# autonomousvision/gta

Hardware: AMD Instinct MI355X
Metric: GTA-attn Mtokens/s (V=5,H=W=128,d=768) (higher is better)
Workload: dtype bf16; 1 GPU; ms-enc: GTA attention forward (rep build + K/V rep pre-pass + attention kernel), B=32/GPU, H=8, Tq=1280, Tk=1280, dh=96, f_dims={'triv': 0, 'se3': 48, 'so3': 24, 'so2': 24}, views q/k=5/5; global_batch=32, parallelism=dp1

## Files before the change

gta_amd/csrc/gen_attn64.py:

```python
#!/usr/bin/env python3
import argparse

from isa_model import CheckError, Ins, barrier, branch, check_wait_states, clobber_list, label, nop, wait, write_macro

RB = 2
KS, DB, CHP = 6, 3, 12
IMG = 64 * CHP * 16
TILE = 2 * IMG
NP = IMG // 4096
THR_BITS = 0x42c00000


def _sbase(p, rb, hh):
    return 64 + 16 * rb if hh == 0 else 96 + 16 * (p * 2 + rb)


def S(p, rb, hh, r=None):
    b = _sbase(p, rb, hh)
    return f"v[{b}:{b + 15}]" if r is None else f"v{b + r}"


def Sregs(p, rb, hh):
    b = _sbase(p, rb, hh)
    return [f"v{b + i}" for i in range(16)]
# ... 620 lines not shown
                if fallthrough and step_state is not None and pend and [sorted(x) for x in pend] != [sorted(x) for x in step_state]:
                    raise CheckError(f"outstanding LDS reads at {ins.label} differ between paths")
                if fallthrough and pend:
                    step_state = [set(x) for x in pend]
                elif step_state is not None:
                    pend = [set(x) for x in step_state]
            else:
                if pend and fallthrough:
                    out.append(wait(lgkm=0))
                pend = []
            out.append(ins)
            prev = ins
            continue
        if ins.kind == "branch":
            uncond = ins.text.startswith("s_branch")
            to_step = ins.target.startswith("L_step")
            rare = ins.target.startswith("L_slow") or ins.target.startswith("L_tail")
            if pend and ((uncond and not (to_step and carry)) or (not uncond and not rare)):
                out.append(wait(lgkm=0))
                pend = []
            if uncond and to_step and carry and pend:
                if step_state is None:
                    step_state = [set(x) for x in pend]
                elif [sorted(x) for x in pend] != [sorted(x) for x in step_state]:
                    raise CheckError(f"outstanding LDS reads at the jump to {ins.target} differ from the step label's state")
            out.append(ins)
            prev = ins
            continue
        if ins.kind == "wait" and ins.fx[2] is not None:
            del pend[:max(0, len(pend) - ins.fx[2])]
            out.append(ins)
            prev = ins
            continue
        touched = list(ins.rd) + list(ins.wr)
        i = need(touched)
        if i >= 0:
            left = min(len(pend) - 1 - i, 15)
            out.append(wait(lgkm=left))
            del pend[:len(pend) - left]
        if ins.kind == "ready":
            continue
        out.append(ins)
        if ins.kind == "ds":
            pend.append(set(ins.wr))
        prev = ins
    if pend:
        out.append(wait(lgkm=0))
    if carry and seed_state is None and step_state is not None:
        return insert_waits(prog, carry=True, seed_state=step_state)
    return out


class Sim:
    def __init__(self, gen, prog, n_tiles, rebase_at=(), has_tail=False, items=2, first_rebase=True):
        self.g, self.prog, self.n, self.rebase_at, self.has_tail, self.items = gen, prog, n_tiles, set(rebase_at), has_tail, items
        self.first_rebase = first_rebase or not gen.first_fast
        self.labels = {ins.label: i for i, ins in enumerate(prog) if ins.kind == "label"}
        self.count = 0

    def fail(self, msg, ins=None):
        raise CheckError(f"{msg}" + (f"   at: {ins.text}" if ins is not None else ""))

    def run(self):
        R = self.g.R
        self.kslot = [None] * R
        self.vslot = [None] * R
        self.vmq = []
        self.got = {}
        self.hist = []
        stats = {"instr": 0, "mfma": 0}
        for t in range(R):
            for i in range(NP):
                self.vmq.append(("K", t % R, i, (0, t)))
        for t in range(R - 1):
            for i in range(NP):
                self.vmq.append(("V", t % R, i, (0, t)))
        kptr, vptr = (0, R), (0, R - 1)
        for item in range(self.items):
            kptr, vptr = self.run_item(item, kptr, vptr, stats)
        return stats

    def land(self, ent):
        ring, slot, piece, tile = ent
        key = (ring, slot)
        cur = self.pending_tile.get(key)
        if cur is None or cur[0] != tile:
            self.pending_tile[key] = (tile, set())
        self.pending_tile[key][1].add(piece)

    def run_item(self, item, kptr, vptr, stats):
        g, R, n = self.g, self.g.R, self.n
        regs = {}
        pend_ds = []
        pending_regs = set()
        sc = {}
        self.pending_tile = getattr(self, "pending_tile", {})
        msver = [0, 0]
        o_done = {(rb, d): set() for rb in range(RB) for d in range(DB)}
        l_done = {rb: set() for rb in range(RB)}
        sums = {}
        packed_from = {}
        exps = {}
        flags = {"scc": 0, "vcc": 0}
        ksel_done = vsel_done = False
        pc = 0
        prog = self.prog
        rebased_tiles = set()
        steps = 0

        def setreg(r, tag, need):
            old = regs.get(r)
            if old is not None and old[1] > 0:
                self.fail(f"register {r} overwritten with {old[1]} reads of {old[0]} outstanding", cur)
            regs[r] = [tag, need]

        def usereg(r, expect_prefix, cur_ins):
            v = regs.get(r)
            if v is None:
                self.fail(f"register {r} read but never written (expected {expect_prefix})", cur_ins)
            if r in pending_regs:
                self.fail(f"register {r} read before its LDS read was waited for", cur_ins)
            if tuple(v[0][:len(expect_prefix)]) != tuple(expect_prefix):
                self.fail(f"register {r} holds {v[0]}, expected {expect_prefix}", cur_ins)
            v[1] -= 1
            return v[0]

        while True:
            if pc >= len(prog):
                self.fail("fell off the end of the program")
            cur = prog[pc]
            pc += 1
            if cur.kind == "label":
                continue
            stats["instr"] += 1
            check_wait_states(self.hist, cur)
            sem = cur.sem
            k = cur.kind
            for r in list(cur.rd) + list(cur.wr):
                if r in pending_regs and k != "ds":
                    self.fail(f"{r} touched while its LDS read is outstanding", cur)
            if k == "mfma":
                stats["mfma"] += 1
            if sem is None:
                self.hist.append(cur)
                continue
            op = sem[0]
            if op == "nop":
                pass
            elif op == "waitcnt":
                vm, lgkm = sem[1:]
                while lgkm is not None and len(pend_ds) > lgkm:
                    for r in pend_ds.pop(0):
                        pending_regs.discard(r)
                while vm is not None and len(self.vmq) > vm:
                    self.land(self.vmq.pop(0))
            elif op == "barrier":
                for key, (tile, pieces) in list(self.pending_tile.items()):
                    if len(pieces) == NP:
                        (self.kslot if key[0] == "K" else self.vslot)[key[1]] = tile
                        del self.pending_tile[key]
            elif op == "item_begin":
                for t in range(R):
                    if self.kslot[t] != (item, t):
                        self.fail(f"item {item}: K slot {t} holds {self.kslot[t]} at item begin")
                for t in range(R - 1):
                    if self.vslot[t] != (item, t):
                        self.fail(f"item {item}: V slot {t} holds {self.vslot[t]} at item begin")
            elif op == "j0":
                sc["j"] = 0
            elif op == "j1":
                sc["j1"] = sc["j"] + 1
            elif op == "jinc":
                sc["j"] += 1
                steps += 1
            elif op in ("nm1", "nmr", "nmr1", "readkn", "ds_tab"):
                if op == "ds_tab":
                    pend_ds.append(list(cur.wr))
                    pending_regs.update(cur.wr)
            elif op == "cmp_nmr":
                flags["scc_eq"] = sc["j"] == n - R
            elif op == "cmp_nmr1":
                flags["scc_eq"] = sc["j"] == n - R + 1
            elif op == "kinit":
                sc["kptr"] = kptr
            elif op == "vinit":
                sc["vptr"] = vptr
            elif op == "ksel":
                if flags["scc_eq"]:
                    if sc["kptr"] != (item, n):
                        self.fail(f"K stream switches items at position {sc['kptr']}")
                    sc["kptr"] = (item + 1, 0)
                    ksel_done = True
            elif op == "vsel":
                if flags["scc_eq"]:
                    if sc["vptr"] != (item, n):
                        self.fail(f"V stream switches items at position {sc['vptr']}")
                    sc["vptr"] = (item + 1, 0)
                    vsel_done = True
            elif op == "kadv":
                if sem[1] == 0:
                    sc["kptr"] = (sc["kptr"][0], sc["kptr"][1] + 1)
            elif op == "vadv":
                if sem[1] == 0:
                    sc["vptr"] = (sc["vptr"][0], sc["vptr"][1] + 1)
            elif op == "dma":
                ring, slot, piece = sem[1], sem[2], sem[3]
                tile = sc["kptr"] if ring == "K" else sc["vptr"]
                held = (self.kslot if ring == "K" else self.vslot)[slot]
                if held is not None and held[0] == item:
                    last_needed = held[1] - 1 if ring == "K" else held[1]
                    if last_needed >= sc["j"]:
                        self.fail(f"DMA into {ring} slot {slot} at step {sc['j']} while tile {held} is still needed", cur)
                if piece == 0:
                    (self.kslot if ring == "K" else self.vslot)[slot] = None
                self.vmq.append((ring, slot, piece, tile))
            elif op == "ds_k":
                slot, ks, hh, rel = sem[1], sem[2], sem[3], sem[4]
                t = sc.get("j", 0) + rel
# ... 280 lines not shown
```

gta_amd/csrc/gen_item64.py:

```python
#!/usr/bin/env python3
import argparse

import numpy as np

import gen_attn64 as G
from isa_model import (LANES, Asm, CheckError, Ins, Wave, as_u32, assemble_check, auto_waits, bf16_rne, bf16_to_f32, check_wait_states, clobber_list,
                       regs, rtext, u2f, write_macro)

KS, DB, RB, R = 6, 3, 2, 4
IMG = 64 * 12 * 16
TILE = 2 * IMG
OFF_K, OFF_V, OFF_TAB = 0, R * IMG, 2 * R * IMG
OFF_CS = OFF_TAB + (KS + 2 * DB) * 256
CS_ROW, CS_WAVE = 96, 64 * 96
OFF_X = OFF_CS + 256 * CS_ROW
XROW, XB = 208, 32 * 208
OFF_ITEMS = OFF_X + 4 * XB
ITEM_BYTES = 64
MAX_ITEMS = 128
LDS_BYTES = OFF_ITEMS + (MAX_ITEMS + 2) * ITEM_BYTES
QT_BYTES = 1024
LN2_BITS, QN_BITS = 0x3f317218, 0x3f808659
assert LDS_BYTES <= 160 * 1024 and OFF_ITEMS % 16 == 0

D_Q, D_O, D_CS, D_LSE, D_IMG, D_KN, D_AQ, D_V = 0, 2, 4, 6, 8, 10, 12, 13
D_WORDS = 14


def row0(i):
    return 5 * i + i // 3


def V(n, k=1):
    return regs("v", n, k)


def A(n, k=1):
    return regs("a", n, k)


def Sr(n, k=1):
    return regs("s", n, k)


V_LANE16, V_LANE4 = "v8", "v9"
V_XFR = "v10"
V_XL = ["v11", "v12", "v13"]
V_QG = ["v14", "v15", "v16"]
V_OG = ["v17", "v18", "v19"]
V_CSG, V_CSG2 = "v20", "v21"
V_CSR, V_CSRA, V_CSRB = "v23", "v24", "v25"
V_OXW = "v26"
V_LSE = "v27"
V_QN = ["v28", "v29"]
V_KN = "v30"
V_LR, V_MR = ["v240", "v241"], ["v242", "v243"]
TMP = V(244, 12)
TMPX = TMP + ["v31", "v22"]
QL = [A(220 + 4 * i, 4) for i in range(9)] + [A(4 * i, 4) for i in range(3)]
AT = [A(172 + 4 * i, 4) for i in range(12)]
CT = [A(124 + 4 * i, 4) for i in range(12)]
S_STAMP = Sr(20, 4)
S_B = [Sr(24 + 2 * j, 2) for j in range(4)]
S_Q16, S_O16, S_XW = "s54", "s55", "s34"
S_PREV, S_ROW = Sr(36, 2), Sr(38, 2)
S_CUR, S_NXT = 40, 56
S_KPTR, S_VPTR, S_NXK, S_NXV = Sr(72, 2), Sr(74, 2), Sr(76, 2), Sr(78, 2)
S_WOFF = "s80"
S_T = Sr(81, 3)
S_K, S_TAB = "s97", "s35"
S_PH3 = Sr(98, 2)
S_HI = Sr(70, 2)
CLOBBER_S = [i for i in range(20, 100) if i != 32]

LOOP_OPERANDS = {"%[kptr]": rtext(S_KPTR), "%[vptr]": rtext(S_VPTR), "%[nxt_k]": rtext(S_NXK), "%[nxt_v]": rtext(S_NXV),
                 "%[woff]": S_WOFF, "%[lane16]": V_LANE16, "%[qn0]": V_QN[0], "%[qn1]": V_QN[1], "%[kn]": V_KN,
                 "%[lr0]": V_LR[0], "%[lr1]": V_LR[1], "%[mr0]": V_MR[0], "%[mr1]": V_MR[1]}
OPERANDS = ("tabl", "nit", "wave", "qrb", "orb", "qtb_lo", "qtb_hi", "prof_lo", "prof_hi", "n", "tailj", "Tk")


def cur(d, k=2):
    return Sr(S_CUR + d, k) if k > 1 else f"s{S_CUR + d}"


def nxt(d, k=2):
    return Sr(S_NXT + d, k) if k > 1 else f"s{S_NXT + d}"


class ItemGen:
    def __init__(self, loop_kw=None, stamps=True, head_wait=False, phases=False):
        self.loop_kw = dict(G.BEST) if loop_kw is None else loop_kw
        self.stamps = stamps
        self.head_wait = head_wait
        self.phases = phases

    def phase(self, a, k):
        if not self.phases:
            return
        t = TMP
        self._nph = getattr(self, "_nph", 0) + 1
        lab = f"L_noph{k}_{self._nph}_%="
        a.waitcnt(lgkm=0)
        a.s_or_b32(S_T[0], "%[prof_lo]", "%[prof_hi]")
        a.branch("s_cbranch_scc0", lab)
        if k == 3:
            a.s_memtime(S_PH3)
            a.waitcnt(lgkm=0)
            a.label(lab)
            return
        a.s_memtime(S_T[1:3])
        a.waitcnt(lgkm=0)
        a.s_exec_set("lane0")
        a.v_mov_b32(t[4], 0)
        a.v_mov_b32(t[6], S_T[1])
        a.v_mov_b32(t[7], S_T[2])
        a.global_store(2, t[4], t[6:8], S_ROW, 8 * (1, 2, 3)[k])
        a.s_exec_set("all")
        a.label(lab)

    def hi(self, a):
        a.s_exec_set("hi", S_HI)

    def chunk_prologue(self, a):
        t = TMP
        lane, l31, lh = t[0], t[1], t[2]
        a.v_mbcnt_lane(lane)
        a.v_and_b32(l31, 31, lane)
        a.v_lshrrev_b32(lh, 5, lane)
        a.v_lshlrev_b32(V_LANE16, 4, lane)
        a.v_lshlrev_b32(V_LANE4, 2, lane)
        a.s_mul_i32(S_XW, "%[wave]", XB)
        a.s_add_u32(S_XW, S_XW, OFF_X)
        a.s_mul_i32(S_WOFF, "%[wave]", IMG // 4)
        a.s_lshl_b32(S_Q16, "%[qrb]", 4)
        a.s_lshl_b32(S_O16, "%[orb]", 4)
        a.s_mov_b32(S_HI[0], 0)
        a.s_mov_b32(S_HI[1], -1)
        a.s_lshl_b32(S_T[0], "%[wave]", 6)
        for m in range(3):
            lm, g, col = t[3], t[4], t[5]
            a.v_add_u32(lm, 4 * m, lane)
            a.v_mul_u32_u24(g, 43, lm)
            a.v_lshrrev_b32(g, 9, g)
            a.v_mul_u32_u24(col, 12, g)
            a.v_sub_u32(col, lm, col)
            a.v_lshlrev_b32(col, 4, col)
            a.v_mul_u32_u24(t[6], XROW, g)
            a.v_add_u32(t[6], t[6], col)
            a.v_add_u32(V_XL[m], S_XW, t[6])
            a.v_add_u32(t[7], row0(m), g)
            a.v_add_u32(t[7], S_T[0], t[7])
            a.v_mul_lo_u32(t[6], t[7], "%[qrb]")
            a.v_add_u32(V_QG[m], t[6], col)
            a.v_add_u32(t[7], row0(m), g)
            a.v_mul_lo_u32(t[6], t[7], "%[orb]")
            a.v_add_u32(V_OG[m], t[6], col)
        a.s_mul_i32(S_T[1], "%[wave]", CS_WAVE)
        a.v_add_u32(V_CSG, S_T[1], V_LANE16)
        a.v_add_u32(V_CSG2, 4096, V_CSG)
        a.s_mov_b32(S_K, 0)
        a.s_mov_b32(S_TAB, "%[tabl]")
        if self.phases:
            a.s_mov_b64(S_PH3, 0)
        self.read_desc(a, 0)
        self.request(a)
        self.cs_dma(a)
        self.advance_desc(a)
        a.v_mbcnt_lane(lane)
        a.v_and_b32(l31, 31, lane)
        a.v_lshrrev_b32(lh, 5, lane)
        a.v_mul_u32_u24(t[3], XROW, l31)
        a.v_add_u32(t[3], S_XW, t[3])
        a.v_lshlrev_b32(t[4], 4, lh)
        a.v_add_u32(V_XFR, t[3], t[4])
        a.v_lshlrev_b32(t[4], 5, lh)
        a.v_add_u32(V_OXW, t[3], t[4])
        a.s_mul_i32(S_T[1], "%[wave]", CS_WAVE)
        a.s_add_u32(S_T[1], S_T[1], OFF_CS)
        a.v_mul_u32_u24(t[3], CS_ROW, l31)
        a.v_add_u32(V_CSR, S_T[1], t[3])
        a.v_lshlrev_b32(t[4], 5, lh)
        a.v_add_u32(V_CSRA, V_CSR, t[4])
        a.v_lshlrev_b32(t[4], 6, lh)
        a.v_add_u32(V_CSRB, V_CSR, t[4])
        a.s_lshl_b32(S_T[0], "%[wave]", 6)
        a.v_add_u32(t[3], S_T[0], l31)
        a.v_lshlrev_b32(V_LSE, 2, t[3])
        a.v_add_u32(t[3], OFF_TAB, V_LANE4)
        for i, r in enumerate(G.KOFF + [G.VOFF[d][h] for d in range(DB) for h in range(2)]):
            a.ds_read(32, [r], t[3], 256 * i)
        a.waitcnt(lgkm=0)
        self.read_desc(a, 1)
        self.stamp_row(a, S_PREV)
        a.waitcnt(vm=0)

    def read_desc(self, a, entry):
        t = TMPX
        a.v_mov_b32(V_QN[0], S_TAB)
        for i in range(3):
            a.ds_read(128, t[4 * i:4 * i + 4], V_QN[0], ITEM_BYTES * entry + 16 * i)
        a.ds_read(32, [t[12]], V_QN[0], ITEM_BYTES * entry + 48)
        a.ds_read(32, [t[13]], V_QN[0], ITEM_BYTES * entry + 52)
        a.waitcnt(lgkm=0)
        for d in range(D_WORDS):
            a.v_readfirstlane_b32(f"s{S_NXT + d}", t[d])

    def advance_desc(self, a):
        for d in range(0, D_WORDS, 2):
            a.s_mov_b64(Sr(S_CUR + d, 2), Sr(S_NXT + d, 2))

    def bases(self, a, first, step, n=4):
        a.s_mov_b64(S_B[0], first)
        for j in range(1, n):
            a.s_add_u32(S_B[j][0], S_B[j - 1][0], step)
            a.s_addc_u32(S_B[j][1], S_B[j - 1][1], 0)

    def tile_bases(self, a, desc, typ):
        a.s_add_u32(S_B[0][0], "%[qtb_lo]", desc(D_AQ, 1))
        a.s_addc_u32(S_B[0][1], "%[qtb_hi]", 0)
        if typ:
            a.s_add_u32(S_B[0][0], S_B[0][0], 12 * QT_BYTES)
            a.s_addc_u32(S_B[0][1], S_B[0][1], 0)
        for j in range(1, 3):
            a.s_add_u32(S_B[j][0], S_B[j - 1][0], 4096)
            a.s_addc_u32(S_B[j][1], S_B[j - 1][1], 0)

    def request(self, a):
        self.bases(a, nxt(D_Q), S_Q16)
        for i in range(12):
            a.global_load(4, QL[i], V_QG[i % 3], S_B[i // 3])
        self.tile_bases(a, nxt, 0)
        for i in range(12):
            a.global_load(4, AT[i], V_LANE16, S_B[i // 4], 1024 * (i % 4))
        a.global_load(1, [V_KN], V_LANE4, nxt(D_KN))

    def cs_dma(self, a):
        a.s_mul_i32(S_T[0], "%[wave]", CS_WAVE)
        for part, (voff, cnt) in enumerate(((V_CSG, 4), (V_CSG2, 2))):
            a.add(f"s_add_u32 m0, {S_T[0]}, {OFF_CS + 4096 * part}", "salu", [S_T[0]], ["m0", "scc"], ("s_add_m0", S_T[0], OFF_CS + 4096 * part))
            a.nop(1)
            for i in range(cnt):
                a.add(f"global_load_lds_dwordx4 {voff}, {rtext(nxt(D_CS))}" + (f" offset:{1024 * i}" if i else ""), "dma",
                      ["m0", voff] + nxt(D_CS), [], ("global_load_lds", voff, nxt(D_CS), 1024 * i))

    def stamp_row(self, a, dst):
        a.s_lshl_b32(S_T[0], cur(D_V, 1), 6)
        a.s_add_u32(dst[0], "%[prof_lo]", S_T[0])
        a.s_addc_u32(dst[1], "%[prof_hi]", 0)

    def stamp(self, a, tag, last=False):
        if not self.stamps:
            return
        lab = f"L_nostamp_{tag}_%="
        t = TMP
        a.s_or_b32(S_T[0], "%[prof_lo]", "%[prof_hi]")
        a.branch("s_cbranch_scc0", lab)
        a.s_memtime(S_STAMP[0:2])
        a.s_memrealtime(S_STAMP[2:4])
        a.waitcnt(lgkm=0)
        if not last:
            self.stamp_row(a, S_ROW)
        a.s_exec_set("lane0")
        a.v_mov_b32(t[4], 0)
        for i in range(4):
            a.v_mov_b32(t[i], S_STAMP[i])
        a.global_store(2, t[4], t[0:2], S_PREV, 8 * 4)
        a.global_store(2, t[4], t[2:4], S_PREV, 8 * 6)
        if self.phases:
            a.v_mov_b32(t[6], S_PH3[0])
            a.v_mov_b32(t[7], S_PH3[1])
            a.global_store(2, t[4], t[6:8], S_PREV, 8 * 7)
        if not last:
            a.global_store(2, t[4], t[0:2], S_ROW, 8 * 0)
            a.global_store(2, t[4], t[2:4], S_ROW, 8 * 5)
            a.s_mov_b64(S_PREV, S_ROW)
        a.s_exec_set("all")
        a.label(lab)

    def prologue(self, a):
        t = TMP
        QR = [[V(44 + 4 * (rb * KS + ks), 4) for ks in range(KS)] for rb in range(RB)]
        ACC = [[V(92 + 48 * rb + 16 * d, 16) for d in range(DB)] for rb in range(RB)]
        CSP = [[V(188 + 16 * rb + 8 * sl, 8) for sl in range(2)] for rb in range(RB)]
        QSQ = ["v220", "v221"]
        PK = V(222, 8)
        a.waitcnt(vm=14)
        self.phase(a, 0)
        for rb in range(RB):
            for i in range(KS):
                a.ds_write(128, V_XL[i % 3], QL[rb * KS + i], row0(i) * XROW)
            for ks in range(KS):
                a.ds_read(128, QR[rb][ks], V_XFR, 32 * ks)
        for rb in range(RB):
            for h in range(2):
                a.ds_read(128, CSP[rb][0][4 * h:4 * h + 4], V_CSR, rb * 32 * CS_ROW + 16 * h)
            for h in range(2):
                a.ds_read(128, CSP[rb][1][4 * h:4 * h + 4], V_CSRA, rb * 32 * CS_ROW + 32 + 16 * h)

        def mfmas(rb):
            out = []
            for i in range(12):
                d, kk, lo = i % 3, (i // 3) & 1, i // 6
                tl = 2 * d + kk
                out.append((ACC[rb][d], AT[6 * lo + tl], QR[rb][tl], 0 if i < 3 else ACC[rb][d]))
            return out

        def post(rb):
            ops = []
            for ks in range(KS):
                x = ACC[rb][ks >> 1][8 * (ks & 1):8 * (ks & 1) + 8]
                if ks >= 4:
                    cs = CSP[rb][ks - 4]
                    if ks == 4:
                        ops.append(lambda: self.hi(a))
                    for p in range(4):
                        x0, x1, c, s = x[2 * p], x[2 * p + 1], cs[2 * p], cs[2 * p + 1]
                        tt = t[p]
                        ops.append(lambda x1=x1, s=s, tt=tt: a.v_mul_f32(tt, x1, s))
                        ops.append(lambda x1=x1, c=c: a.v_mul_f32(x1, x1, c))
                        ops.append(lambda x0=x0, x1=x1, s=s: a.v_fmac_f32(x1, x0, s))
                        ops.append(lambda x0=x0, c=c, tt=tt: a.v_fma_f32(x0, x0, c, tt, neg=(False, False, True)))
                    if ks == 4:
                        ops.append(lambda: a.s_exec_set("all"))
                pk = PK[4 * (ks & 1):4 * (ks & 1) + 4]
                for w in range(4):
                    ops.append(lambda w=w, pk=pk, x=x: a.v_cvt_pk_bf16_f32(pk[w], x[2 * w], x[2 * w + 1]))
                for w in range(4):
                    ops.append(lambda w=w, pk=pk, ks=ks: a.v_accvgpr_write_b32(G.Qregs(rb, ks)[w], pk[w]))
                for i in range(8):
                    if ks == 0 and i == 0:
                        ops.append(lambda x=x: a.v_mul_f32(QSQ[rb], x[0], x[0]))
                    else:
                        ops.append(lambda i=i, x=x: a.v_fmac_f32(QSQ[rb], x[i], x[i]))
            return ops

        m0, m1 = mfmas(0), mfmas(1)
        for d16, a4, b4, c in m0:
            a.mfma(d16, a4, b4, c)
        p0 = post(0)
        k = 0
# ... 140 lines not shown
            k = 0
            for i, (d16, a4, b4, c) in enumerate(mf):
                a.mfma(d16, a4, b4, c)
                if pad_at is not None and i == pad_at:
                    a.nop(pad)
                if i >= first:
                    for _ in range(per):
                        if k < len(fill):
                            fill[k]()
                            k += 1
            while k < len(fill):
                fill[k]()
                k += 1

        for op in build_of(0):
            op()
        arith, a = a.out, main
        mi, per = 0, max(1, len(arith) // max(len(mem.out), 1))
        for i, ins in enumerate(arith):
            a.raw(ins)
            if (i + 1) % per == 0 and mi < len(mem.out):
                a.raw(mem.out[mi])
                mi += 1
        for ins in mem.out[mi:]:
            a.raw(ins)
        a.s_lshl_b32(S_T[0], "%[wave]", 2)
        a.s_mul_i32(S_T[0], S_T[0], S_O16)
        a.s_add_u32(S_B[0][0], cur(D_O)[0], S_T[0])
        a.s_addc_u32(S_B[0][1], cur(D_O)[1], 0)
        for j in range(1, 4):
            a.s_add_u32(S_B[j][0], S_B[j - 1][0], S_O16)
            a.s_addc_u32(S_B[j][1], S_B[j - 1][1], 0)
        a.waitcnt(vm=0 if last else 31)
        weave(mfmas(0), build_of(1))
        weave(mfmas(1), post(0) + stores(0), first=3, pad_at=2, pad=8)
        a.nop(8)
        for op in post(1) + stores(1):
            op()
        a.s_exec_set("lo")
        for rb in range(RB):
            a.global_store(1, V_LSE, [t[8 + rb]], cur(D_LSE), 128 * rb)
        a.s_exec_set("all")

    def loop_program(self):
        G.configure(96)
        gen = G.Gen(R=R, **self.loop_kw)
        out = []
        head_vm = not self.head_wait
        for ins in gen.program():
            if ins.sem and ins.sem[0] == "ds_tab":
                continue
            if head_vm and ins.kind == "wait" and ins.fx == ("waitcnt", 0, None):
                head_vm = False
                continue
            out.append(ins.bound(LOOP_OPERANDS))
        return gen, out

    def program(self, stub_loop=False, pad4=False):
        a = Asm()
        self.chunk_prologue(a)
        a.label("L_item_%=")
        self.stamp(a, "item")
        self.prologue(a)
        a.waitcnt(lgkm=0)
        self.phase(a, 1)
        if pad4:
            a.nop(1)
        head = auto_waits(a.out)
        a = Asm()
        self.phase(a, 2)
        a.s_add_u32(S_T[0], S_K, 1)
        a.s_cmp("ge", "u32", S_T[0], "%[nit]")
        a.branch("s_cbranch_scc1", "L_last_%=")
        self.epilogue(a)
        a.waitcnt(lgkm=0)
        self.phase(a, 3)
        self.advance_desc(a)
        a.s_add_u32(S_K, S_K, 1)
        a.s_add_u32(S_TAB, S_TAB, ITEM_BYTES)
        self.read_desc(a, 1)
        a.branch("s_branch", "L_item_%=")
        a.label("L_last_%=")
        self.epilogue(a, last=True)
        a.waitcnt(lgkm=0)
        self.phase(a, 3)
        self.stamp(a, "end", last=True)
        a.waitcnt(vm=0)
        a.pseudo("end")
        tail = auto_waits(a.out)
        if stub_loop:
            mid = [Ins("", "pseudo", fx=("pseudo", "loop"))]
        else:
            mid = self.loop_program()[1]
        return head + mid + tail


def qt_chan_q(d, rho):
    lh, j, i = (rho >> 2) & 1, rho >> 3, rho & 3
    return 32 * d + 8 * lh + 4 * j + i if j < 2 else 32 * d + 16 + 8 * lh + 4 * (j - 2) + i


def qt_chan_o_in(d, kk, k):
    lh, i = k >> 3, k & 7
    return 32 * d + 16 * kk + (i & 3) + 8 * (i >> 2) + 4 * lh


# ... 8 lines not shown
    for typ, M in ((0, Mf), (1, Mi)):
        for d in range(3):
            for kk in range(2):
                for rho in range(32):
                    r = qt_chan_o_out(d, rho) if typ else qt_chan_q(d, rho)
                    for k in range(16):
                        c = qt_chan_o_in(d, kk, k) if typ else 32 * d + 16 * kk + k
                        x = np.float32(M[r, c])
                        hi = bf16_rne(np.array([x], np.float32))[0]
                        lo = bf16_rne(np.array([x - bf16_to_f32(np.uint32(hi))], np.float32))[0]
                        for part, val in ((0, hi), (1, lo)):
                            tile = 12 * typ + 6 * part + 2 * d + kk
                            o16[(tile * 1024 + (((k >> 3) * 32 + rho) * 16 + (k & 7) * 2)) // 2] = val
    return out


def decode_matrix(tiles, typ):
    M = np.zeros((96, 96), np.float64)
    t16 = tiles.view(np.uint16)
    for d in range(3):
        for kk in range(2):
            for rho in range(32):
                r = qt_chan_o_out(d, rho) if typ else qt_chan_q(d, rho)
                for k in range(16):
                    c = qt_chan_o_in(d, kk, k) if typ else 32 * d + 16 * kk + k
                    for part in range(2):
                        tile = 12 * typ + 6 * part + 2 * d + kk
                        M[r, c] += float(bf16_to_f32(np.uint32(t16[(tile * 1024 + (((k >> 3) * 32 + rho) * 16 + (k & 7) * 2)) // 2])))
    return M


class Case:

    def __init__(self, seed, n_items, exact, n_tiles=8):
        rng = np.random.default_rng(seed)
        self.rng, self.exact, self.n_items, self.n_tiles = rng, exact, n_items, n_tiles
        B, H, Nq, Tq = 2, 3, 2, 512
        self.B, self.H, self.Nq, self.Tq = B, H, Nq, Tq
        self.q_st, self.o_st = 3 * H * 96, H * 96
        if exact:
            q = rng.integers(-3, 4, size=(B, Tq, 3 * H * 96)).astype(np.float32)
        else:
            q = rng.standard_normal((B, Tq, 3 * H * 96)).astype(np.float32)
        self.qbits = bf16_rne(q).astype(np.uint16)
        self.obits = np.zeros((B, Tq, H * 96), np.uint16)
        if exact:
            ang = rng.integers(0, 4, size=(B, Tq, 12))
            cs = np.stack([np.round(np.cos(ang * np.pi / 2)), np.round(np.sin(ang * np.pi / 2))], -1).astype(np.float32)
        else:
            ang = rng.uniform(0, 2 * np.pi, size=(B, Tq, 12))
            cs = np.stack([np.cos(ang), np.sin(ang)], -1).astype(np.float32)
        self.cs = cs
        self.lse = np.zeros((B, H, Tq), np.float32)
        self.kn = rng.uniform(0.5, 2.0, size=(B, H, 64)).astype(np.float32)
        self.Mf, self.Mi, tiles = [], [], []
        for v in range(B * Nq):
            Mf, Mi = np.zeros((96, 96)), np.zeros((96, 96))
            scale = 2.0 if exact else 0.1472
            for M, inv in ((Mf, 0), (Mi, 1)):
                blocks = [(4 * i, 4) for i in range(12)] + [x for g in range(3) for x in ((48 + 8 * g, 3), (51 + 8 * g, 5))]
                for o, n in blocks:
                    if exact:
                        blk = rng.integers(-2, 3, size=(n, n)).astype(np.float64)
                    else:
                        blk = rng.standard_normal((n, n)) * (1.0 if inv else scale)
                    M[o:o + n, o:o + n] = blk
                for c in range(72, 96):
                    M[c, c] = 1.0 if inv else scale
            self.Mf.append(Mf); self.Mi.append(Mi)
            tiles.append(build_view_tiles(Mf, Mi))
        self.tiles = np.concatenate(tiles)
        self.MfD = [decode_matrix(self.tiles[24 * 1024 * v:24 * 1024 * (v + 1)], 0) for v in range(B * Nq)]
        self.MiD = [decode_matrix(self.tiles[24 * 1024 * v:24 * 1024 * (v + 1)], 1) for v in range(B * Nq)]
        self.A_Q, self.A_O, self.A_CS, self.A_LSE, self.A_KN, self.A_QT, self.A_IMG, self.A_PROF = (0x1000000 * (i + 1) for i in range(8))
        self.items = []
        order = rng.permutation(B * H * 2)[:n_items]
        for w in order:
            bh, qt = divmod(int(w), 2)
            b, h = divmod(bh, H)
            self.items.append(dict(b=b, h=h, q0=256 * qt, view=(256 * qt) // (Tq // Nq), V=int(w)))
        self.oacc, self.lrun, self.mrun = {}, {}, {}

    def desc(self, it):
        b, h, q0 = it["b"], it["h"], it["q0"]
        bh = b * self.H + h
        d = np.zeros(16, np.uint32)

        def put(i, addr):
            d[i], d[i + 1] = addr & 0xffffffff, addr >> 32
        put(D_Q, self.A_Q + ((b * self.Tq + q0) * self.q_st + h * 96) * 2)
        put(D_O, self.A_O + ((b * self.Tq + q0) * self.o_st + h * 96) * 2)
        put(D_CS, self.A_CS + ((b * self.Tq + q0) * 24) * 4)
        put(D_LSE, self.A_LSE + (bh * self.Tq + q0) * 4)
        put(D_IMG, self.A_IMG + bh * self.n_tiles * TILE)
        put(D_KN, self.A_KN + bh * 64 * 4)
        d[D_AQ] = (b * self.Nq + it["view"]) * 24 * 1024
        d[D_V] = it["V"]
        return d

    def loop_results(self, item, wave):
        key = (item, wave)
        if key not in self.oacc:
            rng = np.random.default_rng(1000 * item + wave + 7)
            if self.exact:
                l_half = np.full((RB, LANES), 2.0, np.float32)
                o = (rng.integers(-8, 9, size=(RB, DB, 16, LANES)) * 4).astype(np.float32)
            else:
                l_half = rng.uniform(1.0, 40.0, size=(RB, LANES)).astype(np.float32)
                o = (rng.standard_normal((RB, DB, 16, LANES)) * 8).astype(np.float32)
            self.oacc[key], self.lrun[key] = o, l_half
            self.mrun[key] = rng.uniform(-3, 9, size=(RB, 32)).astype(np.float32)
        return self.oacc[key], self.lrun[key], self.mrun[key]

    def expect_q(self, item, wave):
        it = self.items[item]
        out = np.zeros((RB, 32, 96), np.float64)
        for rb in range(RB):
            for r in range(32):
                t = it["q0"] + wave * 64 + rb * 32 + r
                q = bf16_to_f32(self.qbits[it["b"], t, it["h"] * 96:(it["h"] + 1) * 96].astype(np.uint32)).astype(np.float64)
                x = self.MfD[it["b"] * self.Nq + it["view"]] @ q
                for p in range(12):
                    c, s = (float(v) for v in self.cs[it["b"], t, p])
                    x0, x1 = x[72 + 2 * p], x[73 + 2 * p]
                    x[72 + 2 * p], x[73 + 2 * p] = c * x0 - s * x1, s * x0 + c * x1
                out[rb, r] = x
        return out

    def expect_o(self, item, wave):
        it = self.items[item]
        o, lh_, m = self.loop_results(item, wave)
        rows = np.zeros((RB, 32, 96), np.float64)
        lse = np.zeros((RB, 32), np.float64)
        for rb in range(RB):
            for r in range(32):
                l = np.float32(lh_[rb, r] + lh_[rb, r + 32])
                inv = np.float32(1.0) / l
                ot = np.zeros(96, np.float64)
                for d in range(DB):
                    for reg in range(16):
                        for h in range(2):
                            chan = 32 * d + (reg & 3) + 8 * (reg >> 2) + 4 * h
                            ot[chan] = bf16_to_f32(bf16_rne(np.array([o[rb, d, reg, r + 32 * h] * inv], np.float32)))[0]
                t = it["q0"] + wave * 64 + rb * 32 + r
                x = self.MiD[it["b"] * self.Nq + it["view"]] @ ot
                for p in range(12):
                    c, s = (float(v) for v in self.cs[it["b"], t, p])
                    x0, x1 = x[72 + 2 * p], x[73 + 2 * p]
                    x[72 + 2 * p], x[73 + 2 * p] = c * x0 + s * x1, c * x1 - s * x0
                rows[rb, r] = x
                lse[rb, r] = (float(m[rb, r]) + np.log2(float(l))) * np.log(2.0)
        return rows, lse


def run_case(prog, case, wave, prof=False):
    LDS0 = np.zeros(160 * 1024, np.uint8)
    n = case.n_items
    for k in range(n + 2):
        it = case.items[min(k, n - 1)]
        LDS0[OFF_ITEMS + 64 * k:OFF_ITEMS + 64 * k + 64] = case.desc(it).view(np.uint8)
    tab = (np.arange(12 * 64, dtype=np.uint32) * 4 + 0x100000).view(np.uint8)
    LDS0[OFF_TAB:OFF_TAB + len(tab)] = tab
    inputs = {"%[tabl]": OFF_ITEMS, "%[nit]": n, "%[wave]": wave, "%[qrb]": case.q_st * 2, "%[orb]": case.o_st * 2,
              "%[qtb_lo]": case.A_QT & 0xffffffff, "%[qtb_hi]": case.A_QT >> 32,
              "%[prof_lo]": (case.A_PROF & 0xffffffff) if prof else 0, "%[prof_hi]": (case.A_PROF >> 32) if prof else 0,
              "%[n]": case.n_tiles, "%[tailj]": 0xffffffff, "%[Tk]": 64 * case.n_tiles}
    w = Wave(inputs=inputs, seed=wave + 11)
    w.lds[:] = LDS0
    qb = case.qbits.reshape(-1).view(np.uint8)
    ob = case.obits.reshape(-1).view(np.uint8)
    profb = np.zeros(64 * 64, np.uint8)
    for base, arr in ((case.A_Q, qb), (case.A_O, ob), (case.A_CS, case.cs.reshape(-1).view(np.uint8)), (case.A_LSE, case.lse.reshape(-1).view(np.uint8)),
                      (case.A_KN, case.kn.reshape(-1).view(np.uint8)), (case.A_QT, case.tiles), (case.A_PROF, profb)):
        w.map_buffer(base, arr)
    state = {"item": 0}
    tol = 0.0 if case.exact else 2.0 ** -7

    def chk(name, got, want, rel):
        got, want = np.asarray(got, np.float64), np.asarray(want, np.float64)
        err = np.abs(got - want)
        lim = rel * np.maximum(np.abs(want), 1e-3) + (0 if rel == 0 else 1e-6)
        if not (err <= lim).all():
            i = np.unravel_index(np.argmax(err - lim), err.shape)
            raise CheckError(f"wave {wave} item {state['item']}: {name} differs at {i}: got {got[i]!r}, expected {want[i]!r}")

    def loop_hook(wv):
        k = state["item"]
        it = case.items[k]
        wv.wait(0, None)
        exp = case.expect_q(k, wave)
        for rb in range(RB):
            for ks in range(KS):
                rr = G.Qregs(rb, ks)
                for lane in range(LANES):
                    l31, lh = lane & 31, lane >> 5
                    chunk = 2 * ks + lh
                    got = []
                    for wd in range(4):
                        u = int(wv.v[wv.ridx(rr[wd])][lane])
                        got += [float(bf16_to_f32(np.uint32(u & 0xffff))), float(bf16_to_f32(np.uint32(u >> 16)))]
                    want = exp[rb, l31, 8 * chunk:8 * chunk + 8]
                    if case.exact:
                        chk(f"Q' rb {rb} k-step {ks} lane {lane}", got, want, 0.0)
                    else:
                        wb = bf16_to_f32(bf16_rne(want.astype(np.float32))).astype(np.float64)
                        err = np.abs(np.array(got) - wb)
                        if not (err <= 2.0 ** -7 * np.maximum(np.abs(wb), 1e-2)).all():
                            raise CheckError(f"wave {wave} item {k}: Q' rb {rb} k-step {ks} lane {lane}: {got} vs {wb}")
            qn = u2f(wv.v[wv.ridx(V_QN[rb])])
            want = np.sqrt((exp[rb] ** 2).sum(-1)) * 1.0041
            chk(f"|q'| rb {rb}", qn[:32], want, 1e-5)
            chk(f"|q'| rb {rb} (upper lanes)", qn[32:], want, 1e-5)
        bh = it["b"] * case.H + it["h"]
        chk("key norms", u2f(wv.v[wv.ridx(V_KN)])[:case.n_tiles], case.kn[it["b"], it["h"], :case.n_tiles], 0.0)
        img = case.A_IMG + bh * case.n_tiles * TILE + wave * (IMG // 4)
        nit_ = case.items[min(k + 1, n - 1)]
        nimg = case.A_IMG + (nit_["b"] * case.H + nit_["h"]) * case.n_tiles * TILE + wave * (IMG // 4)
        for nm, pair, want in (("kptr", S_KPTR, img + R * TILE), ("vptr", S_VPTR, img + (R - 1) * TILE + IMG), ("nxt_k", S_NXK, nimg), ("nxt_v", S_NXV, nimg + IMG)):
            if wv.s64(pair) != want:
                raise CheckError(f"wave {wave} item {k}: {nm} = 0x{wv.s64(pair):x}, expected 0x{want:x}")
        for i, r in enumerate(G.KOFF + [G.VOFF[d][h] for d in range(DB) for h in range(2)]):
            if not (wv.v[wv.ridx(r)] == (np.arange(64) + 64 * i) * 4 + 0x100000).all():
                raise CheckError(f"the loop's LDS offset register {r} does not hold table row {i}")
        junk = np.random.default_rng(5).integers(0x7f800001, 0x7fffffff, size=(208, LANES), dtype=np.uint32)
        wv.v[32 + 12:240] = junk[:196]
        wv.v[256 + 124:512] = np.random.default_rng(6).integers(0x7f800001, 0x7fffffff, size=(132, LANES), dtype=np.uint32)
        o, lh_, m = case.loop_results(k, wave)
        for rb in range(RB):
            for d in range(DB):
                for i, r in enumerate(G.Oregs(rb, d)):
                    wv.v[wv.ridx(r)] = as_u32(o[rb, d, i])
            wv.v[wv.ridx(V_LR[rb])] = as_u32(lh_[rb])
            wv.v[wv.ridx(V_MR[rb])] = as_u32(np.concatenate([m[rb], m[rb]]))
        for _ in range(21):
            wv.vm.append([])
        return None

    def end_hook(wv):
        return "__end__"

    def check_outputs(k):
        rows, lse = case.expect_o(k, wave)
        it = case.items[k]
        for rb in range(RB):
            for r in range(32):
                t = it["q0"] + wave * 64 + rb * 32 + r
                got = bf16_to_f32(case.obits[it["b"], t, it["h"] * 96:(it["h"] + 1) * 96].astype(np.uint32)).astype(np.float64)
                want = rows[rb, r]
                if case.exact:
                    chk(f"O row {t}", got, want, 0.0)
                else:
                    wb = bf16_to_f32(bf16_rne(want.astype(np.float32))).astype(np.float64)
                    err = np.abs(got - wb)
                    if not (err <= 2.0 ** -6 * np.maximum(np.abs(wb), 2e-2)).all():
                        i = int(np.argmax(err))
                        raise CheckError(f"wave {wave} item {k}: O row {t} channel {i}: {got[i]} vs {wb[i]}")
                chk(f"LSE row {t}", [case.lse[it["b"], it["h"], t]], [lse[rb, r]], 1e-5)

    def loop_hook2(wv):
        r = loop_hook(wv)
        state["item"] += 1
        return r
    w.hooks = {"loop": loop_hook2, "end": end_hook}
    w.run(prog, checker=check_wait_states)
    if w.vm or w.lgkm:
        raise CheckError("memory operations outstanding at the end of the statement")
    for k in range(n):
        state["item"] = k
        check_outputs(k)
    if prof:
        P = profb.view(np.uint64).reshape(-1, 8)
        for k, it in enumerate(case.items):
            row = P[it["V"]]
            if not (row[0] > 0 and row[4] > row[0] and row[5] > 0 and row[6] > row[5]):
                raise CheckError(f"profile row of item {k}: {row}")
    return w


def check(verbose=False, waves=(0, 1, 2, 3), **kw):
    gen = ItemGen(**kw)
    prog = gen.program(stub_loop=True)
    stats = {"instructions": sum(1 for x in prog if x.kind not in ("label", "pseudo")), "mfma": sum(1 for x in prog if x.kind == "mfma")}
    for seed, n_items, exact in ((1, 3, True), (2, 3, False), (3, 1, False)):
        case = Case(seed, n_items, exact)
        for wave in waves:
            run_case(prog, case, wave, prof=(seed == 2 and wave == 1))
        if verbose:
            print(f"  ok: case seed {seed}: {n_items} items, {'exact' if exact else 'random'} inputs, waves {list(waves)}")
    return stats


def emit(path, prog, prog_p4=None, prog_ph=None):
    with open(path, "w") as f:
        f.write("// generated by gen_item64.py (make regen) -- do not edit\n")
        for name, val in (("OFF_CS", OFF_CS), ("OFF_X", OFF_X), ("OFF_ITEMS", OFF_ITEMS), ("ITEM_BYTES", ITEM_BYTES), ("MAX_ITEMS", MAX_ITEMS),
                          ("LDS_BYTES", LDS_BYTES), ("D_Q", D_Q), ("D_O", D_O), ("D_CS", D_CS), ("D_LSE", D_LSE), ("D_IMG", D_IMG), ("D_KN", D_KN),
                          ("D_AQ", D_AQ), ("D_V", D_V)):
            f.write(f"#define GTA_ITEM64_{name} {val}\n")
        write_macro(f, "GTA_ATTN64_ITEMS", prog)
        if prog_p4 is not None:
            f.write("#ifdef GTA_ATTN64_DIAG\n")
            write_macro(f, "GTA_ATTN64_ITEMS_P4", prog_p4)
            if prog_ph is not None:
                write_macro(f, "GTA_ATTN64_ITEMS_PH", prog_ph)
            f.write("#endif\n")
        regs_ = [f"v{i}" for i in range(8, 256)] + [f"a{i}" for i in range(256)] + [f"s{i}" for i in CLOBBER_S]
        f.write("#define GTA_ATTN64_ITEMS_CLOBBERS \\\n    " + clobber_list(regs_) + "\n")


if __name__ == "__main__":
    ap = argparse.ArgumentParser()
    ap.add_argument("--out", default=None)
    ap.add_argument("--verbose", action="store_true")
    ap.add_argument("--no-check", action="store_true")
    a_ = ap.parse_args()
    if not a_.no_check:
        st = check(verbose=a_.verbose)
        if a_.verbose:
            print("item stream without the tile loop:", st)
    full = ItemGen().program()
    assemble_check(full, sops=OPERANDS)
    if a_.out:
        emit(a_.out, full, ItemGen().program(pad4=True), ItemGen(phases=True).program())
```

gta_amd/csrc/gta_attn64_items.inc:

```
#define GTA_ITEM64_OFF_CS 101376
#define GTA_ITEM64_OFF_X 125952
#define GTA_ITEM64_OFF_ITEMS 152576
#define GTA_ITEM64_ITEM_BYTES 64
#define GTA_ITEM64_MAX_ITEMS 128
#define GTA_ITEM64_LDS_BYTES 160896
#define GTA_ITEM64_D_Q 0
#define GTA_ITEM64_D_O 2
#define GTA_ITEM64_D_CS 4
#define GTA_ITEM64_D_LSE 6
#define GTA_ITEM64_D_IMG 8
#define GTA_ITEM64_D_KN 10
#define GTA_ITEM64_D_AQ 12
#define GTA_ITEM64_D_V 13
#define GTA_ATTN64_ITEMS \
    "v_mbcnt_lo_u32_b32 v244, -1, 0\n\t" \
    "v_mbcnt_hi_u32_b32 v244, -1, v244\n\t" \
    "v_and_b32 v245, 31, v244\n\t" \
    "v_lshrrev_b32 v246, 5, v244\n\t" \
    "v_lshlrev_b32 v8, 4, v244\n\t" \
    "v_lshlrev_b32 v9, 2, v244\n\t" \
    "s_mul_i32 s34, %[wave], 0x00001a00\n\t" \
    "s_add_u32 s34, s34, 0x0001ec00\n\t" \
    "s_mul_i32 s80, %[wave], 0x00000c00\n\t" \
    "s_lshl_b32 s54, %[qrb], 4\n\t" \
// ... 74 lines not shown
    "v_readfirstlane_b32 s66, v254\n\t" \
    "v_readfirstlane_b32 s67, v255\n\t" \
    "v_readfirstlane_b32 s68, v31\n\t" \
    "v_readfirstlane_b32 s69, v22\n\t" \
    "s_mov_b64 s[24:25], s[56:57]\n\t" \
    "s_add_u32 s26, s24, s54\n\t" \
    "s_addc_u32 s27, s25, 0\n\t" \
    "s_add_u32 s28, s26, s54\n\t" \
    "s_addc_u32 s29, s27, 0\n\t" \
    "s_add_u32 s30, s28, s54\n\t" \
    "s_addc_u32 s31, s29, 0\n\t" \
    "global_load_dwordx4 a[220:223], v14, s[24:25]\n\t" \
    "global_load_dwordx4 a[224:227], v15, s[24:25]\n\t" \
    "global_load_dwordx4 a[228:231], v16, s[24:25]\n\t" \
    "global_load_dwordx4 a[232:235], v14, s[26:27]\n\t" \
    "global_load_dwordx4 a[236:239], v15, s[26:27]\n\t" \
    "global_load_dwordx4 a[240:243], v16, s[26:27]\n\t" \
    "global_load_dwordx4 a[244:247], v14, s[28:29]\n\t" \
    "global_load_dwordx4 a[248:251], v15, s[28:29]\n\t" \
    "global_load_dwordx4 a[252:255], v16, s[28:29]\n\t" \
    "global_load_dwordx4 a[0:3], v14, s[30:31]\n\t" \
    "global_load_dwordx4 a[4:7], v15, s[30:31]\n\t" \
    "global_load_dwordx4 a[8:11], v16, s[30:31]\n\t" \
    "s_add_u32 s24, %[qtb_lo], s68\n\t" \
    "s_addc_u32 s25, %[qtb_hi], 0\n\t" \
    "s_add_u32 s26, s24, 0x00001000\n\t" \
    "s_addc_u32 s27, s25, 0\n\t" \
    "s_add_u32 s28, s26, 0x00001000\n\t" \
    "s_addc_u32 s29, s27, 0\n\t" \
    "global_load_dwordx4 a[172:175], v8, s[24:25]\n\t" \
    "global_load_dwordx4 a[176:179], v8, s[24:25] offset:1024\n\t" \
    "global_load_dwordx4 a[180:183], v8, s[24:25] offset:2048\n\t" \
    "global_load_dwordx4 a[184:187], v8, s[24:25] offset:3072\n\t" \
    "global_load_dwordx4 a[188:191], v8, s[26:27]\n\t" \
    "global_load_dwordx4 a[192:195], v8, s[26:27] offset:1024\n\t" \
    "global_load_dwordx4 a[196:199], v8, s[26:27] offset:2048\n\t" \
    "global_load_dwordx4 a[200:203], v8, s[26:27] offset:3072\n\t" \
    "global_load_dwordx4 a[204:207], v8, s[28:29]\n\t" \
    "global_load_dwordx4 a[208:211], v8, s[28:29] offset:1024\n\t" \
    "global_load_dwordx4 a[212:215], v8, s[28:29] offset:2048\n\t" \
    "global_load_dwordx4 a[216:219], v8, s[28:29] offset:3072\n\t" \
    "global_load_dword v30, v9, s[66:67]\n\t" \
    "s_mul_i32 s81, %[wave], 0x00001800\n\t" \
    "s_add_u32 m0, s81, 101376\n\t" \
    "s_nop 0\n\t" \
    "global_load_lds_dwordx4 v20, s[60:61]\n\t" \
    "global_load_lds_dwordx4 v20, s[60:61] offset:1024\n\t" \
    "global_load_lds_dwordx4 v20, s[60:61] offset:2048\n\t" \
    "global_load_lds_dwordx4 v20, s[60:61] offset:3072\n\t" \
    "s_add_u32 m0, s81, 105472\n\t" \
    "s_nop 0\n\t" \
    "global_load_lds_dwordx4 v21, s[60:61]\n\t" \
    "global_load_lds_dwordx4 v21, s[60:61] offset:1024\n\t" \
    "s_mov_b64 s[40:41], s[56:57]\n\t" \
    "s_mov_b64 s[42:43], s[58:59]\n\t" \
    "s_mov_b64 s[44:45], s[60:61]\n\t" \
    "s_mov_b64 s[46:47], s[62:63]\n\t" \
    "s_mov_b64 s[48:49], s[64:65]\n\t" \
    "s_mov_b64 s[50:51], s[66:67]\n\t" \
    "s_mov_b64 s[52:53], s[68:69]\n\t" \
    "v_mbcnt_lo_u32_b32 v244, -1, 0\n\t" \
    "v_mbcnt_hi_u32_b32 v244, -1, v244\n\t" \
    "v_and_b32 v245, 31, v244\n\t" \
    "v_lshrrev_b32 v246, 5, v244\n\t" \
    "v_mul_u32_u24 v247, 0x000000d0, v245\n\t" \
    "v_add_u32 v247, s34, v247\n\t" \
    "v_lshlrev_b32 v248, 4, v246\n\t" \
    "v_add_u32 v10, v247, v248\n\t" \
    "v_lshlrev_b32 v248, 5, v246\n\t" \
    "v_add_u32 v26, v247, v248\n\t" \
    "s_mul_i32 s82, %[wave], 0x00001800\n\t" \
    "s_add_u32 s82, s82, 0x00018c00\n\t" \
    "v_mul_u32_u24 v247, 0x00000060, v245\n\t" \
    "v_add_u32 v23, s82, v247\n\t" \
    "v_lshlrev_b32 v248, 5, v246\n\t" \
    "v_add_u32 v24, v23, v248\n\t" \
    "v_lshlrev_b32 v248, 6, v246\n\t" \
    "v_add_u32 v25, v23, v248\n\t" \
    "s_lshl_b32 s81, %[wave], 6\n\t" \
    "v_add_u32 v247, s81, v245\n\t" \
    "v_lshlrev_b32 v27, 2, v247\n\t" \
    "v_add_u32 v247, 0x00018000, v9\n\t" \
    "ds_read_b32 v32, v247\n\t" \
    "ds_read_b32 v33, v247 offset:256\n\t" \
    "ds_read_b32 v34, v247 offset:512\n\t" \
    "ds_read_b32 v35, v247 offset:768\n\t" \
    "ds_read_b32 v36, v247 offset:1024\n\t" \
    "ds_read_b32 v37, v247 offset:1280\n\t" \
    "ds_read_b32 v38, v247 offset:1536\n\t" \
    "ds_read_b32 v39, v247 offset:1792\n\t" \
    "ds_read_b32 v40, v247 offset:2048\n\t" \
    "ds_read_b32 v41, v247 offset:2304\n\t" \
    "ds_read_b32 v42, v247 offset:2560\n\t" \
    "ds_read_b32 v43, v247 offset:2816\n\t" \
    "s_waitcnt lgkmcnt(0)\n\t" \
    "v_mov_b32 v28, s35\n\t" \
    "ds_read_b128 v[244:247], v28 offset:64\n\t" \
    "ds_read_b128 v[248:251], v28 offset:80\n\t" \
    "ds_read_b128 v[252:255], v28 offset:96\n\t" \
    "ds_read_b32 v31, v28 offset:112\n\t" \
    "ds_read_b32 v22, v28 offset:116\n\t" \
    "s_waitcnt lgkmcnt(0)\n\t" \
    "v_readfirstlane_b32 s56, v244\n\t" \
    "v_readfirstlane_b32 s57, v245\n\t" \
    "v_readfirstlane_b32 s58, v246\n\t" \
    "v_readfirstlane_b32 s59, v247\n\t" \
    "v_readfirstlane_b32 s60, v248\n\t" \
    "v_readfirstlane_b32 s61, v249\n\t" \
    "v_readfirstlane_b32 s62, v250\n\t" \
    "v_readfirstlane_b32 s63, v251\n\t" \
    "v_readfirstlane_b32 s64, v252\n\t" \
    "v_readfirstlane_b32 s65, v253\n\t" \
    "v_readfirstlane_b32 s66, v254\n\t" \
    "v_readfirstlane_b32 s67, v255\n\t" \
    "v_readfirstlane_b32 s68, v31\n\t" \
    "v_readfirstlane_b32 s69, v22\n\t" \
    "s_lshl_b32 s81, s53, 6\n\t" \
    "s_add_u32 s36, %[prof_lo], s81\n\t" \
    "s_addc_u32 s37, %[prof_hi], 0\n\t" \
    "s_waitcnt vmcnt(0)\n\t" \
    "L_item_%=:\n\t" \
    "s_or_b32 s81, %[prof_lo], %[prof_hi]\n\t" \
    "s_cbranch_scc0 L_nostamp_item_%=\n\t" \
    "s_memtime s[20:21]\n\t" \
    "s_memrealtime s[22:23]\n\t" \
    "s_waitcnt lgkmcnt(0)\n\t" \
    "s_lshl_b32 s81, s53, 6\n\t" \
    "s_add_u32 s38, %[prof_lo], s81\n\t" \
    "s_addc_u32 s39, %[prof_hi], 0\n\t" \
    "s_mov_b64 exec, 1\n\t" \
    "v_mov_b32 v248, 0\n\t" \
    "v_mov_b32 v244, s20\n\t" \
    "v_mov_b32 v245, s21\n\t" \
    "v_mov_b32 v246, s22\n\t" \
    "v_mov_b32 v247, s23\n\t" \
    "global_store_dwordx2 v248, v[244:245], s[36:37] offset:32\n\t" \
    "global_store_dwordx2 v248, v[246:247], s[36:37] offset:48\n\t" \
    "global_store_dwordx2 v248, v[244:245], s[38:39]\n\t" \
    "global_store_dwordx2 v248, v[246:247], s[38:39] offset:40\n\t" \
    "s_mov_b64 s[36:37], s[38:39]\n\t" \
    "s_mov_b64 exec, -1\n\t" \
    "L_nostamp_item_%=:\n\t" \
    "s_waitcnt vmcnt(14)\n\t" \
    "ds_write_b128 v11, a[220:223]\n\t" \
    "ds_write_b128 v12, a[224:227] offset:1040\n\t" \
    "ds_write_b128 v13, a[228:231] offset:2080\n\t" \
    "ds_write_b128 v11, a[232:235] offset:3328\n\t" \
    "ds_write_b128 v12, a[236:239] offset:4368\n\t" \
    "ds_write_b128 v13, a[240:243] offset:5408\n\t" \
    "ds_read_b128 v[44:47], v10\n\t" \
    "ds_read_b128 v[48:51], v10 offset:32\n\t" \
    "ds_read_b128 v[52:55], v10 offset:64\n\t" \
    "ds_read_b128 v[56:59], v10 offset:96\n\t" \
    "ds_read_b128 v[60:63], v10 offset:128\n\t" \
    "ds_read_b128 v[64:67], v10 offset:160\n\t" \
    "ds_write_b128 v11, a[244:247]\n\t" \
    "ds_write_b128 v12, a[248:251] offset:1040\n\t" \
    "ds_write_b128 v13, a[252:255] offset:2080\n\t" \
    "ds_write_b128 v11, a[0:3] offset:3328\n\t" \
    "ds_write_b128 v12, a[4:7] offset:4368\n\t" \
    "ds_write_b128 v13, a[8:11] offset:5408\n\t" \
    "ds_read_b128 v[68:71], v10\n\t" \
    "ds_read_b128 v[72:75], v10 offset:32\n\t" \
    "ds_read_b128 v[76:79], v10 offset:64\n\t" \
    "ds_read_b128 v[80:83], v10 offset:96\n\t" \
    "ds_read_b128 v[84:87], v10 offset:128\n\t" \
    "ds_read_b128 v[88:91], v10 offset:160\n\t" \
    "ds_read_b128 v[188:191], v23\n\t" \
    "ds_read_b128 v[192:195], v23 offset:16\n\t" \
    "ds_read_b128 v[196:199], v24 offset:32\n\t" \
    "ds_read_b128 v[200:203], v24 offset:48\n\t" \
    "ds_read_b128 v[204:207], v23 offset:3072\n\t" \
    "ds_read_b128 v[208:211], v23 offset:3088\n\t" \
    "ds_read_b128 v[212:215], v24 offset:3104\n\t" \
    "ds_read_b128 v[216:219], v24 offset:3120\n\t" \
    "s_waitcnt lgkmcnt(15)\n\t" \
    "v_mfma_f32_32x32x16_bf16 v[92:107], a[172:175], v[44:47], 0\n\t" \
    "v_mfma_f32_32x32x16_bf16 v[108:123], a[180:183], v[52:55], 0\n\t" \
    "v_mfma_f32_32x32x16_bf16 v[124:139], a[188:191], v[60:63], 0\n\t" \
    "v_mfma_f32_32x32x16_bf16 v[92:107], a[176:179], v[48:51], v[92:107]\n\t" \
    "v_mfma_f32_32x32x16_bf16 v[108:123], a[184:187], v[56:59], v[108:123]\n\t" \
    "v_mfma_f32_32x32x16_bf16 v[124:139], a[192:195], v[64:67], v[124:139]\n\t" \
    "v_mfma_f32_32x32x16_bf16 v[92:107], a[196:199], v[44:47], v[92:107]\n\t" \
    "v_mfma_f32_32x32x16_bf16 v[108:123], a[204:207], v[52:55], v[108:123]\n\t" \
    "v_mfma_f32_32x32x16_bf16 v[124:139], a[212:215], v[60:63], v[124:139]\n\t" \
    "v_mfma_f32_32x32x16_bf16 v[92:107], a[200:203], v[48:51], v[92:107]\n\t" \
    "v_mfma_f32_32x32x16_bf16 v[108:123], a[208:211], v[56:59], v[108:123]\n\t" \
    "v_mfma_f32_32x32x16_bf16 v[124:139], a[216:219], v[64:67], v[124:139]\n\t" \
    "s_waitcnt lgkmcnt(13)\n\t" \
    "v_mfma_f32_32x32x16_bf16 v[140:155], a[172:175], v[68:71], 0\n\t" \
    "s_waitcnt lgkmcnt(11)\n\t" \
    "v_mfma_f32_32x32x16_bf16 v[156:171], a[180:183], v[76:79], 0\n\t" \
    "s_waitcnt lgkmcnt(9)\n\t" \
    "v_mfma_f32_32x32x16_bf16 v[172:187], a[188:191], v[84:87], 0\n\t" \
    "s_nop 6\n\t" \
    "v_mfma_f32_32x32x16_bf16 v[140:155], a[176:179], v[72:75], v[140:155]\n\t" \
// ... 258 lines not shown
    "v_mul_f32 v187, v187, v218\n\t" \
    "v_fmac_f32 v187, v186, v219\n\t" \
    "v_fma_f32 v186, v186, v218, -v247\n\t" \
    "v_cvt_pk_bf16_f32 v226, v180, v181\n\t" \
    "v_cvt_pk_bf16_f32 v227, v182, v183\n\t" \
    "v_cvt_pk_bf16_f32 v228, v184, v185\n\t" \
    "v_cvt_pk_bf16_f32 v229, v186, v187\n\t" \
    "v_accvgpr_write_b32 a168, v226\n\t" \
    "v_accvgpr_write_b32 a169, v227\n\t" \
    "v_accvgpr_write_b32 a170, v228\n\t" \
    "v_accvgpr_write_b32 a171, v229\n\t" \
    "v_fmac_f32 v221, v180, v180\n\t" \
    "v_fmac_f32 v221, v181, v181\n\t" \
    "v_fmac_f32 v221, v182, v182\n\t" \
    "v_fmac_f32 v221, v183, v183\n\t" \
    "v_fmac_f32 v221, v184, v184\n\t" \
    "v_fmac_f32 v221, v185, v185\n\t" \
    "v_fmac_f32 v221, v186, v186\n\t" \
    "v_fmac_f32 v221, v187, v187\n\t" \
    "v_mov_b32 v252, v220\n\t" \
    "v_mov_b32 v253, v221\n\t" \
    "s_nop 0\n\t" \
    "v_permlane32_swap_b32 v220, v252\n\t" \
    "v_permlane32_swap_b32 v221, v253\n\t" \
    "v_add_f32 v220, v220, v252\n\t" \
    "v_add_f32 v221, v221, v253\n\t" \
    "v_sqrt_f32 v220, v220\n\t" \
    "v_sqrt_f32 v221, v221\n\t" \
    "s_nop 0\n\t" \
    "v_mul_f32 v28, 0x3f808659, v220\n\t" \
    "v_mul_f32 v29, 0x3f808659, v221\n\t" \
    "s_add_u32 s81, s80, 0x00018000\n\t" \
    "s_add_u32 s72, s48, s81\n\t" \
    "s_addc_u32 s73, s49, 0\n\t" \
    "s_add_u32 s81, s80, 0x00015000\n\t" \
    "s_add_u32 s74, s48, s81\n\t" \
    "s_addc_u32 s75, s49, 0\n\t" \
    "s_add_u32 s81, s80, 0\n\t" \
    "s_add_u32 s76, s64, s81\n\t" \
    "s_addc_u32 s77, s65, 0\n\t" \
    "s_add_u32 s81, s80, 0x00003000\n\t" \
    "s_add_u32 s78, s64, s81\n\t" \
    "s_addc_u32 s79, s65, 0\n\t" \
    "s_waitcnt lgkmcnt(0)\n\t" \
    "s_mov_b32 s84, 0\n\t" \
    "s_mov_b32 s87, s80\n\t" \
    "s_mov_b64 s[90:91], s[72:73]\n\t" \
    "s_mov_b64 s[92:93], s[74:75]\n\t" \
    "s_sub_u32 s94, %[n], 1\n\t" \
    "s_sub_u32 s95, %[n], 4\n\t" \
    "s_sub_u32 s96, %[n], 3\n\t" \
    "v_mov_b32 v52, 0\n\t" \
    "v_mov_b32 v53, 0\n\t" \
    "s_waitcnt lgkmcnt(0)\n\t" \
    "s_barrier\n\t" \
    "ds_read_b128 a[172:175], v32 offset:0\n\t" \
    "ds_read_b128 a[176:179], v32 offset:6144\n\t" \
    "ds_read_b128 a[180:183], v33 offset:0\n\t" \
    "ds_read_b128 a[184:187], v33 offset:6144\n\t" \
    "ds_read_b128 a[188:191], v34 offset:0\n\t" \
    "ds_read_b128 a[192:195], v34 offset:6144\n\t" \
    "ds_read_b128 a[196:199], v35 offset:0\n\t" \
    "ds_read_b128 a[200:203], v35 offset:6144\n\t" \
    "ds_read_b128 a[204:207], v36 offset:0\n\t" \
    "ds_read_b128 a[208:211], v36 offset:6144\n\t" \
    "ds_read_b128 a[212:215], v37 offset:0\n\t" \
    "ds_read_b128 a[216:219], v37 offset:6144\n\t" \
    "s_waitcnt lgkmcnt(11)\n\t" \
    "v_mfma_f32_32x32x16_bf16 v[64:79], a[172:175], a[124:127], 0\n\t" \
    "v_accvgpr_write_b32 a28, 0\n\t" \
    "v_accvgpr_write_b32 a29, 0\n\t" \
    "v_accvgpr_write_b32 a30, 0\n\t" \
    "v_accvgpr_write_b32 a31, 0\n\t" \
    "v_mfma_f32_32x32x16_bf16 v[80:95], a[172:175], a[148:151], 0\n\t" \
    "v_accvgpr_write_b32 a32, 0\n\t" \
    "v_accvgpr_write_b32 a33, 0\n\t" \
    "v_accvgpr_write_b32 a34, 0\n\t" \
    "v_accvgpr_write_b32 a35, 0\n\t" \
    "s_waitcnt lgkmcnt(10)\n\t" \
    "v_mfma_f32_32x32x16_bf16 v[96:111], a[176:179], a[124:127], 0\n\t" \
    "ds_read_b128 a[172:175], v32 offset:12288\n\t" \
    "v_accvgpr_write_b32 a36, 0\n\t" \
    "v_accvgpr_write_b32 a37, 0\n\t" \
    "v_accvgpr_write_b32 a38, 0\n\t" \
    "v_accvgpr_write_b32 a39, 0\n\t" \
    "v_mfma_f32_32x32x16_bf16 v[112:127], a[176:179], a[148:151], 0\n\t" \
    "v_accvgpr_write_b32 a40, 0\n\t" \
    "v_accvgpr_write_b32 a41, 0\n\t" \
    "v_accvgpr_write_b32 a42, 0\n\t" \
    "v_accvgpr_write_b32 a43, 0\n\t" \
    "s_waitcnt lgkmcnt(10)\n\t" \
    "v_mfma_f32_32x32x16_bf16 v[64:79], a[180:183], a[128:131], v[64:79]\n\t" \
    "ds_read_b128 a[176:179], v32 offset:18432\n\t" \
    "v_accvgpr_write_b32 a44, 0\n\t" \
    "v_accvgpr_write_b32 a45, 0\n\t" \
    "v_accvgpr_write_b32 a46, 0\n\t" \
    "v_accvgpr_write_b32 a47, 0\n\t" \
    "v_mfma_f32_32x32x16_bf16 v[80:95], a[180:183], a[152:155], v[80:95]\n\t" \
    "v_accvgpr_write_b32 a48, 0\n\t" \
    "v_accvgpr_write_b32 a49, 0\n\t" \
    "v_accvgpr_write_b32 a50, 0\n\t" \
    "v_accvgpr_write_b32 a51, 0\n\t" \
    "s_waitcnt lgkmcnt(10)\n\t" \
    "v_mfma_f32_32x32x16_bf16 v[96:111], a[184:187], a[128:131], v[96:111]\n\t" \
    "ds_read_b128 a[180:183], v33 offset:12288\n\t" \
    "v_accvgpr_write_b32 a52, 0\n\t" \
    "v_accvgpr_write_b32 a53, 0\n\t" \
// ... 5834 lines not shown
    "v_readfirstlane_b32 s66, v254\n\t" \
    "v_readfirstlane_b32 s67, v255\n\t" \
    "v_readfirstlane_b32 s68, v31\n\t" \
    "v_readfirstlane_b32 s69, v22\n\t" \
    "s_mov_b64 s[24:25], s[56:57]\n\t" \
    "s_add_u32 s26, s24, s54\n\t" \
    "s_addc_u32 s27, s25, 0\n\t" \
    "s_add_u32 s28, s26, s54\n\t" \
    "s_addc_u32 s29, s27, 0\n\t" \
    "s_add_u32 s30, s28, s54\n\t" \
    "s_addc_u32 s31, s29, 0\n\t" \
    "global_load_dwordx4 a[220:223], v14, s[24:25]\n\t" \
    "global_load_dwordx4 a[224:227], v15, s[24:25]\n\t" \
    "global_load_dwordx4 a[228:231], v16, s[24:25]\n\t" \
    "global_load_dwordx4 a[232:235], v14, s[26:27]\n\t" \
    "global_load_dwordx4 a[236:239], v15, s[26:27]\n\t" \
    "global_load_dwordx4 a[240:243], v16, s[26:27]\n\t" \
    "global_load_dwordx4 a[244:247], v14, s[28:29]\n\t" \
    "global_load_dwordx4 a[248:251], v15, s[28:29]\n\t" \
    "global_load_dwordx4 a[252:255], v16, s[28:29]\n\t" \
    "global_load_dwordx4 a[0:3], v14, s[30:31]\n\t" \
    "global_load_dwordx4 a[4:7], v15, s[30:31]\n\t" \
    "global_load_dwordx4 a[8:11], v16, s[30:31]\n\t" \
    "s_add_u32 s24, %[qtb_lo], s68\n\t" \
    "s_addc_u32 s25, %[qtb_hi], 0\n\t" \
    "s_add_u32 s26, s24, 0x00001000\n\t" \
    "s_addc_u32 s27, s25, 0\n\t" \
    "s_add_u32 s28, s26, 0x00001000\n\t" \
    "s_addc_u32 s29, s27, 0\n\t" \
    "global_load_dwordx4 a[172:175], v8, s[24:25]\n\t" \
    "global_load_dwordx4 a[176:179], v8, s[24:25] offset:1024\n\t" \
    "global_load_dwordx4 a[180:183], v8, s[24:25] offset:2048\n\t" \
    "global_load_dwordx4 a[184:187], v8, s[24:25] offset:3072\n\t" \
    "global_load_dwordx4 a[188:191], v8, s[26:27]\n\t" \
    "global_load_dwordx4 a[192:195], v8, s[26:27] offset:1024\n\t" \
    "global_load_dwordx4 a[196:199], v8, s[26:27] offset:2048\n\t" \
    "global_load_dwordx4 a[200:203], v8, s[26:27] offset:3072\n\t" \
    "global_load_dwordx4 a[204:207], v8, s[28:29]\n\t" \
    "global_load_dwordx4 a[208:211], v8, s[28:29] offset:1024\n\t" \
    "global_load_dwordx4 a[212:215], v8, s[28:29] offset:2048\n\t" \
    "global_load_dwordx4 a[216:219], v8, s[28:29] offset:3072\n\t" \
    "global_load_dword v30, v9, s[66:67]\n\t" \
    "s_mul_i32 s81, %[wave], 0x00001800\n\t" \
    "s_add_u32 m0, s81, 101376\n\t" \
    "s_nop 0\n\t" \
    "global_load_lds_dwordx4 v20, s[60:61]\n\t" \
    "global_load_lds_dwordx4 v20, s[60:61] offset:1024\n\t" \
    "global_load_lds_dwordx4 v20, s[60:61] offset:2048\n\t" \
    "global_load_lds_dwordx4 v20, s[60:61] offset:3072\n\t" \
    "s_add_u32 m0, s81, 105472\n\t" \
    "s_nop 0\n\t" \
    "global_load_lds_dwordx4 v21, s[60:61]\n\t" \
    "global_load_lds_dwordx4 v21, s[60:61] offset:1024\n\t" \
    "s_mov_b64 s[40:41], s[56:57]\n\t" \
    "s_mov_b64 s[42:43], s[58:59]\n\t" \
    "s_mov_b64 s[44:45], s[60:61]\n\t" \
    "s_mov_b64 s[46:47], s[62:63]\n\t" \
    "s_mov_b64 s[48:49], s[64:65]\n\t" \
    "s_mov_b64 s[50:51], s[66:67]\n\t" \
    "s_mov_b64 s[52:53], s[68:69]\n\t" \
    "v_mbcnt_lo_u32_b32 v244, -1, 0\n\t" \
    "v_mbcnt_hi_u32_b32 v244, -1, v244\n\t" \
    "v_and_b32 v245, 31, v244\n\t" \
    "v_lshrrev_b32 v246, 5, v244\n\t" \
    "v_mul_u32_u24 v247, 0x000000d0, v245\n\t" \
    "v_add_u32 v247, s34, v247\n\t" \
    "v_lshlrev_b32 v248, 4, v246\n\t" \
    "v_add_u32 v10, v247, v248\n\t" \
    "v_lshlrev_b32 v248, 5, v246\n\t" \
    "v_add_u32 v26, v247, v248\n\t" \
    "s_mul_i32 s82, %[wave], 0x00001800\n\t" \
    "s_add_u32 s82, s82, 0x00018c00\n\t" \
    "v_mul_u32_u24 v247, 0x00000060, v245\n\t" \
    "v_add_u32 v23, s82, v247\n\t" \
    "v_lshlrev_b32 v248, 5, v246\n\t" \
    "v_add_u32 v24, v23, v248\n\t" \
    "v_lshlrev_b32 v248, 6, v246\n\t" \
    "v_add_u32 v25, v23, v248\n\t" \
    "s_lshl_b32 s81, %[wave], 6\n\t" \
    "v_add_u32 v247, s81, v245\n\t" \
    "v_lshlrev_b32 v27, 2, v247\n\t" \
    "v_add_u32 v247, 0x00018000, v9\n\t" \
    "ds_read_b32 v32, v247\n\t" \
    "ds_read_b32 v33, v247 offset:256\n\t" \
    "ds_read_b32 v34, v247 offset:512\n\t" \
    "ds_read_b32 v35, v247 offset:768\n\t" \
    "ds_read_b32 v36, v247 offset:1024\n\t" \
    "ds_read_b32 v37, v247 offset:1280\n\t" \
    "ds_read_b32 v38, v247 offset:1536\n\t" \
    "ds_read_b32 v39, v247 offset:1792\n\t" \
    "ds_read_b32 v40, v247 offset:2048\n\t" \
    "ds_read_b32 v41, v247 offset:2304\n\t" \
    "ds_read_b32 v42, v247 offset:2560\n\t" \
    "ds_read_b32 v43, v247 offset:2816\n\t" \
    "s_waitcnt lgkmcnt(0)\n\t" \
    "v_mov_b32 v28, s35\n\t" \
    "ds_read_b128 v[244:247], v28 offset:64\n\t" \
    "ds_read_b128 v[248:251], v28 offset:80\n\t" \
    "ds_read_b128 v[252:255], v28 offset:96\n\t" \
    "ds_read_b32 v31, v28 offset:112\n\t" \
    "ds_read_b32 v22, v28 offset:116\n\t" \
    "s_waitcnt lgkmcnt(0)\n\t" \
    "v_readfirstlane_b32 s56, v244\n\t" \
    "v_readfirstlane_b32 s57, v245\n\t" \
    "v_readfirstlane_b32 s58, v246\n\t" \
    "v_readfirstlane_b32 s59, v247\n\t" \
    "v_readfirstlane_b32 s60, v248\n\t" \
    "v_readfirstlane_b32 s61, v249\n\t" \
    "v_readfirstlane_b32 s62, v250\n\t" \
    "v_readfirstlane_b32 s63, v251\n\t" \
    "v_readfirstlane_b32 s64, v252\n\t" \
    "v_readfirstlane_b32 s65, v253\n\t" \
    "v_readfirstlane_b32 s66, v254\n\t" \
    "v_readfirstlane_b32 s67, v255\n\t" \
    "v_readfirstlane_b32 s68, v31\n\t" \
    "v_readfirstlane_b32 s69, v22\n\t" \
    "s_lshl_b32 s81, s53, 6\n\t" \
    "s_add_u32 s36, %[prof_lo], s81\n\t" \
    "s_addc_u32 s37, %[prof_hi], 0\n\t" \
    "s_waitcnt vmcnt(0)\n\t" \
    "L_item_%=:\n\t" \
    "s_or_b32 s81, %[prof_lo], %[prof_hi]\n\t" \
    "s_cbranch_scc0 L_nostamp_item_%=\n\t" \
    "s_memtime s[20:21]\n\t" \
    "s_memrealtime s[22:23]\n\t" \
    "s_waitcnt lgkmcnt(0)\n\t" \
    "s_lshl_b32 s81, s53, 6\n\t" \
    "s_add_u32 s38, %[prof_lo], s81\n\t" \
    "s_addc_u32 s39, %[prof_hi], 0\n\t" \
    "s_mov_b64 exec, 1\n\t" \
    "v_mov_b32 v248, 0\n\t" \
    "v_mov_b32 v244, s20\n\t" \
    "v_mov_b32 v245, s21\n\t" \
    "v_mov_b32 v246, s22\n\t" \
    "v_mov_b32 v247, s23\n\t" \
    "global_store_dwordx2 v248, v[244:245], s[36:37] offset:32\n\t" \
    "global_store_dwordx2 v248, v[246:247], s[36:37] offset:48\n\t" \
    "global_store_dwordx2 v248, v[244:245], s[38:39]\n\t" \
    "global_store_dwordx2 v248, v[246:247], s[38:39] offset:40\n\t" \
    "s_mov_b64 s[36:37], s[38:39]\n\t" \
    "s_mov_b64 exec, -1\n\t" \
    "L_nostamp_item_%=:\n\t" \
    "s_waitcnt vmcnt(14)\n\t" \
    "ds_write_b128 v11, a[220:223]\n\t" \
    "ds_write_b128 v12, a[224:227] offset:1040\n\t" \
    "ds_write_b128 v13, a[228:231] offset:2080\n\t" \
    "ds_write_b128 v11, a[232:235] offset:3328\n\t" \
    "ds_write_b128 v12, a[236:239] offset:4368\n\t" \
    "ds_write_b128 v13, a[240:243] offset:5408\n\t" \
    "ds_read_b128 v[44:47], v10\n\t" \
    "ds_read_b128 v[48:51], v10 offset:32\n\t" \
    "ds_read_b128 v[52:55], v10 offset:64\n\t" \
    "ds_read_b128 v[56:59], v10 offset:96\n\t" \
    "ds_read_b128 v[60:63], v10 offset:128\n\t" \
    "ds_read_b128 v[64:67], v10 offset:160\n\t" \
    "ds_write_b128 v11, a[244:247]\n\t" \
    "ds_write_b128 v12, a[248:251] offset:1040\n\t" \
    "ds_write_b128 v13, a[252:255] offset:2080\n\t" \
    "ds_write_b128 v11, a[0:3] offset:3328\n\t" \
    "ds_write_b128 v12, a[4:7] offset:4368\n\t" \
    "ds_write_b128 v13, a[8:11] offset:5408\n\t" \
    "ds_read_b128 v[68:71], v10\n\t" \
    "ds_read_b128 v[72:75], v10 offset:32\n\t" \
    "ds_read_b128 v[76:79], v10 offset:64\n\t" \
    "ds_read_b128 v[80:83], v10 offset:96\n\t" \
    "ds_read_b128 v[84:87], v10 offset:128\n\t" \
    "ds_read_b128 v[88:91], v10 offset:160\n\t" \
    "ds_read_b128 v[188:191], v23\n\t" \
    "ds_read_b128 v[192:195], v23 offset:16\n\t" \
    "ds_read_b128 v[196:199], v24 offset:32\n\t" \
    "ds_read_b128 v[200:203], v24 offset:48\n\t" \
    "ds_read_b128 v[204:207], v23 offset:3072\n\t" \
    "ds_read_b128 v[208:211], v23 offset:3088\n\t" \
    "ds_read_b128 v[212:215], v24 offset:3104\n\t" \
    "ds_read_b128 v[216:219], v24 offset:3120\n\t" \
    "s_waitcnt lgkmcnt(15)\n\t" \
    "v_mfma_f32_32x32x16_bf16 v[92:107], a[172:175], v[44:47], 0\n\t" \
    "v_mfma_f32_32x32x16_bf16 v[108:123], a[180:183], v[52:55], 0\n\t" \
    "v_mfma_f32_32x32x16_bf16 v[124:139], a[188:191], v[60:63], 0\n\t" \
    "v_mfma_f32_32x32x16_bf16 v[92:107], a[176:179], v[48:51], v[92:107]\n\t" \
    "v_mfma_f32_32x32x16_bf16 v[108:123], a[184:187], v[56:59], v[108:123]\n\t" \
    "v_mfma_f32_32x32x16_bf16 v[124:139], a[192:195], v[64:67], v[124:139]\n\t" \
    "v_mfma_f32_32x32x16_bf16 v[92:107], a[196:199], v[44:47], v[92:107]\n\t" \
    "v_mfma_f32_32x32x16_bf16 v[108:123], a[204:207], v[52:55], v[108:123]\n\t" \
    "v_mfma_f32_32x32x16_bf16 v[124:139], a[212:215], v[60:63], v[124:139]\n\t" \
    "v_mfma_f32_32x32x16_bf16 v[92:107], a[200:203], v[48:51], v[92:107]\n\t" \
    "v_mfma_f32_32x32x16_bf16 v[108:123], a[208:211], v[56:59], v[108:123]\n\t" \
    "v_mfma_f32_32x32x16_bf16 v[124:139], a[216:219], v[64:67], v[124:139]\n\t" \
    "s_waitcnt lgkmcnt(13)\n\t" \
    "v_mfma_f32_32x32x16_bf16 v[140:155], a[172:175], v[68:71], 0\n\t" \
    "s_waitcnt lgkmcnt(11)\n\t" \
    "v_mfma_f32_32x32x16_bf16 v[156:171], a[180:183], v[76:79], 0\n\t" \
    "s_waitcnt lgkmcnt(9)\n\t" \
    "v_mfma_f32_32x32x16_bf16 v[172:187], a[188:191], v[84:87], 0\n\t" \
    "s_nop 6\n\t" \
    "v_mfma_f32_32x32x16_bf16 v[140:155], a[176:179], v[72:75], v[140:155]\n\t" \
// ... 259 lines not shown
    "v_fmac_f32 v187, v186, v219\n\t" \
    "v_fma_f32 v186, v186, v218, -v247\n\t" \
    "v_cvt_pk_bf16_f32 v226, v180, v181\n\t" \
    "v_cvt_pk_bf16_f32 v227, v182, v183\n\t" \
    "v_cvt_pk_bf16_f32 v228, v184, v185\n\t" \
    "v_cvt_pk_bf16_f32 v229, v186, v187\n\t" \
    "v_accvgpr_write_b32 a168, v226\n\t" \
    "v_accvgpr_write_b32 a169, v227\n\t" \
    "v_accvgpr_write_b32 a170, v228\n\t" \
    "v_accvgpr_write_b32 a171, v229\n\t" \
    "v_fmac_f32 v221, v180, v180\n\t" \
    "v_fmac_f32 v221, v181, v181\n\t" \
    "v_fmac_f32 v221, v182, v182\n\t" \
    "v_fmac_f32 v221, v183, v183\n\t" \
    "v_fmac_f32 v221, v184, v184\n\t" \
    "v_fmac_f32 v221, v185, v185\n\t" \
    "v_fmac_f32 v221, v186, v186\n\t" \
    "v_fmac_f32 v221, v187, v187\n\t" \
    "v_mov_b32 v252, v220\n\t" \
    "v_mov_b32 v253, v221\n\t" \
    "s_nop 0\n\t" \
    "v_permlane32_swap_b32 v220, v252\n\t" \
    "v_permlane32_swap_b32 v221, v253\n\t" \
    "v_add_f32 v220, v220, v252\n\t" \
    "v_add_f32 v221, v221, v253\n\t" \
    "v_sqrt_f32 v220, v220\n\t" \
    "v_sqrt_f32 v221, v221\n\t" \
    "s_nop 0\n\t" \
    "v_mul_f32 v28, 0x3f808659, v220\n\t" \
    "v_mul_f32 v29, 0x3f808659, v221\n\t" \
    "s_add_u32 s81, s80, 0x00018000\n\t" \
    "s_add_u32 s72, s48, s81\n\t" \
    "s_addc_u32 s73, s49, 0\n\t" \
    "s_add_u32 s81, s80, 0x00015000\n\t" \
    "s_add_u32 s74, s48, s81\n\t" \
    "s_addc_u32 s75, s49, 0\n\t" \
    "s_add_u32 s81, s80, 0\n\t" \
    "s_add_u32 s76, s64, s81\n\t" \
    "s_addc_u32 s77, s65, 0\n\t" \
    "s_add_u32 s81, s80, 0x00003000\n\t" \
    "s_add_u32 s78, s64, s81\n\t" \
    "s_addc_u32 s79, s65, 0\n\t" \
    "s_waitcnt lgkmcnt(0)\n\t" \
    "s_nop 0\n\t" \
    "s_mov_b32 s84, 0\n\t" \
    "s_mov_b32 s87, s80\n\t" \
    "s_mov_b64 s[90:91], s[72:73]\n\t" \
    "s_mov_b64 s[92:93], s[74:75]\n\t" \
    "s_sub_u32 s94, %[n], 1\n\t" \
    "s_sub_u32 s95, %[n], 4\n\t" \
    "s_sub_u32 s96, %[n], 3\n\t" \
    "v_mov_b32 v52, 0\n\t" \
    "v_mov_b32 v53, 0\n\t" \
    "s_waitcnt lgkmcnt(0)\n\t" \
    "s_barrier\n\t" \
    "ds_read_b128 a[172:175], v32 offset:0\n\t" \
    "ds_read_b128 a[176:179], v32 offset:6144\n\t" \
    "ds_read_b128 a[180:183], v33 offset:0\n\t" \
    "ds_read_b128 a[184:187], v33 offset:6144\n\t" \
    "ds_read_b128 a[188:191], v34 offset:0\n\t" \
    "ds_read_b128 a[192:195], v34 offset:6144\n\t" \
    "ds_read_b128 a[196:199], v35 offset:0\n\t" \
    "ds_read_b128 a[200:203], v35 offset:6144\n\t" \
    "ds_read_b128 a[204:207], v36 offset:0\n\t" \
    "ds_read_b128 a[208:211], v36 offset:6144\n\t" \
    "ds_read_b128 a[212:215], v37 offset:0\n\t" \
    "ds_read_b128 a[216:219], v37 offset:6144\n\t" \
    "s_waitcnt lgkmcnt(11)\n\t" \
    "v_mfma_f32_32x32x16_bf16 v[64:79], a[172:175], a[124:127], 0\n\t" \
    "v_accvgpr_write_b32 a28, 0\n\t" \
    "v_accvgpr_write_b32 a29, 0\n\t" \
    "v_accvgpr_write_b32 a30, 0\n\t" \
    "v_accvgpr_write_b32 a31, 0\n\t" \
    "v_mfma_f32_32x32x16_bf16 v[80:95], a[172:175], a[148:151], 0\n\t" \
    "v_accvgpr_write_b32 a32, 0\n\t" \
    "v_accvgpr_write_b32 a33, 0\n\t" \
    "v_accvgpr_write_b32 a34, 0\n\t" \
    "v_accvgpr_write_b32 a35, 0\n\t" \
    "s_waitcnt lgkmcnt(10)\n\t" \
    "v_mfma_f32_32x32x16_bf16 v[96:111], a[176:179], a[124:127], 0\n\t" \
    "ds_read_b128 a[172:175], v32 offset:12288\n\t" \
    "v_accvgpr_write_b32 a36, 0\n\t" \
    "v_accvgpr_write_b32 a37, 0\n\t" \
    "v_accvgpr_write_b32 a38, 0\n\t" \
    "v_accvgpr_write_b32 a39, 0\n\t" \
    "v_mfma_f32_32x32x16_bf16 v[112:127], a[176:179], a[148:151], 0\n\t" \
    "v_accvgpr_write_b32 a40, 0\n\t" \
    "v_accvgpr_write_b32 a41, 0\n\t" \
    "v_accvgpr_write_b32 a42, 0\n\t" \
    "v_accvgpr_write_b32 a43, 0\n\t" \
    "s_waitcnt lgkmcnt(10)\n\t" \
    "v_mfma_f32_32x32x16_bf16 v[64:79], a[180:183], a[128:131], v[64:79]\n\t" \
    "ds_read_b128 a[176:179], v32 offset:18432\n\t" \
    "v_accvgpr_write_b32 a44, 0\n\t" \
    "v_accvgpr_write_b32 a45, 0\n\t" \
    "v_accvgpr_write_b32 a46, 0\n\t" \
    "v_accvgpr_write_b32 a47, 0\n\t" \
    "v_mfma_f32_32x32x16_bf16 v[80:95], a[180:183], a[152:155], v[80:95]\n\t" \
    "v_accvgpr_write_b32 a48, 0\n\t" \
    "v_accvgpr_write_b32 a49, 0\n\t" \
    "v_accvgpr_write_b32 a50, 0\n\t" \
    "v_accvgpr_write_b32 a51, 0\n\t" \
    "s_waitcnt lgkmcnt(10)\n\t" \
    "v_mfma_f32_32x32x16_bf16 v[96:111], a[184:187], a[128:131], v[96:111]\n\t" \
    "ds_read_b128 a[180:183], v33 offset:12288\n\t" \
    "v_accvgpr_write_b32 a52, 0\n\t" \
    "v_accvgpr_write_b32 a53, 0\n\t" \
// ... 5834 lines not shown
    "v_readfirstlane_b32 s66, v254\n\t" \
    "v_readfirstlane_b32 s67, v255\n\t" \
    "v_readfirstlane_b32 s68, v31\n\t" \
    "v_readfirstlane_b32 s69, v22\n\t" \
    "s_mov_b64 s[24:25], s[56:57]\n\t" \
    "s_add_u32 s26, s24, s54\n\t" \
    "s_addc_u32 s27, s25, 0\n\t" \
    "s_add_u32 s28, s26, s54\n\t" \
    "s_addc_u32 s29, s27, 0\n\t" \
    "s_add_u32 s30, s28, s54\n\t" \
    "s_addc_u32 s31, s29, 0\n\t" \
    "global_load_dwordx4 a[220:223], v14, s[24:25]\n\t" \
    "global_load_dwordx4 a[224:227], v15, s[24:25]\n\t" \
    "global_load_dwordx4 a[228:231], v16, s[24:25]\n\t" \
    "global_load_dwordx4 a[232:235], v14, s[26:27]\n\t" \
    "global_load_dwordx4 a[236:239], v15, s[26:27]\n\t" \
    "global_load_dwordx4 a[240:243], v16, s[26:27]\n\t" \
    "global_load_dwordx4 a[244:247], v14, s[28:29]\n\t" \
    "global_load_dwordx4 a[248:251], v15, s[28:29]\n\t" \
    "global_load_dwordx4 a[252:255], v16, s[28:29]\n\t" \
    "global_load_dwordx4 a[0:3], v14, s[30:31]\n\t" \
    "global_load_dwordx4 a[4:7], v15, s[30:31]\n\t" \
    "global_load_dwordx4 a[8:11], v16, s[30:31]\n\t" \
    "s_add_u32 s24, %[qtb_lo], s68\n\t" \
    "s_addc_u32 s25, %[qtb_hi], 0\n\t" \
    "s_add_u32 s26, s24, 0x00001000\n\t" \
    "s_addc_u32 s27, s25, 0\n\t" \
    "s_add_u32 s28, s26, 0x00001000\n\t" \
    "s_addc_u32 s29, s27, 0\n\t" \
    "global_load_dwordx4 a[172:175], v8, s[24:25]\n\t" \
    "global_load_dwordx4 a[176:179], v8, s[24:25] offset:1024\n\t" \
    "global_load_dwordx4 a[180:183], v8, s[24:25] offset:2048\n\t" \
    "global_load_dwordx4 a[184:187], v8, s[24:25] offset:3072\n\t" \
    "global_load_dwordx4 a[188:191], v8, s[26:27]\n\t" \
    "global_load_dwordx4 a[192:195], v8, s[26:27] offset:1024\n\t" \
    "global_load_dwordx4 a[196:199], v8, s[26:27] offset:2048\n\t" \
    "global_load_dwordx4 a[200:203], v8, s[26:27] offset:3072\n\t" \
    "global_load_dwordx4 a[204:207], v8, s[28:29]\n\t" \
    "global_load_dwordx4 a[208:211], v8, s[28:29] offset:1024\n\t" \
    "global_load_dwordx4 a[212:215], v8, s[28:29] offset:2048\n\t" \
    "global_load_dwordx4 a[216:219], v8, s[28:29] offset:3072\n\t" \
    "global_load_dword v30, v9, s[66:67]\n\t" \
    "s_mul_i32 s81, %[wave], 0x00001800\n\t" \
    "s_add_u32 m0, s81, 101376\n\t" \
    "s_nop 0\n\t" \
    "global_load_lds_dwordx4 v20, s[60:61]\n\t" \
    "global_load_lds_dwordx4 v20, s[60:61] offset:1024\n\t" \
    "global_load_lds_dwordx4 v20, s[60:61] offset:2048\n\t" \
    "global_load_lds_dwordx4 v20, s[60:61] offset:3072\n\t" \
    "s_add_u32 m0, s81, 105472\n\t" \
    "s_nop 0\n\t" \
    "global_load_lds_dwordx4 v21, s[60:61]\n\t" \
    "global_load_lds_dwordx4 v21, s[60:61] offset:1024\n\t" \
    "s_mov_b64 s[40:41], s[56:57]\n\t" \
    "s_mov_b64 s[42:43], s[58:59]\n\t" \
    "s_mov_b64 s[44:45], s[60:61]\n\t" \
    "s_mov_b64 s[46:47], s[62:63]\n\t" \
    "s_mov_b64 s[48:49], s[64:65]\n\t" \
    "s_mov_b64 s[50:51], s[66:67]\n\t" \
    "s_mov_b64 s[52:53], s[68:69]\n\t" \
    "v_mbcnt_lo_u32_b32 v244, -1, 0\n\t" \
    "v_mbcnt_hi_u32_b32 v244, -1, v244\n\t" \
    "v_and_b32 v245, 31, v244\n\t" \
    "v_lshrrev_b32 v246, 5, v244\n\t" \
    "v_mul_u32_u24 v247, 0x000000d0, v245\n\t" \
    "v_add_u32 v247, s34, v247\n\t" \
    "v_lshlrev_b32 v248, 4, v246\n\t" \
    "v_add_u32 v10, v247, v248\n\t" \
    "v_lshlrev_b32 v248, 5, v246\n\t" \
    "v_add_u32 v26, v247, v248\n\t" \
    "s_mul_i32 s82, %[wave], 0x00001800\n\t" \
    "s_add_u32 s82, s82, 0x00018c00\n\t" \
    "v_mul_u32_u24 v247, 0x00000060, v245\n\t" \
    "v_add_u32 v23, s82, v247\n\t" \
    "v_lshlrev_b32 v248, 5, v246\n\t" \
    "v_add_u32 v24, v23, v248\n\t" \
    "v_lshlrev_b32 v248, 6, v246\n\t" \
    "v_add_u32 v25, v23, v248\n\t" \
    "s_lshl_b32 s81, %[wave], 6\n\t" \
    "v_add_u32 v247, s81, v245\n\t" \
    "v_lshlrev_b32 v27, 2, v247\n\t" \
    "v_add_u32 v247, 0x00018000, v9\n\t" \
    "ds_read_b32 v32, v247\n\t" \
    "ds_read_b32 v33, v247 offset:256\n\t" \
    "ds_read_b32 v34, v247 offset:512\n\t" \
    "ds_read_b32 v35, v247 offset:768\n\t" \
    "ds_read_b32 v36, v247 offset:1024\n\t" \
    "ds_read_b32 v37, v247 offset:1280\n\t" \
    "ds_read_b32 v38, v247 offset:1536\n\t" \
    "ds_read_b32 v39, v247 offset:1792\n\t" \
    "ds_read_b32 v40, v247 offset:2048\n\t" \
    "ds_read_b32 v41, v247 offset:2304\n\t" \
    "ds_read_b32 v42, v247 offset:2560\n\t" \
    "ds_read_b32 v43, v247 offset:2816\n\t" \
    "s_waitcnt lgkmcnt(0)\n\t" \
    "v_mov_b32 v28, s35\n\t" \
    "ds_read_b128 v[244:247], v28 offset:64\n\t" \
    "ds_read_b128 v[248:251], v28 offset:80\n\t" \
    "ds_read_b128 v[252:255], v28 offset:96\n\t" \
    "ds_read_b32 v31, v28 offset:112\n\t" \
    "ds_read_b32 v22, v28 offset:116\n\t" \
    "s_waitcnt lgkmcnt(0)\n\t" \
    "v_readfirstlane_b32 s56, v244\n\t" \
    "v_readfirstlane_b32 s57, v245\n\t" \
    "v_readfirstlane_b32 s58, v246\n\t" \
    "v_readfirstlane_b32 s59, v247\n\t" \
    "v_readfirstlane_b32 s60, v248\n\t" \
    "v_readfirstlane_b32 s61, v249\n\t" \
    "v_readfirstlane_b32 s62, v250\n\t" \
    "v_readfirstlane_b32 s63, v251\n\t" \
    "v_readfirstlane_b32 s64, v252\n\t" \
    "v_readfirstlane_b32 s65, v253\n\t" \
    "v_readfirstlane_b32 s66, v254\n\t" \
    "v_readfirstlane_b32 s67, v255\n\t" \
    "v_readfirstlane_b32 s68, v31\n\t" \
    "v_readfirstlane_b32 s69, v22\n\t" \
    "s_lshl_b32 s81, s53, 6\n\t" \
    "s_add_u32 s36, %[prof_lo], s81\n\t" \
    "s_addc_u32 s37, %[prof_hi], 0\n\t" \
    "s_waitcnt vmcnt(0)\n\t" \
    "L_item_%=:\n\t" \
    "s_or_b32 s81, %[prof_lo], %[prof_hi]\n\t" \
    "s_cbranch_scc0 L_nostamp_item_%=\n\t" \
    "s_memtime s[20:21]\n\t" \
    "s_memrealtime s[22:23]\n\t" \
    "s_waitcnt lgkmcnt(0)\n\t" \
    "s_lshl_b32 s81, s53, 6\n\t" \
    "s_add_u32 s38, %[prof_lo], s81\n\t" \
    "s_addc_u32 s39, %[prof_hi], 0\n\t" \
    "s_mov_b64 exec, 1\n\t" \
    "v_mov_b32 v248, 0\n\t" \
    "v_mov_b32 v244, s20\n\t" \
    "v_mov_b32 v245, s21\n\t" \
    "v_mov_b32 v246, s22\n\t" \
    "v_mov_b32 v247, s23\n\t" \
    "global_store_dwordx2 v248, v[244:245], s[36:37] offset:32\n\t" \
    "global_store_dwordx2 v248, v[246:247], s[36:37] offset:48\n\t" \
    "v_mov_b32 v250, s98\n\t" \
    "v_mov_b32 v251, s99\n\t" \
    "global_store_dwordx2 v248, v[250:251], s[36:37] offset:56\n\t" \
    "global_store_dwordx2 v248, v[244:245], s[38:39]\n\t" \
    "global_store_dwordx2 v248, v[246:247], s[38:39] offset:40\n\t" \
    "s_mov_b64 s[36:37], s[38:39]\n\t" \
    "s_mov_b64 exec, -1\n\t" \
    "L_nostamp_item_%=:\n\t" \
    "s_waitcnt vmcnt(14)\n\t" \
    "s_waitcnt lgkmcnt(0)\n\t" \
    "s_or_b32 s81, %[prof_lo], %[prof_hi]\n\t" \
    "s_cbranch_scc0 L_noph0_1_%=\n\t" \
    "s_memtime s[82:83]\n\t" \
    "s_waitcnt lgkmcnt(0)\n\t" \
    "s_mov_b64 exec, 1\n\t" \
    "v_mov_b32 v248, 0\n\t" \
    "v_mov_b32 v250, s82\n\t" \
    "v_mov_b32 v251, s83\n\t" \
    "global_store_dwordx2 v248, v[250:251], s[38:39] offset:8\n\t" \
    "s_mov_b64 exec, -1\n\t" \
    "L_noph0_1_%=:\n\t" \
    "ds_write_b128 v11, a[220:223]\n\t" \
    "ds_write_b128 v12, a[224:227] offset:1040\n\t" \
    "ds_write_b128 v13, a[228:231] offset:2080\n\t" \
    "ds_write_b128 v11, a[232:235] offset:3328\n\t" \
    "ds_write_b128 v12, a[236:239] offset:4368\n\t" \
    "ds_write_b128 v13, a[240:243] offset:5408\n\t" \
    "ds_read_b128 v[44:47], v10\n\t" \
    "ds_read_b128 v[48:51], v10 offset:32\n\t" \
    "ds_read_b128 v[52:55], v10 offset:64\n\t" \
    "ds_read_b128 v[56:59], v10 offset:96\n\t" \
    "ds_read_b128 v[60:63], v10 offset:128\n\t" \
    "ds_read_b128 v[64:67], v10 offset:160\n\t" \
    "ds_write_b128 v11, a[244:247]\n\t" \
    "ds_write_b128 v12, a[248:251] offset:1040\n\t" \
    "ds_write_b128 v13, a[252:255] offset:2080\n\t" \
    "ds_write_b128 v11, a[0:3] offset:3328\n\t" \
    "ds_write_b128 v12, a[4:7] offset:4368\n\t" \
    "ds_write_b128 v13, a[8:11] offset:5408\n\t" \
    "ds_read_b128 v[68:71], v10\n\t" \
    "ds_read_b128 v[72:75], v10 offset:32\n\t" \
    "ds_read_b128 v[76:79], v10 offset:64\n\t" \
    "ds_read_b128 v[80:83], v10 offset:96\n\t" \
    "ds_read_b128 v[84:87], v10 offset:128\n\t" \
    "ds_read_b128 v[88:91], v10 offset:160\n\t" \
    "ds_read_b128 v[188:191], v23\n\t" \
    "ds_read_b128 v[192:195], v23 offset:16\n\t" \
    "ds_read_b128 v[196:199], v24 offset:32\n\t" \
    "ds_read_b128 v[200:203], v24 offset:48\n\t" \
    "ds_read_b128 v[204:207], v23 offset:3072\n\t" \
    "ds_read_b128 v[208:211], v23 offset:3088\n\t" \
    "ds_read_b128 v[212:215], v24 offset:3104\n\t" \
    "ds_read_b128 v[216:219], v24 offset:3120\n\t" \
    "s_waitcnt lgkmcnt(15)\n\t" \
    "v_mfma_f32_32x32x16_bf16 v[92:107], a[172:175], v[44:47], 0\n\t" \
    "v_mfma_f32_32x32x16_bf16 v[108:123], a[180:183], v[52:55], 0\n\t" \
    "v_mfma_f32_32x32x16_bf16 v[124:139], a[188:191], v[60:63], 0\n\t" \
    "v_mfma_f32_32x32x16_bf16 v[92:107], a[176:179], v[48:51], v[92:107]\n\t" \
    "v_mfma_f32_32x32x16_bf16 v[108:123], a[184:187], v[56:59], v[108:123]\n\t" \
    "v_mfma_f32_32x32x16_bf16 v[124:139], a[192:195], v[64:67], v[124:139]\n\t" \
    "v_mfma_f32_32x32x16_bf16 v[92:107], a[196:199], v[44:47], v[92:107]\n\t" \
    "v_mfma_f32_32x32x16_bf16 v[108:123], a[204:207], v[52:55], v[108:123]\n\t" \
    "v_mfma_f32_32x32x16_bf16 v[124:139], a[212:215], v[60:63], v[124:139]\n\t" \
    "v_mfma_f32_32x32x16_bf16 v[92:107], a[200:203], v[48:51], v[92:107]\n\t" \
    "v_mfma_f32_32x32x16_bf16 v[108:123], a[208:211], v[56:59], v[108:123]\n\t" \
    "v_mfma_f32_32x32x16_bf16 v[124:139], a[216:219], v[64:67], v[124:139]\n\t" \
    "s_waitcnt lgkmcnt(13)\n\t" \
    "v_mfma_f32_32x32x16_bf16 v[140:155], a[172:175], v[68:71], 0\n\t" \
    "s_waitcnt lgkmcnt(11)\n\t" \
    "v_mfma_f32_32x32x16_bf16 v[156:171], a[180:183], v[76:79], 0\n\t" \
    "s_waitcnt lgkmcnt(9)\n\t" \
    "v_mfma_f32_32x32x16_bf16 v[172:187], a[188:191], v[84:87], 0\n\t" \
    "s_nop 6\n\t" \
    "v_mfma_f32_32x32x16_bf16 v[140:155], a[176:179], v[72:75], v[140:155]\n\t" \
// ... 251 lines not shown
    "v_fma_f32 v182, v182, v214, -v245\n\t" \
    "s_waitcnt lgkmcnt(0)\n\t" \
    "v_mul_f32 v246, v185, v217\n\t" \
    "v_mul_f32 v185, v185, v216\n\t" \
    "v_fmac_f32 v185, v184, v217\n\t" \
    "v_fma_f32 v184, v184, v216, -v246\n\t" \
    "v_mul_f32 v247, v187, v219\n\t" \
    "v_mul_f32 v187, v187, v218\n\t" \
    "v_fmac_f32 v187, v186, v219\n\t" \
    "v_fma_f32 v186, v186, v218, -v247\n\t" \
    "v_cvt_pk_bf16_f32 v226, v180, v181\n\t" \
    "v_cvt_pk_bf16_f32 v227, v182, v183\n\t" \
    "v_cvt_pk_bf16_f32 v228, v184, v185\n\t" \
    "v_cvt_pk_bf16_f32 v229, v186, v187\n\t" \
    "v_accvgpr_write_b32 a168, v226\n\t" \
    "v_accvgpr_write_b32 a169, v227\n\t" \
    "v_accvgpr_write_b32 a170, v228\n\t" \
    "v_accvgpr_write_b32 a171, v229\n\t" \
    "v_fmac_f32 v221, v180, v180\n\t" \
    "v_fmac_f32 v221, v181, v181\n\t" \
    "v_fmac_f32 v221, v182, v182\n\t" \
    "v_fmac_f32 v221, v183, v183\n\t" \
    "v_fmac_f32 v221, v184, v184\n\t" \
    "v_fmac_f32 v221, v185, v185\n\t" \
    "v_fmac_f32 v221, v186, v186\n\t" \
    "v_fmac_f32 v221, v187, v187\n\t" \
    "v_mov_b32 v252, v220\n\t" \
    "v_mov_b32 v253, v221\n\t" \
    "s_nop 0\n\t" \
    "v_permlane32_swap_b32 v220, v252\n\t" \
    "v_permlane32_swap_b32 v221, v253\n\t" \
    "v_add_f32 v220, v220, v252\n\t" \
    "v_add_f32 v221, v221, v253\n\t" \
    "v_sqrt_f32 v220, v220\n\t" \
    "v_sqrt_f32 v221, v221\n\t" \
    "s_nop 0\n\t" \
    "v_mul_f32 v28, 0x3f808659, v220\n\t" \
    "v_mul_f32 v29, 0x3f808659, v221\n\t" \
    "s_add_u32 s81, s80, 0x00018000\n\t" \
    "s_add_u32 s72, s48, s81\n\t" \
    "s_addc_u32 s73, s49, 0\n\t" \
    "s_add_u32 s81, s80, 0x00015000\n\t" \
    "s_add_u32 s74, s48, s81\n\t" \
    "s_addc_u32 s75, s49, 0\n\t" \
    "s_add_u32 s81, s80, 0\n\t" \
    "s_add_u32 s76, s64, s81\n\t" \
    "s_addc_u32 s77, s65, 0\n\t" \
    "s_add_u32 s81, s80, 0x00003000\n\t" \
    "s_add_u32 s78, s64, s81\n\t" \
    "s_addc_u32 s79, s65, 0\n\t" \
    "s_waitcnt lgkmcnt(0)\n\t" \
    "s_waitcnt lgkmcnt(0)\n\t" \
    "s_or_b32 s81, %[prof_lo], %[prof_hi]\n\t" \
    "s_cbranch_scc0 L_noph1_2_%=\n\t" \
    "s_memtime s[82:83]\n\t" \
    "s_waitcnt lgkmcnt(0)\n\t" \
    "s_mov_b64 exec, 1\n\t" \
    "v_mov_b32 v248, 0\n\t" \
    "v_mov_b32 v250, s82\n\t" \
    "v_mov_b32 v251, s83\n\t" \
    "global_store_dwordx2 v248, v[250:251], s[38:39] offset:16\n\t" \
    "s_mov_b64 exec, -1\n\t" \
    "L_noph1_2_%=:\n\t" \
    "s_mov_b32 s84, 0\n\t" \
    "s_mov_b32 s87, s80\n\t" \
    "s_mov_b64 s[90:91], s[72:73]\n\t" \
    "s_mov_b64 s[92:93], s[74:75]\n\t" \
    "s_sub_u32 s94, %[n], 1\n\t" \
    "s_sub_u32 s95, %[n], 4\n\t" \
    "s_sub_u32 s96, %[n], 3\n\t" \
    "v_mov_b32 v52, 0\n\t" \
    "v_mov_b32 v53, 0\n\t" \
    "s_waitcnt lgkmcnt(0)\n\t" \
    "s_barrier\n\t" \
    "ds_read_b128 a[172:175], v32 offset:0\n\t" \
    "ds_read_b128 a[176:179], v32 offset:6144\n\t" \
    "ds_read_b128 a[180:183], v33 offset:0\n\t" \
    "ds_read_b128 a[184:187], v33 offset:6144\n\t" \
    "ds_read_b128 a[188:191], v34 offset:0\n\t" \
    "ds_read_b128 a[192:195], v34 offset:6144\n\t" \
    "ds_read_b128 a[196:199], v35 offset:0\n\t" \
    "ds_read_b128 a[200:203], v35 offset:6144\n\t" \
    "ds_read_b128 a[204:207], v36 offset:0\n\t" \
    "ds_read_b128 a[208:211], v36 offset:6144\n\t" \
    "ds_read_b128 a[212:215], v37 offset:0\n\t" \
    "ds_read_b128 a[216:219], v37 offset:6144\n\t" \
    "s_waitcnt lgkmcnt(11)\n\t" \
    "v_mfma_f32_32x32x16_bf16 v[64:79], a[172:175], a[124:127], 0\n\t" \
    "v_accvgpr_write_b32 a28, 0\n\t" \
    "v_accvgpr_write_b32 a29, 0\n\t" \
    "v_accvgpr_write_b32 a30, 0\n\t" \
    "v_accvgpr_write_b32 a31, 0\n\t" \
    "v_mfma_f32_32x32x16_bf16 v[80:95], a[172:175], a[148:151], 0\n\t" \
    "v_accvgpr_write_b32 a32, 0\n\t" \
    "v_accvgpr_write_b32 a33, 0\n\t" \
    "v_accvgpr_write_b32 a34, 0\n\t" \
    "v_accvgpr_write_b32 a35, 0\n\t" \
    "s_waitcnt lgkmcnt(10)\n\t" \
    "v_mfma_f32_32x32x16_bf16 v[96:111], a[176:179], a[124:127], 0\n\t" \
    "ds_read_b128 a[172:175], v32 offset:12288\n\t" \
    "v_accvgpr_write_b32 a36, 0\n\t" \
    "v_accvgpr_write_b32 a37, 0\n\t" \
    "v_accvgpr_write_b32 a38, 0\n\t" \
    "v_accvgpr_write_b32 a39, 0\n\t" \
    "v_mfma_f32_32x32x16_bf16 v[112:127], a[176:179], a[148:151], 0\n\t" \
    "v_accvgpr_write_b32 a40, 0\n\t" \
    "v_accvgpr_write_b32 a41, 0\n\t" \
    "v_accvgpr_write_b32 a42, 0\n\t" \
    "v_accvgpr_write_b32 a43, 0\n\t" \
    "s_waitcnt lgkmcnt(10)\n\t" \
    "v_mfma_f32_32x32x16_bf16 v[64:79], a[180:183], a[128:131], v[64:79]\n\t" \
    "ds_read_b128 a[176:179], v32 offset:18432\n\t" \
    "v_accvgpr_write_b32 a44, 0\n\t" \
    "v_accvgpr_write_b32 a45, 0\n\t" \
    "v_accvgpr_write_b32 a46, 0\n\t" \
    "v_accvgpr_write_b32 a47, 0\n\t" \
    "v_mfma_f32_32x32x16_bf16 v[80:95], a[180:183], a[152:155], v[80:95]\n\t" \
    "v_accvgpr_write_b32 a48, 0\n\t" \
    "v_accvgpr_write_b32 a49, 0\n\t" \
    "v_accvgpr_write_b32 a50, 0\n\t" \
    "v_accvgpr_write_b32 a51, 0\n\t" \
    "s_waitcnt lgkmcnt(10)\n\t" \
    "v_mfma_f32_32x32x16_bf16 v[96:111], a[184:187], a[128:131], v[96:111]\n\t" \
    "ds_read_b128 a[180:183], v33 offset:12288\n\t" \
    "v_accvgpr_write_b32 a52, 0\n\t" \
    "v_accvgpr_write_b32 a53, 0\n\t" \
// ... 4571 lines not shown
    "v_exp_f32 v141, v141\n\t" \
    "v_add_f32 v46, v46, v154\n\t" \
    "v_add_f32 v47, v47, v155\n\t" \
    "v_cvt_pk_bf16_f32 v205, v154, v155\n\t" \
    "v_exp_f32 v156, v156\n\t" \
    "v_exp_f32 v157, v157\n\t" \
    "v_mfma_f32_32x32x16_bf16 a[92:107], a[236:239], v[188:191], a[92:107]\n\t" \
    "ds_read_b64_tr_b16 a[226:227], v41 offset:46080\n\t" \
    "v_add_f32 v44, v44, v140\n\t" \
    "v_add_f32 v45, v45, v141\n\t" \
    "v_cvt_pk_bf16_f32 v198, v140, v141\n\t" \
    "v_exp_f32 v142, v142\n\t" \
    "v_exp_f32 v143, v143\n\t" \
    "v_add_f32 v46, v46, v156\n\t" \
    "v_add_f32 v47, v47, v157\n\t" \
    "v_cvt_pk_bf16_f32 v206, v156, v157\n\t" \
    "v_mfma_f32_32x32x16_bf16 a[60:75], a[240:243], v[180:183], a[60:75]\n\t" \
    "ds_read_b64_tr_b16 a[228:229], v42 offset:46080\n\t" \
    "v_exp_f32 v158, v158\n\t" \
    "v_exp_f32 v159, v159\n\t" \
    "v_add_f32 v44, v44, v142\n\t" \
    "v_add_f32 v45, v45, v143\n\t" \
    "v_cvt_pk_bf16_f32 v199, v142, v143\n\t" \
    "v_add_f32 v46, v46, v158\n\t" \
    "v_add_f32 v47, v47, v159\n\t" \
    "v_cvt_pk_bf16_f32 v207, v158, v159\n\t" \
    "v_mfma_f32_32x32x16_bf16 a[108:123], a[240:243], v[188:191], a[108:123]\n\t" \
    "ds_read_b64_tr_b16 a[230:231], v43 offset:46080\n\t" \
    "s_waitcnt lgkmcnt(6)\n\t" \
    "v_mfma_f32_32x32x16_bf16 a[28:43], a[244:247], v[192:195], a[28:43]\n\t" \
    "v_mfma_f32_32x32x16_bf16 a[76:91], a[244:247], v[200:203], a[76:91]\n\t" \
    "v_mfma_f32_32x32x16_bf16 a[44:59], a[248:251], v[192:195], a[44:59]\n\t" \
    "v_mfma_f32_32x32x16_bf16 a[92:107], a[248:251], v[200:203], a[92:107]\n\t" \
    "v_mfma_f32_32x32x16_bf16 a[60:75], a[252:255], v[192:195], a[60:75]\n\t" \
    "v_mfma_f32_32x32x16_bf16 a[108:123], a[252:255], v[200:203], a[108:123]\n\t" \
    "s_waitcnt lgkmcnt(0)\n\t" \
    "v_mfma_f32_32x32x16_bf16 a[28:43], a[220:223], v[196:199], a[28:43]\n\t" \
    "v_mfma_f32_32x32x16_bf16 a[76:91], a[220:223], v[204:207], a[76:91]\n\t" \
    "v_mfma_f32_32x32x16_bf16 a[44:59], a[224:227], v[196:199], a[44:59]\n\t" \
    "v_mfma_f32_32x32x16_bf16 a[92:107], a[224:227], v[204:207], a[92:107]\n\t" \
    "v_mfma_f32_32x32x16_bf16 a[60:75], a[228:231], v[196:199], a[60:75]\n\t" \
    "v_mfma_f32_32x32x16_bf16 a[108:123], a[228:231], v[204:207], a[108:123]\n\t" \
    "s_nop 15\n\t" \
    "v_add_f32 v44, v44, v45\n\t" \
    "v_add_f32 v48, v48, v49\n\t" \
    "v_add_f32 v240, v44, v48\n\t" \
    "v_mov_b32 v242, v52\n\t" \
    "v_add_f32 v46, v46, v47\n\t" \
    "v_add_f32 v50, v50, v51\n\t" \
    "v_add_f32 v241, v46, v50\n\t" \
    "v_mov_b32 v243, v53\n\t" \
    "s_waitcnt lgkmcnt(0)\n\t" \
    "s_or_b32 s81, %[prof_lo], %[prof_hi]\n\t" \
    "s_cbranch_scc0 L_noph2_3_%=\n\t" \
    "s_memtime s[82:83]\n\t" \
    "s_waitcnt lgkmcnt(0)\n\t" \
    "s_mov_b64 exec, 1\n\t" \
    "v_mov_b32 v248, 0\n\t" \
    "v_mov_b32 v250, s82\n\t" \
    "v_mov_b32 v251, s83\n\t" \
    "global_store_dwordx2 v248, v[250:251], s[38:39] offset:24\n\t" \
    "s_mov_b64 exec, -1\n\t" \
    "L_noph2_3_%=:\n\t" \
    "s_add_u32 s81, s97, 1\n\t" \
    "s_cmp_ge_u32 s81, %[nit]\n\t" \
    "s_cbranch_scc1 L_last_%=\n\t" \
    "ds_read_b128 v[188:191], v25\n\t" \
    "ds_read_b128 v[192:195], v25 offset:16\n\t" \
    "ds_read_b128 v[196:199], v23 offset:32\n\t" \
    "ds_read_b128 v[200:203], v23 offset:48\n\t" \
    "ds_read_b128 v[204:207], v25 offset:3072\n\t" \
    "ds_read_b128 v[208:211], v25 offset:3088\n\t" \
    "ds_read_b128 v[212:215], v23 offset:3104\n\t" \
    "ds_read_b128 v[216:219], v23 offset:3120\n\t" \
    "v_mov_b32 v244, v240\n\t" \
    "v_mov_b32 v245, v241\n\t" \
    "s_add_u32 s24, %[qtb_lo], s52\n\t" \
    "s_nop 0\n\t" \
    "v_permlane32_swap_b32 v240, v244\n\t" \
    "s_addc_u32 s25, %[qtb_hi], 0\n\t" \
    "v_permlane32_swap_b32 v241, v245\n\t" \
    "v_add_f32 v222, v240, v244\n\t" \
    "s_add_u32 s24, s24, 0x00003000\n\t" \
    "v_add_f32 v223, v241, v245\n\t" \
    "v_div_scale_f32 v246, s[82:83], v222, v222, 1.0\n\t" \
    "s_addc_u32 s25, s25, 0\n\t" \
    "v_rcp_f32 v247, v246\n\t" \
    "v_div_scale_f32 v248, vcc, 1.0, v222, 1.0\n\t" \
    "s_add_u32 s26, s24, 0x00001000\n\t" \
    "v_fma_f32 v249, -v246, v247, 1.0\n\t" \
    "v_fmac_f32 v247, v249, v247\n\t" \
    "s_addc_u32 s27, s25, 0\n\t" \
    "v_mul_f32 v250, v248, v247\n\t" \
    "v_fma_f32 v251, -v246, v250, v248\n\t" \
    "s_add_u32 s28, s26, 0x00001000\n\t" \
    "v_fmac_f32 v250, v251, v247\n\t" \
    "v_fma_f32 v246, -v246, v250, v248\n\t" \
    "s_addc_u32 s29, s27, 0\n\t" \
    "v_div_fmas_f32 v246, v246, v247, v250\n\t" \
    "v_div_fixup_f32 v220, v246, v222, 1.0\n\t" \
    "global_load_dwordx4 a[124:127], v8, s[24:25]\n\t" \
    "v_log_f32 v252, v222\n\t" \
    "v_div_scale_f32 v246, s[82:83], v223, v223, 1.0\n\t" \
    "global_load_dwordx4 a[128:131], v8, s[24:25] offset:1024\n\t" \
    "v_rcp_f32 v247, v246\n\t" \
    "v_div_scale_f32 v248, vcc, 1.0, v223, 1.0\n\t" \
    "global_load_dwordx4 a[132:135], v8, s[24:25] offset:2048\n\t" \
    "v_fma_f32 v249, -v246, v247, 1.0\n\t" \
    "v_fmac_f32 v247, v249, v247\n\t" \
    "global_load_dwordx4 a[136:139], v8, s[24:25] offset:3072\n\t" \
    "v_mul_f32 v250, v248, v247\n\t" \
    "v_fma_f32 v251, -v246, v250, v248\n\t" \
    "global_load_dwordx4 a[140:143], v8, s[26:27]\n\t" \
    "v_fmac_f32 v250, v251, v247\n\t" \
    "v_fma_f32 v246, -v246, v250, v248\n\t" \
    "global_load_dwordx4 a[144:147], v8, s[26:27] offset:1024\n\t" \
// ... 459 lines not shown
    "s_mov_b64 exec, s[70:71]\n\t" \
    "v_mul_f32 v232, v173, v213\n\t" \
    "v_mul_f32 v233, v172, v213\n\t" \
    "v_fma_f32 v172, v172, v212, v232\n\t" \
    "v_fma_f32 v173, v173, v212, -v233\n\t" \
    "v_mul_f32 v234, v175, v215\n\t" \
    "v_mul_f32 v235, v174, v215\n\t" \
    "v_fma_f32 v174, v174, v214, v234\n\t" \
    "v_fma_f32 v175, v175, v214, -v235\n\t" \
    "v_mul_f32 v236, v177, v217\n\t" \
    "v_mul_f32 v237, v176, v217\n\t" \
    "v_fma_f32 v176, v176, v216, v236\n\t" \
    "v_fma_f32 v177, v177, v216, -v237\n\t" \
    "v_mul_f32 v238, v179, v219\n\t" \
    "v_mul_f32 v239, v178, v219\n\t" \
    "v_fma_f32 v178, v178, v218, v238\n\t" \
    "v_fma_f32 v179, v179, v218, -v239\n\t" \
    "s_mov_b64 exec, -1\n\t" \
    "v_cvt_pk_bf16_f32 v84, v172, v173\n\t" \
    "v_cvt_pk_bf16_f32 v85, v174, v175\n\t" \
    "v_cvt_pk_bf16_f32 v86, v176, v177\n\t" \
    "v_cvt_pk_bf16_f32 v87, v178, v179\n\t" \
    "ds_write_b128 v26, v[84:87] offset:128\n\t" \
    "v_cvt_pk_bf16_f32 v88, v180, v181\n\t" \
    "v_cvt_pk_bf16_f32 v89, v182, v183\n\t" \
    "v_cvt_pk_bf16_f32 v90, v184, v185\n\t" \
    "v_cvt_pk_bf16_f32 v91, v186, v187\n\t" \
    "ds_write_b128 v26, v[88:91] offset:144\n\t" \
    "ds_read_b128 v[140:143], v11\n\t" \
    "ds_read_b128 v[144:147], v12 offset:1040\n\t" \
    "ds_read_b128 v[148:151], v13 offset:2080\n\t" \
    "ds_read_b128 v[152:155], v11 offset:3328\n\t" \
    "ds_read_b128 v[156:159], v12 offset:4368\n\t" \
    "ds_read_b128 v[160:163], v13 offset:5408\n\t" \
    "s_waitcnt lgkmcnt(5)\n\t" \
    "global_store_dwordx4 v17, v[140:143], s[28:29]\n\t" \
    "s_waitcnt lgkmcnt(4)\n\t" \
    "global_store_dwordx4 v18, v[144:147], s[28:29]\n\t" \
    "s_waitcnt lgkmcnt(3)\n\t" \
    "global_store_dwordx4 v19, v[148:151], s[28:29]\n\t" \
    "s_waitcnt lgkmcnt(2)\n\t" \
    "global_store_dwordx4 v17, v[152:155], s[30:31]\n\t" \
    "s_waitcnt lgkmcnt(1)\n\t" \
    "global_store_dwordx4 v18, v[156:159], s[30:31]\n\t" \
    "s_waitcnt lgkmcnt(0)\n\t" \
    "global_store_dwordx4 v19, v[160:163], s[30:31]\n\t" \
    "s_mov_b64 exec, 0xffffffff\n\t" \
    "global_store_dword v27, v252, s[46:47]\n\t" \
    "global_store_dword v27, v253, s[46:47] offset:128\n\t" \
    "s_mov_b64 exec, -1\n\t" \
    "s_waitcnt lgkmcnt(0)\n\t" \
    "s_waitcnt lgkmcnt(0)\n\t" \
    "s_or_b32 s81, %[prof_lo], %[prof_hi]\n\t" \
    "s_cbranch_scc0 L_noph3_4_%=\n\t" \
    "s_memtime s[98:99]\n\t" \
    "s_waitcnt lgkmcnt(0)\n\t" \
    "L_noph3_4_%=:\n\t" \
    "s_mov_b64 s[40:41], s[56:57]\n\t" \
    "s_mov_b64 s[42:43], s[58:59]\n\t" \
    "s_mov_b64 s[44:45], s[60:61]\n\t" \
    "s_mov_b64 s[46:47], s[62:63]\n\t" \
    "s_mov_b64 s[48:49], s[64:65]\n\t" \
    "s_mov_b64 s[50:51], s[66:67]\n\t" \
    "s_mov_b64 s[52:53], s[68:69]\n\t" \
    "s_add_u32 s97, s97, 1\n\t" \
    "s_add_u32 s35, s35, 64\n\t" \
    "v_mov_b32 v28, s35\n\t" \
    "ds_read_b128 v[244:247], v28 offset:64\n\t" \
    "ds_read_b128 v[248:251], v28 offset:80\n\t" \
    "ds_read_b128 v[252:255], v28 offset:96\n\t" \
    "ds_read_b32 v31, v28 offset:112\n\t" \
    "ds_read_b32 v22, v28 offset:116\n\t" \
    "s_waitcnt lgkmcnt(0)\n\t" \
    "v_readfirstlane_b32 s56, v244\n\t" \
    "v_readfirstlane_b32 s57, v245\n\t" \
    "v_readfirstlane_b32 s58, v246\n\t" \
    "v_readfirstlane_b32 s59, v247\n\t" \
    "v_readfirstlane_b32 s60, v248\n\t" \
    "v_readfirstlane_b32 s61, v249\n\t" \
    "v_readfirstlane_b32 s62, v250\n\t" \
    "v_readfirstlane_b32 s63, v251\n\t" \
    "v_readfirstlane_b32 s64, v252\n\t" \
    "v_readfirstlane_b32 s65, v253\n\t" \
    "v_readfirstlane_b32 s66, v254\n\t" \
    "v_readfirstlane_b32 s67, v255\n\t" \
    "v_readfirstlane_b32 s68, v31\n\t" \
    "v_readfirstlane_b32 s69, v22\n\t" \
    "s_branch L_item_%=\n\t" \
    "L_last_%=:\n\t" \
    "ds_read_b128 v[188:191], v25\n\t" \
    "ds_read_b128 v[192:195], v25 offset:16\n\t" \
    "ds_read_b128 v[196:199], v23 offset:32\n\t" \
    "ds_read_b128 v[200:203], v23 offset:48\n\t" \
    "ds_read_b128 v[204:207], v25 offset:3072\n\t" \
    "ds_read_b128 v[208:211], v25 offset:3088\n\t" \
    "ds_read_b128 v[212:215], v23 offset:3104\n\t" \
    "ds_read_b128 v[216:219], v23 offset:3120\n\t" \
    "v_mov_b32 v244, v240\n\t" \
    "v_mov_b32 v245, v241\n\t" \
    "s_nop 0\n\t" \
    "v_permlane32_swap_b32 v240, v244\n\t" \
    "v_permlane32_swap_b32 v241, v245\n\t" \
    "v_add_f32 v222, v240, v244\n\t" \
    "v_add_f32 v223, v241, v245\n\t" \
    "s_add_u32 s24, %[qtb_lo], s52\n\t" \
    "v_div_scale_f32 v246, s[82:83], v222, v222, 1.0\n\t" \
    "v_rcp_f32 v247, v246\n\t" \
    "v_div_scale_f32 v248, vcc, 1.0, v222, 1.0\n\t" \
    "v_fma_f32 v249, -v246, v247, 1.0\n\t" \
    "v_fmac_f32 v247, v249, v247\n\t" \
// ... 442 lines not shown
    "s_mov_b64 exec, s[70:71]\n\t" \
    "v_mul_f32 v232, v173, v213\n\t" \
    "v_mul_f32 v233, v172, v213\n\t" \
    "v_fma_f32 v172, v172, v212, v232\n\t" \
    "v_fma_f32 v173, v173, v212, -v233\n\t" \
    "v_mul_f32 v234, v175, v215\n\t" \
    "v_mul_f32 v235, v174, v215\n\t" \
    "v_fma_f32 v174, v174, v214, v234\n\t" \
    "v_fma_f32 v175, v175, v214, -v235\n\t" \
    "v_mul_f32 v236, v177, v217\n\t" \
    "v_mul_f32 v237, v176, v217\n\t" \
    "v_fma_f32 v176, v176, v216, v236\n\t" \
    "v_fma_f32 v177, v177, v216, -v237\n\t" \
    "v_mul_f32 v238, v179, v219\n\t" \
    "v_mul_f32 v239, v178, v219\n\t" \
    "v_fma_f32 v178, v178, v218, v238\n\t" \
    "v_fma_f32 v179, v179, v218, -v239\n\t" \
    "s_mov_b64 exec, -1\n\t" \
    "v_cvt_pk_bf16_f32 v84, v172, v173\n\t" \
    "v_cvt_pk_bf16_f32 v85, v174, v175\n\t" \
    "v_cvt_pk_bf16_f32 v86, v176, v177\n\t" \
    "v_cvt_pk_bf16_f32 v87, v178, v179\n\t" \
    "ds_write_b128 v26, v[84:87] offset:128\n\t" \
    "v_cvt_pk_bf16_f32 v88, v180, v181\n\t" \
    "v_cvt_pk_bf16_f32 v89, v182, v183\n\t" \
    "v_cvt_pk_bf16_f32 v90, v184, v185\n\t" \
    "v_cvt_pk_bf16_f32 v91, v186, v187\n\t" \
    "ds_write_b128 v26, v[88:91] offset:144\n\t" \
    "ds_read_b128 v[140:143], v11\n\t" \
    "ds_read_b128 v[144:147], v12 offset:1040\n\t" \
    "ds_read_b128 v[148:151], v13 offset:2080\n\t" \
    "ds_read_b128 v[152:155], v11 offset:3328\n\t" \
    "ds_read_b128 v[156:159], v12 offset:4368\n\t" \
    "ds_read_b128 v[160:163], v13 offset:5408\n\t" \
    "s_waitcnt lgkmcnt(5)\n\t" \
    "global_store_dwordx4 v17, v[140:143], s[28:29]\n\t" \
    "s_waitcnt lgkmcnt(4)\n\t" \
    "global_store_dwordx4 v18, v[144:147], s[28:29]\n\t" \
    "s_waitcnt lgkmcnt(3)\n\t" \
    "global_store_dwordx4 v19, v[148:151], s[28:29]\n\t" \
    "s_waitcnt lgkmcnt(2)\n\t" \
    "global_store_dwordx4 v17, v[152:155], s[30:31]\n\t" \
    "s_waitcnt lgkmcnt(1)\n\t" \
    "global_store_dwordx4 v18, v[156:159], s[30:31]\n\t" \
    "s_waitcnt lgkmcnt(0)\n\t" \
    "global_store_dwordx4 v19, v[160:163], s[30:31]\n\t" \
    "s_mov_b64 exec, 0xffffffff\n\t" \
    "global_store_dword v27, v252, s[46:47]\n\t" \
    "global_store_dword v27, v253, s[46:47] offset:128\n\t" \
    "s_mov_b64 exec, -1\n\t" \
    "s_waitcnt lgkmcnt(0)\n\t" \
    "s_waitcnt lgkmcnt(0)\n\t" \
    "s_or_b32 s81, %[prof_lo], %[prof_hi]\n\t" \
    "s_cbranch_scc0 L_noph3_5_%=\n\t" \
    "s_memtime s[98:99]\n\t" \
    "s_waitcnt lgkmcnt(0)\n\t" \
    "L_noph3_5_%=:\n\t" \
    "s_or_b32 s81, %[prof_lo], %[prof_hi]\n\t" \
    "s_cbranch_scc0 L_nostamp_end_%=\n\t" \
    "s_memtime s[20:21]\n\t" \
    "s_memrealtime s[22:23]\n\t" \
    "s_waitcnt lgkmcnt(0)\n\t" \
    "s_mov_b64 exec, 1\n\t" \
    "v_mov_b32 v248, 0\n\t" \
    "v_mov_b32 v244, s20\n\t" \
    "v_mov_b32 v245, s21\n\t" \
    "v_mov_b32 v246, s22\n\t" \
    "v_mov_b32 v247, s23\n\t" \
    "global_store_dwordx2 v248, v[244:245], s[36:37] offset:32\n\t" \
    "global_store_dwordx2 v248, v[246:247], s[36:37] offset:48\n\t" \
    "v_mov_b32 v250, s98\n\t" \
    "v_mov_b32 v251, s99\n\t" \
    "global_store_dwordx2 v248, v[250:251], s[36:37] offset:56\n\t" \
    "s_mov_b64 exec, -1\n\t" \
    "L_nostamp_end_%=:\n\t" \
    "s_waitcnt vmcnt(0)\n\t" \
    ""
#endif
#define GTA_ATTN64_ITEMS_CLOBBERS \
    "v8", "v9", "v10", "v11", "v12", "v13", "v14", "v15", "v16", "v17", "v18", "v19", "v20", "v21", "v22", "v23", "v24", "v25", "v26", "v27", "v28", "v29", "v30", "v31", "v32", "v33", "v34", "v35", "v36", "v37", "v38", "v39", "v40", "v41", "v42", "v43", "v44", "v45", "v46", "v47", "v48", "v49", "v50", "v51", "v52", "v53", "v54", "v55", "v56", "v57", "v58", "v59", "v60", "v61", "v62", "v63", "v64", "v65", "v66", "v67", "v68", "v69", "v70", "v71", "v72", "v73", "v74", "v75", "v76", "v77", "v78", "v79", "v80", "v81", "v82", "v83", "v84", "v85", "v86", "v87", "v88", "v89", "v90", "v91", "v92", "v93", "v94", "v95", "v96", "v97", "v98", "v99", "v100", "v101", "v102", "v103", "v104", "v105", "v106", "v107", "v108", "v109", "v110", "v111", "v112", "v113", "v114", "v115", "v116", "v117", "v118", "v119", "v120", "v121", "v122", "v123", "v124", "v125", "v126", "v127", "v128", "v129", "v130", "v131", "v132", "v133", "v134", "v135", "v136", "v137", "v138", "v139", "v140", "v141", "v142", "v143", "v144", "v145", "v146", "v147", "v148", "v149", "v150", "v151", "v152", "v153", "v154", "v155", "v156", "v157", "v158", "v159", "v160", "v161", "v162", "v163", "v164", "v165", "v166", "v167", "v168", "v169", "v170", "v171", "v172", "v173", "v174", "v175", "v176", "v177", "v178", "v179", "v180", "v181", "v182", "v183", "v184", "v185", "v186", "v187", "v188", "v189", "v190", "v191", "v192", "v193", "v194", "v195", "v196", "v197", "v198", "v199", "v200", "v201", "v202", "v203", "v204", "v205", "v206", "v207", "v208", "v209", "v210", "v211", "v212", "v213", "v214", "v215", "v216", "v217", "v218", "v219", "v220", "v221", "v222", "v223", "v224", "v225", "v226", "v227", "v228", "v229", "v230", "v231", "v232", "v233", "v234", "v235", "v236", "v237", "v238", "v239", "v240", "v241", "v242", "v243", "v244", "v245", "v246", "v247", "v248", "v249", "v250", "v251", "v252", "v253", "v254", "v255", "a0", "a1", "a2", "a3", "a4", "a5", "a6", "a7", "a8", "a9", "a10", "a11", "a12", "a13", "a14", "a15", "a16", "a17", "a18", "a19", "a20", "a21", "a22", "a23", "a24", "a25", "a26", "a27", "a28", "a29", "a30", "a31", "a32", "a33", "a34", "a35", "a36", "a37", "a38", "a39", "a40", "a41", "a42", "a43", "a44", "a45", "a46", "a47", "a48", "a49", "a50", "a51", "a52", "a53", "a54", "a55", "a56", "a57", "a58", "a59", "a60", "a61", "a62", "a63", "a64", "a65", "a66", "a67", "a68", "a69", "a70", "a71", "a72", "a73", "a74", "a75", "a76", "a77", "a78", "a79", "a80", "a81", "a82", "a83", "a84", "a85", "a86", "a87", "a88", "a89", "a90", "a91", "a92", "a93", "a94", "a95", "a96", "a97", "a98", "a99", "a100", "a101", "a102", "a103", "a104", "a105", "a106", "a107", "a108", "a109", "a110", "a111", "a112", "a113", "a114", "a115", "a116", "a117", "a118", "a119", "a120", "a121", "a122", "a123", "a124", "a125", "a126", "a127", "a128", "a129", "a130", "a131", "a132", "a133", "a134", "a135", "a136", "a137", "a138", "a139", "a140", "a141", "a142", "a143", "a144", "a145", "a146", "a147", "a148", "a149", "a150", "a151", "a152", "a153", "a154", "a155", "a156", "a157", "a158", "a159", "a160", "a161", "a162", "a163", "a164", "a165", "a166", "a167", "a168", "a169", "a170", "a171", "a172", "a173", "a174", "a175", "a176", "a177", "a178", "a179", "a180", "a181", "a182", "a183", "a184", "a185", "a186", "a187", "a188", "a189", "a190", "a191", "a192", "a193", "a194", "a195", "a196", "a197", "a198", "a199", "a200", "a201", "a202", "a203", "a204", "a205", "a206", "a207", "a208", "a209", "a210", "a211", "a212", "a213", "a214", "a215", "a216", "a217", "a218", "a219", "a220", "a221", "a222", "a223", "a224", "a225", "a226", "a227", "a228", "a229", "a230", "a231", "a232", "a233", "a234", "a235", "a236", "a237", "a238", "a239", "a240", "a241", "a242", "a243", "a244", "a245", "a246", "a247", "a248", "a249", "a250", "a251", "a252", "a253", "a254", "a255", "s20", "s21", "s22", "s23", "s24", "s25", "s26", "s27", "s28", "s29", "s30", "s31", "s33", "s34", "s35", "s36", "s37", "s38", "s39", "s40", "s41", "s42", "s43", "s44", "s45", "s46", "s47", "s48", "s49", "s50", "s51", "s52", "s53", "s54", "s55", "s56", "s57", "s58", "s59", "s60", "s61", "s62", "s63", "s64", "s65", "s66", "s67", "s68", "s69", "s70", "s71", "s72", "s73", "s74", "s75", "s76", "s77", "s78", "s79", "s80", "s81", "s82", "s83", "s84", "s85", "s86", "s87", "s88", "s89", "s90", "s91", "s92", "s93", "s94", "s95", "s96", "s97", "s98", "s99", "m0", "vcc", "scc", "memory"
```

gta_amd/csrc/gta_fwd64.hip:

```cpp
#include <atomic>
#include <cstdlib>
#include <hip/hip_ext.h>
#include "gta_flash_common.h"
#define GTA_ASM_M0_BEGIN _Pragma("clang diagnostic push") _Pragma("clang diagnostic ignored \"-Winline-asm\"")
#define GTA_ASM_M0_END _Pragma("clang diagnostic pop")
#ifdef GTA_ATTN64_DEV
#define GTA_ATTN64_DIAG
#include "build_var/gta_attn64_dev.inc"
#else
#include "gta_attn64_loop.inc"
#endif
#include "gta_attn64_items.inc"

extern thread_local void* gta_dbg_fwd_ev_start;
extern thread_local void* gta_dbg_fwd_ev_stop;

namespace {

constexpr int A64_BM = 256;
constexpr int A64_LDS_MAX = 160 * 1024;
__host__ __device__ constexpr bool a64_ks_so2(int layout, int ks) {
    const uint32_t d0 = gta_layout_desc(layout, 2 * ks), d1 = gta_layout_desc(layout, 2 * ks + 1);
    return (!(d0 & GTA_CHUNK_SO3) && ((d0 & 3u) == GTA_HALF_SO2 || ((d0 >> 2) & 3u) == GTA_HALF_SO2)) ||
           (!(d1 & GTA_CHUNK_SO3) && ((d1 & 3u) == GTA_HALF_SO2 || ((d1 >> 2) & 3u) == GTA_HALF_SO2));
// ... 643 lines not shown
                    if (xo && GTA_DL(kp)) chunk_apply<true, 1>(GTA_DL(kp), rec_o + GTA_QREC_O, rec_o + GTA_QREC_D1T, rec_o + GTA_QREC_D2T, ocs[rb][kp], x);
                    if constexpr (COAL && LAYOUT != GTA_LAYOUT_MS) *reinterpret_cast<u32x4_t*>(xw + l31 * A::XROW + GTA_CE(kp) * 16) = pack8(x[0]);
                    else gstore_chunk2<ESZ>(orow + GTA_CE(kp) * 8 * ESZ, 0, x[0]);
                }
            });
            if constexpr (COAL && LAYOUT != GTA_LAYOUT_MS) {
                const unsigned rowb = (unsigned)pp->o_st * 2u;
                char* ob = (char*)pp->o + ((long)b * pp->o_sb + (long)h * pp->o_sh + (long)(q0 + wave * 64 + rb * 32) * pp->o_st) * 2;
                const unsigned xo_ = ((unsigned)lane >> 3) * A::XROW + ((unsigned)lane & 7u) * 16u, go_ = ((unsigned)lane >> 3) * rowb + ((unsigned)lane & 7u) * 16u;
#pragma unroll
                for (int i = 0; i < KS; ++i) {
                    const u32x4_t w = *reinterpret_cast<const u32x4_t*>(xw + 8 * i * A::XROW + xo_);
                    *reinterpret_cast<u32x4_t*>(ob + (unsigned long)(8u * i * rowb) + go_) = w;
                }
            }
        });
    };
    if constexpr (!RHO_MFMA) {
        if constexpr (COAL) o_items(std::true_type{});
        else if (fast) o_items(std::true_type{}); else o_items(std::false_type{});
    } else if (emf) {
        o_block_mfma(std::integral_constant<int, 0>{}, ct);
        if (ev1 == ev0) {
            o_block_mfma(std::integral_constant<int, 1>{}, ct);
        } else {
            u32x4_t ct1[12];
            const char* tp = tile_ptr(b, ev1, 1) + lane * 16;
#pragma unroll
            for (int i = 0; i < 12; ++i) ct1[i] = *reinterpret_cast<const u32x4_t*>(tp + i * GTA_QT_BYTES);
            o_block_mfma(std::integral_constant<int, 1>{}, ct1);
        }
    } else {
        if (fast) o_items(std::true_type{}); else o_items(std::false_type{});
    }
#undef GTA_CE
    }
    GTA_STAMP(V, 4); GTA_STAMPR(V, 6);
    par ^= 1;
    }
#undef GTA_STAMP
#undef GTA_STAMP_ON
#undef GTA_STAMPR
#undef GTA_DL
#undef GTA_DESC
}

static_assert(GTA_ITEM64_OFF_CS == A64<96, GTA_LAYOUT_MS>::OFF_CS && GTA_ITEM64_OFF_X == A64<96, GTA_LAYOUT_MS>::off_x(0, true) &&
              GTA_ITEM64_OFF_ITEMS == A64<96, GTA_LAYOUT_MS>::lds(0, true) && GTA_ITEM64_LDS_BYTES <= A64_LDS_MAX,
              "gen_item64.py's LDS map is A64<96, MS>'s with coalesced item I/O and no view records");

template <int PAD4>
__global__ __launch_bounds__(256, 1) void gta_attn64_items_kernel(const GtaFwdParams p_kernarg) {
    using A = A64<96, GTA_LAYOUT_MS>;
    constexpr int CHP = A::CHP, KS = A::KS, DB = A::DB, R = A::R;
    extern __shared__ __attribute__((aligned(16))) char smem[];
    const GtaFwdParams* const pp = &p_kernarg;
    const int tid = threadIdx.x;
    const int wave = __builtin_amdgcn_readfirstlane(tid >> 6);
    const int n_items = pp->n_items, G = gridDim.x;
    const int n_tiles = (pp->Tk + BN - 1) / BN;
    const int woff = wave * (A::IMG / 4);
    auto img_of = [&](int V) -> const char* {
        const int bh = view_of(item_of64(V, n_items), pp->n_qtiles, pp->inv_nqt);
        return (const char*)pp->kp + (long)bh * n_tiles * (long)A::TILE;
    };
    if (pp->prof != nullptr && tid == 0) {
        unsigned long long* row = reinterpret_cast<unsigned long long*>(pp->prof) + 8l * blockIdx.x;
        row[1] = __builtin_readcyclecounter();
        row[2] = __builtin_amdgcn_s_memrealtime();
    }
    {
        const int lane = tid & 63;
        uint32_t* tab = reinterpret_cast<uint32_t*>(smem + A::OFF_TAB);
#pragma unroll
        for (int ks = 0; ks < KS; ++ks) tab[ks * 64 + lane] = ((lane & 31) * CHP + swz<CHP>(lane & 31, 2 * ks + (lane >> 5))) * 16;
        const int g16 = lane >> 4, p16 = lane & 15;
#pragma unroll
        for (int d = 0; d < DB; ++d) {
            const int u = 4 * d + 2 * (g16 & 1) + ((p16 & 3) >> 1);
            const int hb = (p16 & 1) * 8;
#pragma unroll
            for (int hf = 0; hf < 2; ++hf) {
                const int r = 4 * (lane >> 5) + (p16 >> 2) + 8 * hf;
                tab[(KS + 2 * d + hf) * 64 + lane] = (r * CHP + swz<CHP>(r, u)) * 16 + hb + A::OFF_V;
            }
        }
        const unsigned voff16 = (unsigned)lane * 16u;
        const char* img = img_of(blockIdx.x) + woff;
#pragma unroll
        for (int t = 0; t < R; ++t) dma_group<A::NP>(lds_addr(smem + A::OFF_K + t * A::IMG) + woff, img + (long)t * A::TILE, voff16);
#pragma unroll
        for (int t = 0; t < R - 1; ++t) dma_group<A::NP>(lds_addr(smem + A::OFF_V + t * A::IMG) + woff, img + (long)t * A::TILE + A::IMG, voff16);
    }
    const int n_mine = (n_items - (int)blockIdx.x + G - 1) / G;
    const int tailj = (pp->Tk & (BN - 1)) ? n_tiles - 1 : -1;
    for (int k0 = 0; k0 < n_mine; k0 += GTA_ITEM64_MAX_ITEMS) {
        const int nit = n_mine - k0 < GTA_ITEM64_MAX_ITEMS ? n_mine - k0 : GTA_ITEM64_MAX_ITEMS;
        if (tid < nit + 2) {
            int k = k0 + tid;
            k = k < n_mine ? k : n_mine - 1;
            const int V = (int)blockIdx.x + k * G;
            const int w = item_of64(V, n_items);
            const int bh = view_of(w, pp->n_qtiles, pp->inv_nqt), qt = w - bh * pp->n_qtiles;
            const int b = view_of(bh, pp->H, pp->invH), h = bh - b * pp->H, q0 = qt * A64_BM;
            const int view = view_of(q0, pp->Pq, pp->invPq);
            uint32_t* d = reinterpret_cast<uint32_t*>(smem + GTA_ITEM64_OFF_ITEMS + tid * GTA_ITEM64_ITEM_BYTES);
            auto put = [&](int i, const void* ptr) { d[i] = (uint32_t)(uintptr_t)ptr; d[i + 1] = (uint32_t)((uintptr_t)ptr >> 32); };
            put(GTA_ITEM64_D_Q, (const char*)pp->q + ((long)b * pp->q_sb + (long)h * pp->q_sh + (long)q0 * pp->q_st) * 2);
            put(GTA_ITEM64_D_O, (const char*)pp->o + ((long)b * pp->o_sb + (long)h * pp->o_sh + (long)q0 * pp->o_st) * 2);
            put(GTA_ITEM64_D_CS, pp->cs_q + ((long)b * pp->Tq + q0) * (A::CS_ROW / 4));
            put(GTA_ITEM64_D_LSE, pp->lse + ((long)b * pp->H + h) * pp->Tq + q0);
            put(GTA_ITEM64_D_IMG, (const char*)pp->kp + (long)bh * n_tiles * (long)A::TILE);
            put(GTA_ITEM64_D_KN, pp->kn + (long)bh * n_tiles);
            d[GTA_ITEM64_D_AQ] = (uint32_t)((b * pp->Nq + view) * (GTA_QT_TILES * GTA_QT_BYTES));
            d[GTA_ITEM64_D_V] = (uint32_t)V;
        }
        asm volatile("s_waitcnt lgkmcnt(0)" ::: "memory");
        __builtin_amdgcn_s_barrier();
        {
            const uint32_t tabl = lds_addr(smem + GTA_ITEM64_OFF_ITEMS);
            const uint32_t qrb = (uint32_t)pp->q_st * 2u, orb = (uint32_t)pp->o_st * 2u;
            const uint32_t qtb_lo = (uint32_t)(uintptr_t)pp->qtiles, qtb_hi = (uint32_t)((uintptr_t)pp->qtiles >> 32);
            const uint32_t prof_lo = (uint32_t)(uintptr_t)pp->prof, prof_hi = (uint32_t)((uintptr_t)pp->prof >> 32);
            const int Tk = pp->Tk;
#define A64_ITEMS(TEXT) do { GTA_ASM_M0_BEGIN asm volatile(TEXT \
                         : \
                         : [tabl] "s"(tabl), [nit] "s"(nit), [wave] "s"(wave), [qrb] "s"(qrb), [orb] "s"(orb), [qtb_lo] "s"(qtb_lo), [qtb_hi] "s"(qtb_hi), \
                           [prof_lo] "s"(prof_lo), [prof_hi] "s"(prof_hi), [n] "s"(n_tiles), [tailj] "s"(tailj), [Tk] "s"(Tk) \
                         : GTA_ATTN64_ITEMS_CLOBBERS); GTA_ASM_M0_END } while (0)
            if constexpr (PAD4 == 0) A64_ITEMS(GTA_ATTN64_ITEMS);
#ifdef GTA_ATTN64_DIAG
            else if constexpr (PAD4 == 1) A64_ITEMS(GTA_ATTN64_ITEMS_P4);
            else A64_ITEMS(GTA_ATTN64_ITEMS_PH);
#endif
#undef A64_ITEMS
        }
        __builtin_amdgcn_s_barrier();
    }
}

inline bool attn64_coal_ms(const GtaFwdParams& pl) {
    using A = A64<96, GTA_LAYOUT_MS>;
    return pl.Tq % A64_BM == 0 && pl.cs_q != nullptr && pl.nso2 * 8 == A::CS_ROW && A::lds(pl.vrep_q ? pl.nrec : 0, true) <= A64_LDS_MAX;
}
inline bool attn64_coal_so2(const GtaFwdParams& pl) {
    using A = A64<64, GTA_LAYOUT_SO2>;
    return pl.Tq % A64_BM == 0 && pl.cs_q != nullptr && pl.dh == 64 && pl.nso2 * 8 == A::CS_ROW && A::lds(0, true) <= A64_LDS_MAX &&
           pl.q_st * 2L * A64_BM < (1L << 31) && pl.o_st * 2L * A64_BM < (1L << 31) && !(pl.flags & GTA_FLAG_ITEM_CXX) &&
           (((uintptr_t)pl.cs_q | (uintptr_t)pl.q | (uintptr_t)pl.o) & 15) == 0 && ((pl.q_st | pl.o_st) & 7) == 0;
}
inline bool attn64_items_takes(const GtaFwdParams& p, bool coal) {
    return coal && p.qtiles != nullptr && p.vrep_q != nullptr && (p.flags & GTA_FLAG_V_TRANSFORM) && !(p.flags & GTA_FLAG_ITEM_CXX) &&
           p.Pq % A64_BM == 0 && p.lse != nullptr && p.kn != nullptr && p.q_st * 2L * A64_BM < (1L << 31) && p.o_st * 2L * A64_BM < (1L << 31) &&
           (long)p.B * p.Nq * (GTA_QT_TILES * GTA_QT_BYTES) < (1L << 31) &&
           (((uintptr_t)p.cs_q | (uintptr_t)p.qtiles | (uintptr_t)p.kp) & 15) == 0 && (((uintptr_t)p.lse | (uintptr_t)p.kn) & 3) == 0;
}

GtaFwdParams attn64_params(const GtaFwdParams& p) {
    GtaFwdParams pl = p;
    pl.n_qtiles = (p.Tq + A64_BM - 1) / A64_BM;
    pl.n_items = p.B * p.H * pl.n_qtiles;
    pl.nrec = !p.vrep_q ? 0 : A64_BM / p.Pq + 2 < p.Nq ? A64_BM / p.Pq + 2 : p.Nq;
    pl.per_cu = 1;
    pl.inv_nqt = 1.0f / (float)pl.n_qtiles;
    pl.invH = 1.0f / (float)p.H;
    return pl;
}

template <int PAD4>
int launch_attn64_items_pad(const GtaFwdParams& pl, long grid, hipStream_t stream) {
    if (int rc = gta_lds_optin<&gta_attn64_items_kernel<PAD4>>(A64_LDS_MAX)) return rc;
    hipEvent_t e0 = (hipEvent_t)gta_dbg_fwd_ev_start, e1 = (hipEvent_t)gta_dbg_fwd_ev_stop;
    if (e0 && e1) {
        gta_dbg_fwd_ev_start = gta_dbg_fwd_ev_stop = nullptr;
        hipExtLaunchKernelGGL(gta_attn64_items_kernel<PAD4>, dim3((unsigned)grid), dim3(256), GTA_ITEM64_LDS_BYTES, stream, e0, e1, 0, pl);
    } else {
        hipLaunchKernelGGL(gta_attn64_items_kernel<PAD4>, dim3((unsigned)grid), dim3(256), GTA_ITEM64_LDS_BYTES, stream, pl);
    }
    return hipGetLastError() == hipSuccess ? GTA_OK : GTA_E_LAUNCH;
}
int launch_attn64_items(const GtaFwdParams& pl, long grid, hipStream_t stream) {
// ... 161 lines not shown
```

Measured before the change: 208.7 Mtokens/s.

## Move first K/V ring fill into asm prologue with partial vmcnt waits

The initial LDS-DMA fill of the K/V ring (seven images) moves out of the C++ prologue into the generated asm item loop, issued after the item's Q/descriptor requests. The first item then waits only for part of the fill (vmcnt(21), then vmcnt(12) before the tile loop) instead of draining everything, so Q staging and descriptor work can overlap the ring load. The simulator and checker gain matching first-fill ordering checks. This only affects kernel startup per block, so the gain is limited to prologue latency, and it adds risk of subtle ordering bugs.

After: 208.3 Mtokens/s. About the same (-0.2%).

```diff
diff --git a/gta_amd/csrc/gen_attn64.py b/gta_amd/csrc/gen_attn64.py
--- a/gta_amd/csrc/gen_attn64.py
+++ b/gta_amd/csrc/gen_attn64.py
@@ -696,8 +696,9 @@
 
 
 class Sim:
-    def __init__(self, gen, prog, n_tiles, rebase_at=(), has_tail=False, items=2, first_rebase=True):
+    def __init__(self, gen, prog, n_tiles, rebase_at=(), has_tail=False, items=2, first_rebase=True, first_fill=None):
         self.g, self.prog, self.n, self.rebase_at, self.has_tail, self.items = gen, prog, n_tiles, set(rebase_at), has_tail, items
+        self.first_fill = first_fill
         self.first_rebase = first_rebase or not gen.first_fast
         self.labels = {ins.label: i for i, ins in enumerate(prog) if ins.kind == "label"}
         self.count = 0
@@ -713,12 +714,9 @@
         self.got = {}
         self.hist = []
         stats = {"instr": 0, "mfma": 0}
-        for t in range(R):
+        for ring, t in self.first_fill or [("K", t) for t in range(R)] + [("V", t) for t in range(R - 1)]:
             for i in range(NP):
-                self.vmq.append(("K", t % R, i, (0, t)))
-        for t in range(R - 1):
-            for i in range(NP):
-                self.vmq.append(("V", t % R, i, (0, t)))
+                self.vmq.append((ring, t % R, i, (0, t)))
         kptr, vptr = (0, R), (0, R - 1)
         for item in range(self.items):
             kptr, vptr = self.run_item(item, kptr, vptr, stats)
@@ -739,6 +737,9 @@
         pending_regs = set()
         sc = {}
         self.pending_tile = getattr(self, "pending_tile", {})
+        if self.first_fill is not None and item > 0:
+            while self.vmq:
+                self.land(self.vmq.pop(0))
         msver = [0, 0]
         o_done = {(rb, d): set() for rb in range(RB) for d in range(DB)}
         l_done = {rb: set() for rb in range(RB)}
@@ -804,10 +805,11 @@
                         (self.kslot if key[0] == "K" else self.vslot)[key[1]] = tile
                         del self.pending_tile[key]
             elif op == "item_begin":
-                for t in range(R):
+                counted = self.first_fill is not None and item == 0
+                for t in range(2 if counted else R):
                     if self.kslot[t] != (item, t):
                         self.fail(f"item {item}: K slot {t} holds {self.kslot[t]} at item begin")
-                for t in range(R - 1):
+                for t in range(0 if counted else R - 1):
                     if self.vslot[t] != (item, t):
                         self.fail(f"item {item}: V slot {t} holds {self.vslot[t]} at item begin")
             elif op == "j0":
diff --git a/gta_amd/csrc/gen_item64.py b/gta_amd/csrc/gen_item64.py
--- a/gta_amd/csrc/gen_item64.py
+++ b/gta_amd/csrc/gen_item64.py
@@ -5,7 +5,7 @@
 
 import gen_attn64 as G
 from isa_model import (LANES, Asm, CheckError, Ins, Wave, as_u32, assemble_check, auto_waits, bf16_rne, bf16_to_f32, check_wait_states, clobber_list,
-                       regs, rtext, u2f, write_macro)
+                       regs, rtext, u2f, wait, write_macro)
 
 KS, DB, RB, R = 6, 3, 2, 4
 IMG = 64 * 12 * 16
@@ -22,6 +22,9 @@
 QT_BYTES = 1024
 LN2_BITS, QN_BITS = 0x3f317218, 0x3f808659
 assert LDS_BYTES <= 160 * 1024 and OFF_ITEMS % 16 == 0
+PIECES = IMG // 4096
+FILL_PIECES = (2 * R - 1) * PIECES
+HEAD_VM = (2 * R - 1 - 3) * PIECES
 
 D_Q, D_O, D_CS, D_LSE, D_IMG, D_KN, D_AQ, D_V = 0, 2, 4, 6, 8, 10, 12, 13
 D_WORDS = 14
@@ -76,7 +79,7 @@
 LOOP_OPERANDS = {"%[kptr]": rtext(S_KPTR), "%[vptr]": rtext(S_VPTR), "%[nxt_k]": rtext(S_NXK), "%[nxt_v]": rtext(S_NXV),
                  "%[woff]": S_WOFF, "%[lane16]": V_LANE16, "%[qn0]": V_QN[0], "%[qn1]": V_QN[1], "%[kn]": V_KN,
                  "%[lr0]": V_LR[0], "%[lr1]": V_LR[1], "%[mr0]": V_MR[0], "%[mr1]": V_MR[1]}
-OPERANDS = ("tabl", "nit", "wave", "qrb", "orb", "qtb_lo", "qtb_hi", "prof_lo", "prof_hi", "n", "tailj", "Tk")
+OPERANDS = ("tabl", "nit", "wave", "qrb", "orb", "qtb_lo", "qtb_hi", "prof_lo", "prof_hi", "n", "tailj", "Tk", "first")
 
 
 def cur(d, k=2):
@@ -165,6 +168,10 @@
         self.read_desc(a, 0)
         self.request(a)
         self.cs_dma(a)
+        a.s_cmp("eq", "u32", "%[first]", 0)
+        a.branch("s_cbranch_scc1", "L_ring_kept_%=")
+        self.first_fill(a)
+        a.label("L_ring_kept_%=")
         self.advance_desc(a)
         a.v_mbcnt_lane(lane)
         a.v_and_b32(l31, 31, lane)
@@ -192,7 +199,31 @@
         a.waitcnt(lgkm=0)
         self.read_desc(a, 1)
         self.stamp_row(a, S_PREV)
+        a.s_cmp("eq", "u32", "%[first]", 0)
+        a.branch("s_cbranch_scc1", "L_chunk_next_%=")
+        a.waitcnt(vm=FILL_PIECES)
+        self.stamp(a, "first")
+        self.phase(a, 0)
+        a.branch("s_branch", "L_item_body_%=")
+        a.nop(1)
+        a.label("L_chunk_next_%=")
         a.waitcnt(vm=0)
+
+    def first_fill(self, a):
+        ptr = S_B[0]
+        a.s_add_u32(ptr[0], nxt(D_IMG)[0], S_WOFF)
+        a.s_addc_u32(ptr[1], nxt(D_IMG)[1], 0)
+        for i in range(2 * R - 1):
+            t, is_v = i >> 1, i & 1
+            dst = (OFF_V if is_v else OFF_K) + t * IMG
+            a.add(f"s_add_u32 m0, {S_WOFF}, {dst}", "salu", [S_WOFF], ["m0", "scc"], ("s_add_m0", S_WOFF, dst))
+            a.nop(1)
+            for p in range(IMG // 4096):
+                a.add(f"global_load_lds_dwordx4 {V_LANE16}, {rtext(ptr)}" + (f" offset:{1024 * p}" if p else ""), "dma",
+                      ["m0", V_LANE16] + ptr, [], ("global_load_lds", V_LANE16, ptr, 1024 * p))
+            if i < 2 * R - 2:
+                a.s_add_u32(ptr[0], ptr[0], IMG)
+                a.s_addc_u32(ptr[1], ptr[1], 0)
 
     def read_desc(self, a, entry):
         t = TMPX
@@ -286,6 +317,7 @@
         PK = V(222, 8)
         a.waitcnt(vm=14)
         self.phase(a, 0)
+        a.label("L_item_body_%=")
         for rb in range(RB):
             for i in range(KS):
                 a.ds_write(128, V_XL[i % 3], QL[rb * KS + i], row0(i) * XROW)
@@ -532,6 +564,8 @@
                 continue
             if head_vm and ins.kind == "wait" and ins.fx == ("waitcnt", 0, None):
                 head_vm = False
+                assert out[-1].kind == "wait" and out[-1].fx == ("waitcnt", None, 0)
+                out[-1] = wait(vm=HEAD_VM, lgkm=0)
                 continue
             out.append(ins.bound(LOOP_OPERANDS))
         return gen, out
@@ -646,6 +680,7 @@
             cs = np.stack([np.cos(ang), np.sin(ang)], -1).astype(np.float32)
         self.cs = cs
         self.lse = np.zeros((B, H, Tq), np.float32)
+        self.img = np.random.default_rng(seed + 1000).integers(0, 256, size=B * H * n_tiles * TILE, dtype=np.uint8)
         self.kn = rng.uniform(0.5, 2.0, size=(B, H, 64)).astype(np.float32)
         self.Mf, self.Mi, tiles = [], [], []
         for v in range(B * Nq):
@@ -747,7 +782,14 @@
         return rows, lse
 
 
-def run_case(prog, case, wave, prof=False):
+def ring_quarter(case, item, wave):
+    it = case.items[item]
+    img = (it["b"] * case.H + it["h"]) * case.n_tiles * TILE + wave * (IMG // 4)
+    out = [(OFF_K + t * IMG + wave * (IMG // 4), case.img[img + t * TILE:img + t * TILE + IMG // 4]) for t in range(R)]
+    return out + [(OFF_V + t * IMG + wave * (IMG // 4), case.img[img + t * TILE + IMG:img + t * TILE + IMG + IMG // 4]) for t in range(R - 1)]
+
+
+def run_case(prog, case, wave, prof=False, first=1, snapshot=None):
     LDS0 = np.zeros(160 * 1024, np.uint8)
     n = case.n_items
     for k in range(n + 2):
@@ -758,14 +800,14 @@
     inputs = {"%[tabl]": OFF_ITEMS, "%[nit]": n, "%[wave]": wave, "%[qrb]": case.q_st * 2, "%[orb]": case.o_st * 2,
               "%[qtb_lo]": case.A_QT & 0xffffffff, "%[qtb_hi]": case.A_QT >> 32,
               "%[prof_lo]": (case.A_PROF & 0xffffffff) if prof else 0, "%[prof_hi]": (case.A_PROF >> 32) if prof else 0,
-              "%[n]": case.n_tiles, "%[tailj]": 0xffffffff, "%[Tk]": 64 * case.n_tiles}
+              "%[n]": case.n_tiles, "%[tailj]": 0xffffffff, "%[Tk]": 64 * case.n_tiles, "%[first]": first}
     w = Wave(inputs=inputs, seed=wave + 11)
     w.lds[:] = LDS0
     qb = case.qbits.reshape(-1).view(np.uint8)
     ob = case.obits.reshape(-1).view(np.uint8)
     profb = np.zeros(64 * 64, np.uint8)
     for base, arr in ((case.A_Q, qb), (case.A_O, ob), (case.A_CS, case.cs.reshape(-1).view(np.uint8)), (case.A_LSE, case.lse.reshape(-1).view(np.uint8)),
-                      (case.A_KN, case.kn.reshape(-1).view(np.uint8)), (case.A_QT, case.tiles), (case.A_PROF, profb)):
+                      (case.A_KN, case.kn.reshape(-1).view(np.uint8)), (case.A_QT, case.tiles), (case.A_IMG, case.img), (case.A_PROF, profb)):
         w.map_buffer(base, arr)
     state = {"item": 0}
     tol = 0.0 if case.exact else 2.0 ** -7
@@ -781,7 +823,19 @@
     def loop_hook(wv):
         k = state["item"]
         it = case.items[k]
+        if k == 0:
+            n_dma = sum(isinstance(e, dict) for e in wv.vm)
+            if n_dma != (FILL_PIECES if first else 0) or any(e for e in wv.vm if not isinstance(e, dict)):
+                raise CheckError(f"wave {wave}: {n_dma} LDS-DMA pieces in flight at the first item's tile loop, expected the first fill's {FILL_PIECES if first else 0}")
+            wv.wait(HEAD_VM, None)
+            for off, want in ring_quarter(case, 0, wave)[:2] + ring_quarter(case, 0, wave)[R:R + 1]:
+                if first and not (wv.lds[off:off + IMG // 4] == want).all():
+                    raise CheckError(f"wave {wave}: the tile at LDS {off} has not landed behind the head's wait of the first item's tile loop")
         wv.wait(0, None)
+        if k == 0:
+            for off, want in ring_quarter(case, 0, wave):
+                if not (wv.lds[off:off + IMG // 4] == (want if first else 0)).all():
+                    raise CheckError(f"wave {wave}: ring at LDS {off}: " + ("the first fill left other bytes than the tile's" if first else "a later chunk touched the ring"))
         exp = case.expect_q(k, wave)
         for rb in range(RB):
             for ks in range(KS):
@@ -816,6 +870,8 @@
         for i, r in enumerate(G.KOFF + [G.VOFF[d][h] for d in range(DB) for h in range(2)]):
             if not (wv.v[wv.ridx(r)] == (np.arange(64) + 64 * i) * 4 + 0x100000).all():
                 raise CheckError(f"the loop's LDS offset register {r} does not hold table row {i}")
+        if snapshot is not None:
+            snapshot(wv, k)
         junk = np.random.default_rng(5).integers(0x7f800001, 0x7fffffff, size=(208, LANES), dtype=np.uint32)
         wv.v[32 + 12:240] = junk[:196]
         wv.v[256 + 124:512] = np.random.default_rng(6).integers(0x7f800001, 0x7fffffff, size=(132, LANES), dtype=np.uint32)
@@ -881,7 +937,20 @@
             run_case(prog, case, wave, prof=(seed == 2 and wave == 1))
         if verbose:
             print(f"  ok: case seed {seed}: {n_items} items, {'exact' if exact else 'random'} inputs, waves {list(waves)}")
+    case = Case(4, 2, False)
+    for wave in waves[:2]:
+        run_case(prog, case, wave, first=0)
+    check_ring(gen, verbose)
     return stats
+
+
+def check_ring(gen, verbose=False):
+    g, loop = gen.loop_program()
+    order = [("V" if i & 1 else "K", i >> 1) for i in range(2 * R - 1)]
+    for n, reb, tail in ((R, (), False), (2 * R, (), False), (5 * R, (), False), (2 * R, (1,), False), (3 * R, (2, 5, 2 * R + 1), True), (R, (), True)):
+        G.Sim(g, loop, n, reb, tail, first_fill=order).run()
+        if verbose:
+            print(f"  ok: ring protocol behind the first fill: n_tiles {n}, rebase at {reb}, tail {tail}")
 
 
 def emit(path, prog, prog_p4=None, prog_ph=None):
diff --git a/gta_amd/csrc/gta_attn64_items.inc b/gta_amd/csrc/gta_attn64_items.inc
--- a/gta_amd/csrc/gta_attn64_items.inc
+++ b/gta_amd/csrc/gta_attn64_items.inc
@@ -150,6 +150,58 @@
     "s_nop 0\n\t" \
     "global_load_lds_dwordx4 v21, s[60:61]\n\t" \
     "global_load_lds_dwordx4 v21, s[60:61] offset:1024\n\t" \
+    "s_cmp_eq_u32 %[first], 0\n\t" \
+    "s_cbranch_scc1 L_ring_kept_%=\n\t" \
+    "s_add_u32 s24, s64, s80\n\t" \
+    "s_addc_u32 s25, s65, 0\n\t" \
+    "s_add_u32 m0, s80, 0\n\t" \
+    "s_nop 0\n\t" \
+    "global_load_lds_dwordx4 v8, s[24:25]\n\t" \
+    "global_load_lds_dwordx4 v8, s[24:25] offset:1024\n\t" \
+    "global_load_lds_dwordx4 v8, s[24:25] offset:2048\n\t" \
+    "s_add_u32 s24, s24, 0x00003000\n\t" \
+    "s_addc_u32 s25, s25, 0\n\t" \
+    "s_add_u32 m0, s80, 49152\n\t" \
+    "s_nop 0\n\t" \
+    "global_load_lds_dwordx4 v8, s[24:25]\n\t" \
+    "global_load_lds_dwordx4 v8, s[24:25] offset:1024\n\t" \
+    "global_load_lds_dwordx4 v8, s[24:25] offset:2048\n\t" \
+    "s_add_u32 s24, s24, 0x00003000\n\t" \
+    "s_addc_u32 s25, s25, 0\n\t" \
+    "s_add_u32 m0, s80, 12288\n\t" \
+    "s_nop 0\n\t" \
+    "global_load_lds_dwordx4 v8, s[24:25]\n\t" \
+    "global_load_lds_dwordx4 v8, s[24:25] offset:1024\n\t" \
+    "global_load_lds_dwordx4 v8, s[24:25] offset:2048\n\t" \
+    "s_add_u32 s24, s24, 0x00003000\n\t" \
+    "s_addc_u32 s25, s25, 0\n\t" \
+    "s_add_u32 m0, s80, 61440\n\t" \
+    "s_nop 0\n\t" \
+    "global_load_lds_dwordx4 v8, s[24:25]\n\t" \
+    "global_load_lds_dwordx4 v8, s[24:25] offset:1024\n\t" \
+    "global_load_lds_dwordx4 v8, s[24:25] offset:2048\n\t" \
+    "s_add_u32 s24, s24, 0x00003000\n\t" \
+    "s_addc_u32 s25, s25, 0\n\t" \
+    "s_add_u32 m0, s80, 24576\n\t" \
+    "s_nop 0\n\t" \
+    "global_load_lds_dwordx4 v8, s[24:25]\n\t" \
+    "global_load_lds_dwordx4 v8, s[24:25] offset:1024\n\t" \
+    "global_load_lds_dwordx4 v8, s[24:25] offset:2048\n\t" \
+    "s_add_u32 s24, s24, 0x00003000\n\t" \
+    "s_addc_u32 s25, s25, 0\n\t" \
+    "s_add_u32 m0, s80, 73728\n\t" \
+    "s_nop 0\n\t" \
+    "global_load_lds_dwordx4 v8, s[24:25]\n\t" \
+    "global_load_lds_dwordx4 v8, s[24:25] offset:1024\n\t" \
+    "global_load_lds_dwordx4 v8, s[24:25] offset:2048\n\t" \
+    "s_add_u32 s24, s24, 0x00003000\n\t" \
+    "s_addc_u32 s25, s25, 0\n\t" \
+    "s_add_u32 m0, s80, 36864\n\t" \
+    "s_nop 0\n\t" \
+    "global_load_lds_dwordx4 v8, s[24:25]\n\t" \
+    "global_load_lds_dwordx4 v8, s[24:25] offset:1024\n\t" \
+    "global_load_lds_dwordx4 v8, s[24:25] offset:2048\n\t" \
+    "L_ring_kept_%=:\n\t" \
     "s_mov_b64 s[40:41], s[56:57]\n\t" \
     "s_mov_b64 s[42:43], s[58:59]\n\t" \
     "s_mov_b64 s[44:45], s[60:61]\n\t" \
@@ -216,6 +268,33 @@
     "s_lshl_b32 s81, s53, 6\n\t" \
     "s_add_u32 s36, %[prof_lo], s81\n\t" \
     "s_addc_u32 s37, %[prof_hi], 0\n\t" \
+    "s_cmp_eq_u32 %[first], 0\n\t" \
+    "s_cbranch_scc1 L_chunk_next_%=\n\t" \
+    "s_waitcnt vmcnt(21)\n\t" \
+    "s_or_b32 s81, %[prof_lo], %[prof_hi]\n\t" \
+    "s_cbranch_scc0 L_nostamp_first_%=\n\t" \
+    "s_memtime s[20:21]\n\t" \
+    "s_memrealtime s[22:23]\n\t" \
+    "s_waitcnt lgkmcnt(0)\n\t" \
+    "s_lshl_b32 s81, s53, 6\n\t" \
+    "s_add_u32 s38, %[prof_lo], s81\n\t" \
+    "s_addc_u32 s39, %[prof_hi], 0\n\t" \
+    "s_mov_b64 exec, 1\n\t" \
+    "v_mov_b32 v248, 0\n\t" \
+    "v_mov_b32 v244, s20\n\t" \
+    "v_mov_b32 v245, s21\n\t" \
+    "v_mov_b32 v246, s22\n\t" \
+    "v_mov_b32 v247, s23\n\t" \
+    "global_store_dwordx2 v248, v[244:245], s[36:37] offset:32\n\t" \
+    "global_store_dwordx2 v248, v[246:247], s[36:37] offset:48\n\t" \
+    "global_store_dwordx2 v248, v[244:245], s[38:39]\n\t" \
+    "global_store_dwordx2 v248, v[246:247], s[38:39] offset:40\n\t" \
+    "s_mov_b64 s[36:37], s[38:39]\n\t" \
+    "s_mov_b64 exec, -1\n\t" \
+    "L_nostamp_first_%=:\n\t" \
+    "s_branch L_item_body_%=\n\t" \
+    "s_nop 0\n\t" \
+    "L_chunk_next_%=:\n\t" \
     "s_waitcnt vmcnt(0)\n\t" \
     "L_item_%=:\n\t" \
     "s_or_b32 s81, %[prof_lo], %[prof_hi]\n\t" \
@@ -240,6 +319,7 @@
     "s_mov_b64 exec, -1\n\t" \
     "L_nostamp_item_%=:\n\t" \
     "s_waitcnt vmcnt(14)\n\t" \
+    "L_item_body_%=:\n\t" \
     "ds_write_b128 v11, a[220:223]\n\t" \
     "ds_write_b128 v12, a[224:227] offset:1040\n\t" \
     "ds_write_b128 v13, a[228:231] offset:2080\n\t" \
@@ -604,7 +684,7 @@
     "s_sub_u32 s96, %[n], 3\n\t" \
     "v_mov_b32 v52, 0\n\t" \
     "v_mov_b32 v53, 0\n\t" \
-    "s_waitcnt lgkmcnt(0)\n\t" \
+    "s_waitcnt vmcnt(12) lgkmcnt(0)\n\t" \
     "s_barrier\n\t" \
     "ds_read_b128 a[172:175], v32 offset:0\n\t" \
     "ds_read_b128 a[176:179], v32 offset:6144\n\t" \
@@ -6545,6 +6625,58 @@
     "s_nop 0\n\t" \
     "global_load_lds_dwordx4 v21, s[60:61]\n\t" \
     "global_load_lds_dwordx4 v21, s[60:61] offset:1024\n\t" \
+    "s_cmp_eq_u32 %[first], 0\n\t" \
+    "s_cbranch_scc1 L_ring_kept_%=\n\t" \
+    "s_add_u32 s24, s64, s80\n\t" \
+    "s_addc_u32 s25, s65, 0\n\t" \
+    "s_add_u32 m0, s80, 0\n\t" \
+    "s_nop 0\n\t" \
+    "global_load_lds_dwordx4 v8, s[24:25]\n\t" \
+    "global_load_lds_dwordx4 v8, s[24:25] offset:1024\n\t" \
+    "global_load_lds_dwordx4 v8, s[24:25] offset:2048\n\t" \
+    "s_add_u32 s24, s24, 0x00003000\n\t" \
+    "s_addc_u32 s25, s25, 0\n\t" \
+    "s_add_u32 m0, s80, 49152\n\t" \
+    "s_nop 0\n\t" \
+    "global_load_lds_dwordx4 v8, s[24:25]\n\t" \
+    "global_load_lds_dwordx4 v8, s[24:25] offset:1024\n\t" \
+    "global_load_lds_dwordx4 v8, s[24:25] offset:2048\n\t" \
+    "s_add_u32 s24, s24, 0x00003000\n\t" \
+    "s_addc_u32 s25, s25, 0\n\t" \
+    "s_add_u32 m0, s80, 12288\n\t" \
+    "s_nop 0\n\t" \
+    "global_load_lds_dwordx4 v8, s[24:25]\n\t" \
+    "global_load_lds_dwordx4 v8, s[24:25] offset:1024\n\t" \
+    "global_load_lds_dwordx4 v8, s[24:25] offset:2048\n\t" \
+    "s_add_u32 s24, s24, 0x00003000\n\t" \
+    "s_addc_u32 s25, s25, 0\n\t" \
+    "s_add_u32 m0, s80, 61440\n\t" \
+    "s_nop 0\n\t" \
+    "global_load_lds_dwordx4 v8, s[24:25]\n\t" \
+    "global_load_lds_dwordx4 v8, s[24:25] offset:1024\n\t" \
+    "global_load_lds_dwordx4 v8, s[24:25] offset:2048\n\t" \
+    "s_add_u32 s24, s24, 0x00003000\n\t" \
+    "s_addc_u32 s25, s25, 0\n\t" \
+    "s_add_u32 m0, s80, 24576\n\t" \
+    "s_nop 0\n\t" \
+    "global_load_lds_dwordx4 v8, s[24:25]\n\t" \
+    "global_load_lds_dwordx4 v8, s[24:25] offset:1024\n\t" \
+    "global_load_lds_dwordx4 v8, s[24:25] offset:2048\n\t" \
+    "s_add_u32 s24, s24, 0x00003000\n\t" \
+    "s_addc_u32 s25, s25, 0\n\t" \
+    "s_add_u32 m0, s80, 73728\n\t" \
+    "s_nop 0\n\t" \
+    "global_load_lds_dwordx4 v8, s[24:25]\n\t" \
+    "global_load_lds_dwordx4 v8, s[24:25] offset:1024\n\t" \
+    "global_load_lds_dwordx4 v8, s[24:25] offset:2048\n\t" \
+    "s_add_u32 s24, s24, 0x00003000\n\t" \
+    "s_addc_u32 s25, s25, 0\n\t" \
+    "s_add_u32 m0, s80, 36864\n\t" \
+    "s_nop 0\n\t" \
+    "global_load_lds_dwordx4 v8, s[24:25]\n\t" \
+    "global_load_lds_dwordx4 v8, s[24:25] offset:1024\n\t" \
+    "global_load_lds_dwordx4 v8, s[24:25] offset:2048\n\t" \
+    "L_ring_kept_%=:\n\t" \
     "s_mov_b64 s[40:41], s[56:57]\n\t" \
     "s_mov_b64 s[42:43], s[58:59]\n\t" \
     "s_mov_b64 s[44:45], s[60:61]\n\t" \
@@ -6611,6 +6743,33 @@
     "s_lshl_b32 s81, s53, 6\n\t" \
     "s_add_u32 s36, %[prof_lo], s81\n\t" \
     "s_addc_u32 s37, %[prof_hi], 0\n\t" \
+    "s_cmp_eq_u32 %[first], 0\n\t" \
+    "s_cbranch_scc1 L_chunk_next_%=\n\t" \
+    "s_waitcnt vmcnt(21)\n\t" \
+    "s_or_b32 s81, %[prof_lo], %[prof_hi]\n\t" \
+    "s_cbranch_scc0 L_nostamp_first_%=\n\t" \
+    "s_memtime s[20:21]\n\t" \
+    "s_memrealtime s[22:23]\n\t" \
+    "s_waitcnt lgkmcnt(0)\n\t" \
+    "s_lshl_b32 s81, s53, 6\n\t" \
+    "s_add_u32 s38, %[prof_lo], s81\n\t" \
+    "s_addc_u32 s39, %[prof_hi], 0\n\t" \
+    "s_mov_b64 exec, 1\n\t" \
+    "v_mov_b32 v248, 0\n\t" \
+    "v_mov_b32 v244, s20\n\t" \
+    "v_mov_b32 v245, s21\n\t" \
+    "v_mov_b32 v246, s22\n\t" \
+    "v_mov_b32 v247, s23\n\t" \
+    "global_store_dwordx2 v248, v[244:245], s[36:37] offset:32\n\t" \
+    "global_store_dwordx2 v248, v[246:247], s[36:37] offset:48\n\t" \
+    "global_store_dwordx2 v248, v[244:245], s[38:39]\n\t" \
+    "global_store_dwordx2 v248, v[246:247], s[38:39] offset:40\n\t" \
+    "s_mov_b64 s[36:37], s[38:39]\n\t" \
+    "s_mov_b64 exec, -1\n\t" \
+    "L_nostamp_first_%=:\n\t" \
+    "s_branch L_item_body_%=\n\t" \
+    "s_nop 0\n\t" \
+    "L_chunk_next_%=:\n\t" \
     "s_waitcnt vmcnt(0)\n\t" \
     "L_item_%=:\n\t" \
     "s_or_b32 s81, %[prof_lo], %[prof_hi]\n\t" \
@@ -6635,6 +6794,7 @@
     "s_mov_b64 exec, -1\n\t" \
     "L_nostamp_item_%=:\n\t" \
     "s_waitcnt vmcnt(14)\n\t" \
+    "L_item_body_%=:\n\t" \
     "ds_write_b128 v11, a[220:223]\n\t" \
     "ds_write_b128 v12, a[224:227] offset:1040\n\t" \
     "ds_write_b128 v13, a[228:231] offset:2080\n\t" \
@@ -7000,7 +7160,7 @@
     "s_sub_u32 s96, %[n], 3\n\t" \
     "v_mov_b32 v52, 0\n\t" \
     "v_mov_b32 v53, 0\n\t" \
-    "s_waitcnt lgkmcnt(0)\n\t" \
+    "s_waitcnt vmcnt(12) lgkmcnt(0)\n\t" \
     "s_barrier\n\t" \
     "ds_read_b128 a[172:175], v32 offset:0\n\t" \
     "ds_read_b128 a[176:179], v32 offset:6144\n\t" \
@@ -12941,6 +13101,58 @@
     "s_nop 0\n\t" \
     "global_load_lds_dwordx4 v21, s[60:61]\n\t" \
     "global_load_lds_dwordx4 v21, s[60:61] offset:1024\n\t" \
+    "s_cmp_eq_u32 %[first], 0\n\t" \
+    "s_cbranch_scc1 L_ring_kept_%=\n\t" \
+    "s_add_u32 s24, s64, s80\n\t" \
+    "s_addc_u32 s25, s65, 0\n\t" \
+    "s_add_u32 m0, s80, 0\n\t" \
+    "s_nop 0\n\t" \
+    "global_load_lds_dwordx4 v8, s[24:25]\n\t" \
+    "global_load_lds_dwordx4 v8, s[24:25] offset:1024\n\t" \
+    "global_load_lds_dwordx4 v8, s[24:25] offset:2048\n\t" \
+    "s_add_u32 s24, s24, 0x00003000\n\t" \
+    "s_addc_u32 s25, s25, 0\n\t" \
+    "s_add_u32 m0, s80, 49152\n\t" \
+    "s_nop 0\n\t" \
+    "global_load_lds_dwordx4 v8, s[24:25]\n\t" \
+    "global_load_lds_dwordx4 v8, s[24:25] offset:1024\n\t" \
+    "global_load_lds_dwordx4 v8, s[24:25] offset:2048\n\t" \
+    "s_add_u32 s24, s24, 0x00003000\n\t" \
+    "s_addc_u32 s25, s25, 0\n\t" \
+    "s_add_u32 m0, s80, 12288\n\t" \
+    "s_nop 0\n\t" \
+    "global_load_lds_dwordx4 v8, s[24:25]\n\t" \
+    "global_load_lds_dwordx4 v8, s[24:25] offset:1024\n\t" \
+    "global_load_lds_dwordx4 v8, s[24:25] offset:2048\n\t" \
+    "s_add_u32 s24, s24, 0x00003000\n\t" \
+    "s_addc_u32 s25, s25, 0\n\t" \
+    "s_add_u32 m0, s80, 61440\n\t" \
+    "s_nop 0\n\t" \
+    "global_load_lds_dwordx4 v8, s[24:25]\n\t" \
+    "global_load_lds_dwordx4 v8, s[24:25] offset:1024\n\t" \
+    "global_load_lds_dwordx4 v8, s[24:25] offset:2048\n\t" \
+    "s_add_u32 s24, s24, 0x00003000\n\t" \
+    "s_addc_u32 s25, s25, 0\n\t" \
+    "s_add_u32 m0, s80, 24576\n\t" \
+    "s_nop 0\n\t" \
+    "global_load_lds_dwordx4 v8, s[24:25]\n\t" \
+    "global_load_lds_dwordx4 v8, s[24:25] offset:1024\n\t" \
+    "global_load_lds_dwordx4 v8, s[24:25] offset:2048\n\t" \
+    "s_add_u32 s24, s24, 0x00003000\n\t" \
+    "s_addc_u32 s25, s25, 0\n\t" \
+    "s_add_u32 m0, s80, 73728\n\t" \
+    "s_nop 0\n\t" \
+    "global_load_lds_dwordx4 v8, s[24:25]\n\t" \
+    "global_load_lds_dwordx4 v8, s[24:25] offset:1024\n\t" \
+    "global_load_lds_dwordx4 v8, s[24:25] offset:2048\n\t" \
+    "s_add_u32 s24, s24, 0x00003000\n\t" \
+    "s_addc_u32 s25, s25, 0\n\t" \
+    "s_add_u32 m0, s80, 36864\n\t" \
+    "s_nop 0\n\t" \
+    "global_load_lds_dwordx4 v8, s[24:25]\n\t" \
+    "global_load_lds_dwordx4 v8, s[24:25] offset:1024\n\t" \
+    "global_load_lds_dwordx4 v8, s[24:25] offset:2048\n\t" \
+    "L_ring_kept_%=:\n\t" \
     "s_mov_b64 s[40:41], s[56:57]\n\t" \
     "s_mov_b64 s[42:43], s[58:59]\n\t" \
     "s_mov_b64 s[44:45], s[60:61]\n\t" \
@@ -13007,6 +13219,48 @@
     "s_lshl_b32 s81, s53, 6\n\t" \
     "s_add_u32 s36, %[prof_lo], s81\n\t" \
     "s_addc_u32 s37, %[prof_hi], 0\n\t" \
+    "s_cmp_eq_u32 %[first], 0\n\t" \
+    "s_cbranch_scc1 L_chunk_next_%=\n\t" \
+    "s_waitcnt vmcnt(21)\n\t" \
+    "s_or_b32 s81, %[prof_lo], %[prof_hi]\n\t" \
+    "s_cbranch_scc0 L_nostamp_first_%=\n\t" \
+    "s_memtime s[20:21]\n\t" \
+    "s_memrealtime s[22:23]\n\t" \
+    "s_waitcnt lgkmcnt(0)\n\t" \
+    "s_lshl_b32 s81, s53, 6\n\t" \
+    "s_add_u32 s38, %[prof_lo], s81\n\t" \
+    "s_addc_u32 s39, %[prof_hi], 0\n\t" \
+    "s_mov_b64 exec, 1\n\t" \
+    "v_mov_b32 v248, 0\n\t" \
+    "v_mov_b32 v244, s20\n\t" \
+    "v_mov_b32 v245, s21\n\t" \
+    "v_mov_b32 v246, s22\n\t" \
+    "v_mov_b32 v247, s23\n\t" \
+    "global_store_dwordx2 v248, v[244:245], s[36:37] offset:32\n\t" \
+    "global_store_dwordx2 v248, v[246:247], s[36:37] offset:48\n\t" \
+    "v_mov_b32 v250, s98\n\t" \
+    "v_mov_b32 v251, s99\n\t" \
+    "global_store_dwordx2 v248, v[250:251], s[36:37] offset:56\n\t" \
+    "global_store_dwordx2 v248, v[244:245], s[38:39]\n\t" \
+    "global_store_dwordx2 v248, v[246:247], s[38:39] offset:40\n\t" \
+    "s_mov_b64 s[36:37], s[38:39]\n\t" \
+    "s_mov_b64 exec, -1\n\t" \
+    "L_nostamp_first_%=:\n\t" \
+    "s_waitcnt lgkmcnt(0)\n\t" \
+    "s_or_b32 s81, %[prof_lo], %[prof_hi]\n\t" \
+    "s_cbranch_scc0 L_noph0_1_%=\n\t" \
+    "s_memtime s[82:83]\n\t" \
+    "s_waitcnt lgkmcnt(0)\n\t" \
+    "s_mov_b64 exec, 1\n\t" \
+    "v_mov_b32 v248, 0\n\t" \
+    "v_mov_b32 v250, s82\n\t" \
+    "v_mov_b32 v251, s83\n\t" \
+    "global_store_dwordx2 v248, v[250:251], s[38:39] offset:8\n\t" \
+    "s_mov_b64 exec, -1\n\t" \
+    "L_noph0_1_%=:\n\t" \
+    "s_branch L_item_body_%=\n\t" \
+    "s_nop 0\n\t" \
+    "L_chunk_next_%=:\n\t" \
     "s_waitcnt vmcnt(0)\n\t" \
     "L_item_%=:\n\t" \
     "s_or_b32 s81, %[prof_lo], %[prof_hi]\n\t" \
@@ -13036,7 +13290,7 @@
     "s_waitcnt vmcnt(14)\n\t" \
     "s_waitcnt lgkmcnt(0)\n\t" \
     "s_or_b32 s81, %[prof_lo], %[prof_hi]\n\t" \
-    "s_cbranch_scc0 L_noph0_1_%=\n\t" \
+    "s_cbranch_scc0 L_noph0_2_%=\n\t" \
     "s_memtime s[82:83]\n\t" \
     "s_waitcnt lgkmcnt(0)\n\t" \
     "s_mov_b64 exec, 1\n\t" \
@@ -13045,7 +13299,8 @@
     "v_mov_b32 v251, s83\n\t" \
     "global_store_dwordx2 v248, v[250:251], s[38:39] offset:8\n\t" \
     "s_mov_b64 exec, -1\n\t" \
-    "L_noph0_1_%=:\n\t" \
+    "L_noph0_2_%=:\n\t" \
+    "L_item_body_%=:\n\t" \
     "ds_write_b128 v11, a[220:223]\n\t" \
     "ds_write_b128 v12, a[224:227] offset:1040\n\t" \
     "ds_write_b128 v13, a[228:231] offset:2080\n\t" \
@@ -13403,7 +13658,7 @@
     "s_waitcnt lgkmcnt(0)\n\t" \
     "s_waitcnt lgkmcnt(0)\n\t" \
     "s_or_b32 s81, %[prof_lo], %[prof_hi]\n\t" \
-    "s_cbranch_scc0 L_noph1_2_%=\n\t" \
+    "s_cbranch_scc0 L_noph1_3_%=\n\t" \
     "s_memtime s[82:83]\n\t" \
     "s_waitcnt lgkmcnt(0)\n\t" \
     "s_mov_b64 exec, 1\n\t" \
@@ -13412,7 +13667,7 @@
     "v_mov_b32 v251, s83\n\t" \
     "global_store_dwordx2 v248, v[250:251], s[38:39] offset:16\n\t" \
     "s_mov_b64 exec, -1\n\t" \
-    "L_noph1_2_%=:\n\t" \
+    "L_noph1_3_%=:\n\t" \
     "s_mov_b32 s84, 0\n\t" \
     "s_mov_b32 s87, s80\n\t" \
     "s_mov_b64 s[90:91], s[72:73]\n\t" \
@@ -13422,7 +13677,7 @@
     "s_sub_u32 s96, %[n], 3\n\t" \
     "v_mov_b32 v52, 0\n\t" \
     "v_mov_b32 v53, 0\n\t" \
-    "s_waitcnt lgkmcnt(0)\n\t" \
+    "s_waitcnt vmcnt(12) lgkmcnt(0)\n\t" \
     "s_barrier\n\t" \
     "ds_read_b128 a[172:175], v32 offset:0\n\t" \
     "ds_read_b128 a[176:179], v32 offset:6144\n\t" \
@@ -18100,7 +18355,7 @@
     "v_mov_b32 v243, v53\n\t" \
     "s_waitcnt lgkmcnt(0)\n\t" \
     "s_or_b32 s81, %[prof_lo], %[prof_hi]\n\t" \
-    "s_cbranch_scc0 L_noph2_3_%=\n\t" \
+    "s_cbranch_scc0 L_noph2_4_%=\n\t" \
     "s_memtime s[82:83]\n\t" \
     "s_waitcnt lgkmcnt(0)\n\t" \
     "s_mov_b64 exec, 1\n\t" \
@@ -18109,7 +18364,7 @@
     "v_mov_b32 v251, s83\n\t" \
     "global_store_dwordx2 v248, v[250:251], s[38:39] offset:24\n\t" \
     "s_mov_b64 exec, -1\n\t" \
-    "L_noph2_3_%=:\n\t" \
+    "L_noph2_4_%=:\n\t" \
     "s_add_u32 s81, s97, 1\n\t" \
     "s_cmp_ge_u32 s81, %[nit]\n\t" \
     "s_cbranch_scc1 L_last_%=\n\t" \
@@ -18675,10 +18930,10 @@
     "s_waitcnt lgkmcnt(0)\n\t" \
     "s_waitcnt lgkmcnt(0)\n\t" \
     "s_or_b32 s81, %[prof_lo], %[prof_hi]\n\t" \
-    "s_cbranch_scc0 L_noph3_4_%=\n\t" \
+    "s_cbranch_scc0 L_noph3_5_%=\n\t" \
     "s_memtime s[98:99]\n\t" \
     "s_waitcnt lgkmcnt(0)\n\t" \
-    "L_noph3_4_%=:\n\t" \
+    "L_noph3_5_%=:\n\t" \
     "s_mov_b64 s[40:41], s[56:57]\n\t" \
     "s_mov_b64 s[42:43], s[58:59]\n\t" \
     "s_mov_b64 s[44:45], s[60:61]\n\t" \
@@ -19227,10 +19482,10 @@
     "s_waitcnt lgkmcnt(0)\n\t" \
     "s_waitcnt lgkmcnt(0)\n\t" \
     "s_or_b32 s81, %[prof_lo], %[prof_hi]\n\t" \
-    "s_cbranch_scc0 L_noph3_5_%=\n\t" \
+    "s_cbranch_scc0 L_noph3_6_%=\n\t" \
     "s_memtime s[98:99]\n\t" \
     "s_waitcnt lgkmcnt(0)\n\t" \
-    "L_noph3_5_%=:\n\t" \
+    "L_noph3_6_%=:\n\t" \
     "s_or_b32 s81, %[prof_lo], %[prof_hi]\n\t" \
     "s_cbranch_scc0 L_nostamp_end_%=\n\t" \
     "s_memtime s[20:21]\n\t" \
diff --git a/gta_amd/csrc/gta_fwd64.hip b/gta_amd/csrc/gta_fwd64.hip
--- a/gta_amd/csrc/gta_fwd64.hip
+++ b/gta_amd/csrc/gta_fwd64.hip
@@ -719,18 +719,14 @@
 template <int PAD4>
 __global__ __launch_bounds__(256, 1) void gta_attn64_items_kernel(const GtaFwdParams p_kernarg) {
     using A = A64<96, GTA_LAYOUT_MS>;
-    constexpr int CHP = A::CHP, KS = A::KS, DB = A::DB, R = A::R;
+    constexpr int CHP = A::CHP, KS = A::KS, DB = A::DB;
+    static_assert(A::R == 4 && A::NP == 3, "gen_item64.py's first fill: seven images of three pieces per wave");
     extern __shared__ __attribute__((aligned(16))) char smem[];
     const GtaFwdParams* const pp = &p_kernarg;
     const int tid = threadIdx.x;
     const int wave = __builtin_amdgcn_readfirstlane(tid >> 6);
     const int n_items = pp->n_items, G = gridDim.x;
     const int n_tiles = (pp->Tk + BN - 1) / BN;
-    const int woff = wave * (A::IMG / 4);
-    auto img_of = [&](int V) -> const char* {
-        const int bh = view_of(item_of64(V, n_items), pp->n_qtiles, pp->inv_nqt);
-        return (const char*)pp->kp + (long)bh * n_tiles * (long)A::TILE;
-    };
     if (pp->prof != nullptr && tid == 0) {
         unsigned long long* row = reinterpret_cast<unsigned long long*>(pp->prof) + 8l * blockIdx.x;
         row[1] = __builtin_readcyclecounter();
@@ -752,12 +748,6 @@
                 tab[(KS + 2 * d + hf) * 64 + lane] = (r * CHP + swz<CHP>(r, u)) * 16 + hb + A::OFF_V;
             }
         }
-        const unsigned voff16 = (unsigned)lane * 16u;
-        const char* img = img_of(blockIdx.x) + woff;
-#pragma unroll
-        for (int t = 0; t < R; ++t) dma_group<A::NP>(lds_addr(smem + A::OFF_K + t * A::IMG) + woff, img + (long)t * A::TILE, voff16);
-#pragma unroll
-        for (int t = 0; t < R - 1; ++t) dma_group<A::NP>(lds_addr(smem + A::OFF_V + t * A::IMG) + woff, img + (long)t * A::TILE + A::IMG, voff16);
     }
     const int n_mine = (n_items - (int)blockIdx.x + G - 1) / G;
     const int tailj = (pp->Tk & (BN - 1)) ? n_tiles - 1 : -1;
@@ -790,10 +780,11 @@
             const uint32_t qtb_lo = (uint32_t)(uintptr_t)pp->qtiles, qtb_hi = (uint32_t)((uintptr_t)pp->qtiles >> 32);
             const uint32_t prof_lo = (uint32_t)(uintptr_t)pp->prof, prof_hi = (uint32_t)((uintptr_t)pp->prof >> 32);
             const int Tk = pp->Tk;
+            const int first = __builtin_amdgcn_readfirstlane(k0 == 0 ? 1 : 0);
 #define A64_ITEMS(TEXT) do { GTA_ASM_M0_BEGIN asm volatile(TEXT \
                          : \
                          : [tabl] "s"(tabl), [nit] "s"(nit), [wave] "s"(wave), [qrb] "s"(qrb), [orb] "s"(orb), [qtb_lo] "s"(qtb_lo), [qtb_hi] "s"(qtb_hi), \
-                           [prof_lo] "s"(prof_lo), [prof_hi] "s"(prof_hi), [n] "s"(n_tiles), [tailj] "s"(tailj), [Tk] "s"(Tk) \
+                           [prof_lo] "s"(prof_lo), [prof_hi] "s"(prof_hi), [n] "s"(n_tiles), [tailj] "s"(tailj), [Tk] "s"(Tk), [first] "s"(first) \
                          : GTA_ATTN64_ITEMS_CLOBBERS); GTA_ASM_M0_END } while (0)
             if constexpr (PAD4 == 0) A64_ITEMS(GTA_ATTN64_ITEMS);
 #ifdef GTA_ATTN64_DIAG
```
